# mooch443/trex

Measured on AMD Instinct MI355X. Metric: frames/s end-to-end (segment+CNN-ID), 2048x2048 x100 individuals, higher is better.
Workload: dtype fp16x3-split

## Files before the change

include/trexhip.h:

```cpp
#ifndef TREXHIP_H
#define TREXHIP_H
#include <stddef.h>
#include <stdint.h>
#ifdef __cplusplus
extern "C" {
#endif

#define TREXHIP_ABI_VERSION 26

enum {
    TREXHIP_OK = 0,
    TREXHIP_E_INVALID = -1,
    TREXHIP_E_DEVICE = -2,
    TREXHIP_E_CAPACITY = -3,
    TREXHIP_E_UNSUPPORTED = -4,
    TREXHIP_E_NOMEM = -5
};

#define TREXHIP_FRAME_OVERFLOW_RUNS   1u
#define TREXHIP_FRAME_OVERFLOW_OUTPUT 2u
#define TREXHIP_FRAME_MALFORMED       4u

typedef struct trexhip_params {
    int32_t device;
    int32_t width, height;
    int32_t max_batch;
    int32_t max_runs;
    int32_t max_blobs;
    int32_t max_pixels;
    int32_t threshold;
    int32_t threshold_maximum;
    int32_t enable_difference;
    int32_t absolute_difference;
    int32_t image_invert;
    int32_t inclusive;
    int32_t zero_is_background;
    int32_t connectivity;
    int32_t dilation_size;
    int32_t use_closing;
    int32_t closing_size;
    int32_t n_ranges;
    double  cm_per_pixel;
    double  ranges[16];
    int32_t pixel_encoding;
    int32_t image_adjust, blur_difference, equalize_histogram, correct_luminance, use_adaptive_threshold;
    int32_t device_color_reduce;
    int32_t reserved_[1];
} trexhip_params;
enum { TREXHIP_ENC_GRAY = 0, TREXHIP_ENC_R3G3B2 = 1, TREXHIP_ENC_RGB8 = 2 };

#define TREXHIP_BLOB_IN_RANGE    0u
#define TREXHIP_BLOB_BELOW_RANGE 1u
#define TREXHIP_BLOB_BIG         2u

typedef struct trexhip_run { uint16_t x0, x1, y, pad; } trexhip_run;

typedef struct trexhip_blob {
    uint32_t run_begin, n_runs;
    uint32_t pix_begin, n_pixels;
    uint16_t x0, y0, x1, y1;
    uint32_t bid;
    uint32_t px_min_max;
    uint32_t parent;
    uint32_t flags;
    uint64_t m10, m01;
    uint64_t m20, m11, m02;
    uint64_t sp, spx, spy;
} trexhip_blob;

typedef struct trexhip_frame_info {
    uint32_t n_blobs, n_runs, n_pixels;
    uint32_t blob_begin, run_begin, pix_begin;
    uint32_t n_raw_runs, n_raw_blobs;
    uint32_t flags;
    uint32_t reserved[3];
} trexhip_frame_info;

typedef struct trexhip_batch_result {
    int32_t n_frames;
    uint32_t total_blobs, total_runs, total_pixels;
    const trexhip_frame_info* frames;
    const trexhip_blob* blobs;
    const trexhip_run* runs;
    const uint8_t* pixels;
    uint32_t pixel_channels;
    uint32_t reserved_;
} trexhip_batch_result;

typedef struct trexhip_device_view {
    const trexhip_frame_info* frames;
    const trexhip_blob* blobs;
// ... 96 lines not shown
    double  size_ranges[16];
} trexhip_split_params;
typedef struct trexhip_split_info {
    int32_t threshold;
    int32_t effective_threshold;
    int32_t status;
    int32_t initial_action;
    int32_t n_result;
    int32_t n_evaluated;
    int32_t min_pixel, max_pixel;
    float   first_size;
    float   reserved_;
    double  min_size_bound;
} trexhip_split_info;
void trexhip_default_split_params(trexhip_split_params* p);
int trexhip_split_search_device(trexhip_ctx* ctx, const trexhip_split_params* sp, int32_t method, const int32_t* d_presumed_nr,
                                int32_t n_blobs, int32_t* d_thresholds, trexhip_split_info* d_info);

typedef struct trexhip_posture_params {
    float   outline_resample;
    int32_t outline_smooth_samples;
    int32_t outline_smooth_step;
    int32_t outline_approximate;
    float   outline_curvature_range_ratio;
    float   midline_walk_offset;
    int32_t max_points;
    int32_t posture_closing_steps, peak_mode, posture_direction_smoothing;
} trexhip_posture_params;
typedef struct trexhip_posture_info { int32_t status, n_outline, n_segments, tail_index, head_index, n_traced, reserved[2]; } trexhip_posture_info;
void trexhip_default_posture_params(trexhip_posture_params* p);
int trexhip_posture_device(trexhip_ctx* ctx, int32_t table, const trexhip_posture_params* pp, int32_t n_blobs,
                           float* d_outline, float* d_segments, trexhip_posture_info* d_info);

int trexhip_posture_auto_device(trexhip_ctx* ctx, const trexhip_posture_params* pp, int32_t method, int32_t track_posture_threshold,
                                int32_t n_blobs, float* d_outline, float* d_segments, trexhip_posture_info* d_info,
                                int32_t* d_threshold_used, int32_t* d_iterations);

typedef struct trexhip_midline_params {
    int32_t midline_resolution;
    float   midline_stiff_percentage;
    int32_t midline_invert;
    int32_t midline_start_with_head;
} trexhip_midline_params;
typedef struct trexhip_midline_info { int32_t status, n; float len, angle, offx, offy; int32_t reserved[2]; } trexhip_midline_info;
void trexhip_default_midline_params(trexhip_midline_params* p);
int trexhip_midline_device(trexhip_ctx* ctx, const trexhip_midline_params* mp, int32_t n_blobs, int32_t max_points,
                           const trexhip_posture_info* d_posture_info, float* d_segments, float* d_midline,
                           trexhip_midline_info* d_midline_info);
int trexhip_midline_movement_device(trexhip_ctx* ctx, const trexhip_midline_params* mp, int32_t n_blobs, int32_t max_points,
                                    const trexhip_posture_info* d_posture_info, float* d_segments, float* d_midline,
                                    trexhip_midline_info* d_midline_info, const float* d_movement_direction);

enum { TREXHIP_NORMALIZE_NONE = 0, TREXHIP_NORMALIZE_MOMENTS = 1, TREXHIP_NORMALIZE_POSTURE = 2 };
int trexhip_crops_device(trexhip_ctx* ctx, uint8_t* d_crops, int32_t n_blobs, int32_t out_w, int32_t out_h,
                         int32_t normalization, int32_t difference);

int trexhip_crops_transformed_device(trexhip_ctx* ctx, uint8_t* d_crops, int32_t n_blobs, int32_t out_w, int32_t out_h,
                                     const float* transforms, const float* midline_lengths, int32_t use_legacy,
                                     float image_scale, int32_t difference);
int trexhip_crops_posture_device(trexhip_ctx* ctx, uint8_t* d_crops, int32_t n_blobs, int32_t out_w, int32_t out_h,
                                 const trexhip_midline_info* d_midline_info, const float* midline_lengths, int32_t use_legacy,
                                 float image_scale, int32_t difference);

int trexhip_load_weights(trexhip_ctx* ctx, const void* blob, size_t bytes);
int trexhip_num_classes(trexhip_ctx* ctx);
int trexhip_network_channels(trexhip_ctx* ctx);
int trexhip_network_image_size(trexhip_ctx* ctx, int32_t* width, int32_t* height);
enum { TREXHIP_NET_V118_3 = 0, TREXHIP_NET_V100 = 1, TREXHIP_NET_V110 = 2, TREXHIP_NET_V119 = 3, TREXHIP_NET_V200 = 4 };
int trexhip_network_version(trexhip_ctx* ctx);
size_t trexhip_network_blob_bytes(int32_t version, int32_t classes, int32_t channels, int32_t width, int32_t height);
int trexhip_identify_chunk_crops(trexhip_ctx* ctx, int32_t* crops);
enum { TREXHIP_CNN_FP32 = 0, TREXHIP_CNN_BF16X6 = 1, TREXHIP_CNN_BF16X3 = 2, TREXHIP_CNN_FP16X3 = 3 };
int trexhip_set_identity_precision(trexhip_ctx* ctx, int32_t mode);
int trexhip_identify_device(trexhip_ctx* ctx, const uint8_t* d_crops, int32_t n, float* d_probs, float* d_logits);
int trexhip_identify_prepare_device(trexhip_ctx* ctx, const uint8_t* d_crops, int32_t n);
int trexhip_identify_prepare_stats(trexhip_ctx* ctx, uint32_t* records, uint32_t* hits);
int trexhip_identify(trexhip_ctx* ctx, const uint8_t* crops, int32_t n, float* probs);
int trexhip_identify_guard_stats(trexhip_ctx* ctx, uint32_t* rerun_crops, uint32_t* whole_batch);
int trexhip_identify_skip_stats(trexhip_ctx* ctx, uint32_t* passes, uint32_t* listed, uint64_t* bytes_filled);

int trexhip_identify_skip3_stats(trexhip_ctx* ctx, uint32_t* pairs, uint32_t* listed, uint32_t* passes, uint64_t* bytes_filled);

int trexhip_identify_skip3x_stats(trexhip_ctx* ctx, uint32_t* crops_windowed, uint32_t* windowed_passes, uint32_t* full_passes);

int trexhip_identify_skipx_stats(trexhip_ctx* ctx, uint32_t* crops_windowed, uint32_t* windowed_passes, uint32_t* full_passes);

int trexhip_identify_bgrow_stats(trexhip_ctx* ctx, uint32_t* rows_read, uint32_t* rows_made);

int trexhip_identify_fc1_stats(trexhip_ctx* ctx, uint32_t* rows, uint32_t* listed);

int trexhip_export_id_table_device(trexhip_ctx* ctx, const float* d_probs, int32_t n_blobs, int32_t classes,
                                   uint32_t frame_base, void* d_table, int32_t max_rows);
int trexhip_export_id_table_ex_device(trexhip_ctx* ctx, const float* d_probs, int32_t n_blobs, int32_t classes, uint32_t frame_base,
                                      const float* d_midline, const trexhip_midline_info* d_midline_info, int32_t midline_resolution,
                                      void* d_table, int32_t max_rows);

typedef struct trexhip_comm trexhip_comm;
int trexhip_comm_unique_id(void* id128);
int trexhip_comm_create(trexhip_ctx* ctx, const void* id128, int32_t rank, int32_t world, trexhip_comm** out);
void trexhip_comm_destroy(trexhip_comm* comm);
int trexhip_comm_rank(trexhip_comm* comm);
int trexhip_comm_world(trexhip_comm* comm);
int trexhip_comm_gather_device(trexhip_comm* comm, const void* d_send, size_t bytes, void* d_recv_rank0);
int trexhip_comm_gather_device_on(trexhip_comm* comm, trexhip_ctx* stream_ctx, const void* d_send, size_t bytes, void* d_recv_rank0);
int trexhip_comm_count_ranks(trexhip_comm* comm, int32_t* ranks_seen);

enum { TREXHIP_STAGE_ROWS = 0, TREXHIP_STAGE_SEGMENT_ALL = 1, TREXHIP_STAGE_CONV2 = 2, TREXHIP_STAGE_CONV3 = 3,
       TREXHIP_STAGE_CNN_ALL = 4, TREXHIP_STAGE_CROPS = 5, TREXHIP_STAGE_POSTURE = 6,
       TREXHIP_STAGE_UPLOAD_COPY = 8, TREXHIP_STAGE_UPLOAD_DMA = 9,
       TREXHIP_STAGE_PREPARE = 10, TREXHIP_STAGE_COUNT = 11 };
int trexhip_profile_enable(trexhip_ctx* ctx, int32_t on);
int trexhip_profile_read(trexhip_ctx* ctx, int32_t stage, double* total_ms, int64_t* launches);
int trexhip_profile_reset(trexhip_ctx* ctx);

#define TREXHIP_NET_CATEGORY 100
typedef struct trexhip_trainer trexhip_trainer;
typedef struct {
    int32_t max_batch;
    float lr;
    float beta1, beta2, eps;
    float bn_momentum;
    float dropout;
    int32_t precision;
    uint64_t seed;
} trexhip_train_params;
size_t trexhip_weight_blob_bytes(int32_t classes, int32_t channels);
int trexhip_trainer_create(trexhip_ctx* ctx, const void* blob, size_t bytes, const trexhip_train_params* params, trexhip_trainer** out);
void trexhip_trainer_destroy(trexhip_trainer* trainer);
int trexhip_trainer_set_lr(trexhip_trainer* trainer, float lr);
int64_t trexhip_trainer_steps(trexhip_trainer* trainer);
int trexhip_trainer_image_size(trexhip_trainer* trainer, int32_t* width, int32_t* height);
int trexhip_trainer_version(trexhip_trainer* trainer, int32_t* version);
size_t trexhip_trainer_keep_mask_bytes(trexhip_trainer* trainer, int32_t n);
int trexhip_train_step_device(trexhip_trainer* trainer, const float* d_inputs, const int32_t* d_targets, int32_t n, const uint8_t* d_keep_masks,
                              float* loss, int32_t* correct);
int trexhip_train_eval_device(trexhip_trainer* trainer, const float* d_inputs, const int32_t* d_targets, int32_t n, float* loss, int32_t* correct);
int trexhip_train_eval(trexhip_trainer* trainer, const float* inputs, const int32_t* targets, int32_t n, float* loss, int32_t* correct);
int trexhip_train_step(trexhip_trainer* trainer, const float* inputs, const int32_t* targets, int32_t n, const uint8_t* keep_masks, float* loss,
                       int32_t* correct);
int trexhip_train_predict_device(trexhip_trainer* trainer, const uint8_t* d_crops, int32_t n, float* d_probs);
int trexhip_trainer_read(trexhip_trainer* trainer, int32_t tensor, int32_t kind, float* out, size_t count);
int trexhip_trainer_export(trexhip_trainer* trainer, void* blob, size_t capacity, size_t* bytes);

typedef struct {
    float degrees;
    float translate_x, translate_y;
    float brightness_lo, brightness_hi;
    float contrast_lo, contrast_hi;
    float saturation_lo, saturation_hi;
    float hue_lo, hue_hi;
    uint64_t seed;
} trexhip_augment_params;
typedef struct {
    float angle; int32_t tx, ty;
    float brightness, contrast, saturation, hue;
    int32_t order;
} trexhip_augment_draw;
void trexhip_default_augment_params(trexhip_augment_params* p, int32_t width, int32_t height);
int trexhip_augment_device(trexhip_ctx* ctx, const trexhip_augment_params* ap, const uint8_t* d_pool, const int32_t* d_pool_targets,
                           int32_t pool_size, const int32_t* indices, int32_t n, int32_t width, int32_t height, int32_t channels,
                           trexhip_augment_draw* d_draws, int32_t draws_given, uint64_t counter, float* d_out, int32_t* d_targets_out);

typedef struct {
    uint32_t good_frames, bad_frames;
    float    good_ratio;
    float    mean_unique;
// ... 65 lines not shown
```

trex_amd/capi.py:

```python
import collections
import ctypes as C
import os
import numpy as np

_HERE = os.path.dirname(os.path.abspath(__file__))
LIB_PATH = os.environ.get("TREXHIP_LIB_PATH") or os.path.join(_HERE, "libtrexhip.so")
_LIB = None

RUN_DTYPE = np.dtype([("x0", "<u2"), ("x1", "<u2"), ("y", "<u2"), ("pad", "<u2")])
BLOB_DTYPE = np.dtype([
    ("run_begin", "<u4"), ("n_runs", "<u4"), ("pix_begin", "<u4"), ("n_pixels", "<u4"),
    ("x0", "<u2"), ("y0", "<u2"), ("x1", "<u2"), ("y1", "<u2"),
    ("bid", "<u4"), ("px_min_max", "<u4"), ("parent", "<u4"), ("flags", "<u4"),
    ("m10", "<u8"), ("m01", "<u8"), ("m20", "<u8"), ("m11", "<u8"), ("m02", "<u8"),
    ("sp", "<u8"), ("spx", "<u8"), ("spy", "<u8"),
])
INFO_DTYPE = np.dtype([
    ("n_blobs", "<u4"), ("n_runs", "<u4"), ("n_pixels", "<u4"),
    ("blob_begin", "<u4"), ("run_begin", "<u4"), ("pix_begin", "<u4"),
    ("n_raw_runs", "<u4"), ("n_raw_blobs", "<u4"), ("flags", "<u4"), ("reserved", "<u4", (3,)),
])
assert BLOB_DTYPE.itemsize == 104 and RUN_DTYPE.itemsize == 8 and INFO_DTYPE.itemsize == 48

CNN_FP32, CNN_BF16X6, CNN_BF16X3, CNN_FP16X3 = 0, 1, 2, 3
# ... 74 lines not shown
MIDLINE_INFO_DTYPE = np.dtype([("status", "<i4"), ("n", "<i4"), ("len", "<f4"), ("angle", "<f4"), ("offx", "<f4"), ("offy", "<f4"),
                               ("reserved", "<i4", (2,))])
POSTURE_INFO_DTYPE = np.dtype([("status", "<i4"), ("n_outline", "<i4"), ("n_segments", "<i4"), ("tail_index", "<i4"),
                               ("head_index", "<i4"), ("n_traced", "<i4"), ("reserved", "<i4", (2,))])


class BatchResult(C.Structure):
    _fields_ = [
        ("n_frames", C.c_int32), ("total_blobs", C.c_uint32), ("total_runs", C.c_uint32), ("total_pixels", C.c_uint32),
        ("frames", C.c_void_p), ("blobs", C.c_void_p), ("runs", C.c_void_p), ("pixels", C.c_void_p),
        ("pixel_channels", C.c_uint32), ("reserved_", C.c_uint32),
    ]


ENC_GRAY, ENC_R3G3B2, ENC_RGB8 = 0, 1, 2
FRAME_OVERFLOW_RUNS, FRAME_OVERFLOW_OUTPUT, FRAME_MALFORMED = 1, 2, 4


class DeviceView(C.Structure):
    _fields_ = [("frames", C.c_void_p), ("blobs", C.c_void_p), ("runs", C.c_void_p), ("pixels", C.c_void_p),
                ("totals", C.c_void_p), ("blob_frame", C.c_void_p)]


class TrexHipError(RuntimeError):
    def __init__(self, code, msg):
        super().__init__(f"libtrexhip error {code}: {msg}")
        self.code = code
        self.frames = None


class TrainParams(C.Structure):
    _fields_ = [("max_batch", C.c_int32), ("lr", C.c_float), ("beta1", C.c_float), ("beta2", C.c_float), ("eps", C.c_float),
                ("bn_momentum", C.c_float), ("dropout", C.c_float), ("precision", C.c_int32), ("seed", C.c_uint64)]


class AugmentParams(C.Structure):
    _fields_ = [("degrees", C.c_float), ("translate_x", C.c_float), ("translate_y", C.c_float), ("brightness_lo", C.c_float), ("brightness_hi", C.c_float),
                ("contrast_lo", C.c_float), ("contrast_hi", C.c_float), ("saturation_lo", C.c_float), ("saturation_hi", C.c_float),
                ("hue_lo", C.c_float), ("hue_hi", C.c_float), ("seed", C.c_uint64)]


AUGMENT_DRAW_DTYPE = np.dtype([("angle", "<f4"), ("tx", "<i4"), ("ty", "<i4"), ("brightness", "<f4"), ("contrast", "<f4"), ("saturation", "<f4"),
                               ("hue", "<f4"), ("order", "<i4")])
assert AUGMENT_DRAW_DTYPE.itemsize == 32
AUGMENT_IDENTITY_ORDER = 0xE4


class UniquenessResult(C.Structure):
    _fields_ = [("good_frames", C.c_uint32), ("bad_frames", C.c_uint32), ("good_ratio", C.c_float), ("mean_unique", C.c_float), ("mean_unique_raw", C.c_float)]


class ValidationMetrics:
    __slots__ = ("confusion", "per_class_accuracy", "good_frames", "bad_frames", "good_ratio", "mean_unique", "mean_unique_raw",
                 "unique_percent", "unique_percent_raw", "uniqueness_per_class")

    def __init__(self):
        for k in self.__slots__:
            setattr(self, k, None)


class ClassAverages:
    __slots__ = ("samples", "values", "max_index", "max_p")

    def __init__(self, samples, values, max_index, max_p):
        self.samples, self.values, self.max_index, self.max_p = samples, values, max_index, max_p


class VisualFieldResult:
    __slots__ = VF_OUTPUTS

    def __init__(self):
        for k in self.__slots__:
            setattr(self, k, None)


TrackletLabels = collections.namedtuple("TrackletLabels", "counts rows label share skipped")


SYMBOLS = [
    "trexhip_abi_version", "trexhip_network_channels", "trexhip_network_image_size", "trexhip_network_version", "trexhip_network_blob_bytes", "trexhip_identify_chunk_crops", "trexhip_comm_unique_id", "trexhip_comm_create", "trexhip_comm_destroy", "trexhip_comm_rank", "trexhip_comm_world", "trexhip_comm_gather_device", "trexhip_comm_gather_device_on", "trexhip_comm_count_ranks", "trexhip_last_error", "trexhip_default_params", "trexhip_create", "trexhip_destroy",
    "trexhip_set_stream", "trexhip_get_live_params", "trexhip_update_params", "trexhip_set_background", "trexhip_set_background_device", "trexhip_set_background_color", "trexhip_set_background_color_device", "trexhip_generate_average_device", "trexhip_get_background", "trexhip_segment_device",
    "trexhip_segment", "trexhip_segment_color", "trexhip_segment_color_device", "trexhip_rethreshold_device", "trexhip_rethreshold_per_blob_device", "trexhip_fetch_rethreshold", "trexhip_fetch", "trexhip_device_view_get", "trexhip_synchronize",
    "trexhip_profile_enable", "trexhip_profile_read", "trexhip_profile_reset",
    "trexhip_default_posture_params", "trexhip_posture_device", "trexhip_posture_auto_device", "trexhip_pack_frames_v6_device", "trexhip_crops_device", "trexhip_pixel_channels", "trexhip_device_alloc", "trexhip_device_free", "trexhip_copy_to_host", "trexhip_copy_to_device", "trexhip_crops_transformed_device", "trexhip_crops_posture_device", "trexhip_default_midline_params", "trexhip_midline_device", "trexhip_midline_movement_device", "trexhip_default_split_params", "trexhip_split_search_device", "trexhip_export_id_table_device", "trexhip_export_id_table_ex_device", "trexhip_load_weights", "trexhip_set_identity_precision", "trexhip_num_classes", "trexhip_identify_device", "trexhip_identify", "trexhip_identify_guard_stats", "trexhip_identify_skip_stats", "trexhip_identify_skip3_stats", "trexhip_identify_skip3x_stats", "trexhip_identify_skipx_stats", "trexhip_identify_bgrow_stats", "trexhip_identify_fc1_stats",
    "trexhip_weight_blob_bytes", "trexhip_trainer_create", "trexhip_trainer_destroy", "trexhip_trainer_set_lr", "trexhip_trainer_steps", "trexhip_trainer_image_size", "trexhip_trainer_version", "trexhip_trainer_keep_mask_bytes", "trexhip_train_step_device", "trexhip_train_step", "trexhip_train_eval_device", "trexhip_train_eval", "trexhip_trainer_read", "trexhip_trainer_export",
    "trexhip_default_augment_params", "trexhip_augment_device",
    "trexhip_train_predict_device", "trexhip_validation_metrics_device", "trexhip_class_averages_device",
    "trexhip_lzo1x_bound", "trexhip_lzo1x_compress", "trexhip_pv_write_frames",
    "trexhip_load_frames_v6_device", "trexhip_lzo1x_decompress", "trexhip_pv_read_frames",
    "trexhip_default_prefilter_params", "trexhip_prefilter_device",
    "trexhip_default_vf_params", "trexhip_visual_field_device",
    "trexhip_categorize_load_weights", "trexhip_categorize_info", "trexhip_categorize_blob_bytes", "trexhip_categorize_device", "trexhip_categorize",
    "trexhip_tracklet_labels_device", "trexhip_tracklet_medians_device",
    "trexhip_identify_prepare_device", "trexhip_fetch_begin", "trexhip_fetch_wait", "trexhip_identify_prepare_stats",
]


def lib():
    global _LIB
    if _LIB is None:
        if not os.path.exists(LIB_PATH):
            raise TrexHipError(-1, f"{LIB_PATH} is missing: run __graft_entry__.build() (make -C trex_amd/csrc)")
        L = C.CDLL(LIB_PATH)
        L.trexhip_last_error.restype = C.c_char_p
        L.trexhip_default_params.argtypes = [C.POINTER(Params), C.c_int32, C.c_int32]
        L.trexhip_default_params.restype = None
        L.trexhip_create.argtypes = [C.POINTER(Params), C.POINTER(C.c_void_p)]
        L.trexhip_destroy.argtypes = [C.c_void_p]
        L.trexhip_destroy.restype = None
        L.trexhip_set_stream.argtypes = [C.c_void_p, C.c_void_p]
        L.trexhip_get_live_params.argtypes = [C.c_void_p, C.POINTER(LiveParams)]
        L.trexhip_update_params.argtypes = [C.c_void_p, C.POINTER(LiveParams)]
        L.trexhip_set_background.argtypes = [C.c_void_p, C.c_void_p, C.c_int32]
        L.trexhip_set_background_device.argtypes = [C.c_void_p, C.c_void_p]
        L.trexhip_set_background_color.argtypes = [C.c_void_p, C.c_void_p, C.c_int32, C.c_int32, C.c_int32]
        L.trexhip_set_background_color_device.argtypes = [C.c_void_p, C.c_void_p, C.c_int32, C.c_int32]
        L.trexhip_generate_average_device.argtypes = [C.c_void_p, C.c_void_p, C.c_int32, C.c_int32]
        L.trexhip_get_background.argtypes = [C.c_void_p, C.c_void_p, C.c_int32]
        L.trexhip_segment_device.argtypes = [C.c_void_p, C.c_void_p, C.c_int32]
        L.trexhip_segment.argtypes = [C.c_void_p, C.POINTER(C.c_void_p), C.c_int32, C.c_int32]
        L.trexhip_segment_color.argtypes = [C.c_void_p, C.POINTER(C.c_void_p), C.c_int32, C.c_int32, C.c_int32, C.c_int32]
        L.trexhip_segment_color_device.argtypes = [C.c_void_p, C.c_void_p, C.c_int32, C.c_int32, C.c_int32]
        L.trexhip_rethreshold_device.argtypes = [C.c_void_p, C.c_int32, C.c_int32, C.c_void_p, C.c_int32]
        L.trexhip_rethreshold_per_blob_device.argtypes = [C.c_void_p, C.c_int32, C.c_void_p, C.c_int32, C.c_void_p, C.c_int32]
        L.trexhip_fetch_rethreshold.argtypes = [C.c_void_p, C.POINTER(BatchResult)]
        L.trexhip_fetch.argtypes = [C.c_void_p, C.POINTER(BatchResult)]
        L.trexhip_fetch_begin.argtypes = [C.c_void_p, C.POINTER(BatchResult)]
        L.trexhip_fetch_wait.argtypes = [C.c_void_p]
        L.trexhip_device_view_get.argtypes = [C.c_void_p, C.POINTER(DeviceView)]
        L.trexhip_synchronize.argtypes = [C.c_void_p]
        L.trexhip_profile_enable.argtypes = [C.c_void_p, C.c_int32]
        L.trexhip_profile_read.argtypes = [C.c_void_p, C.c_int32, C.POINTER(C.c_double), C.POINTER(C.c_int64)]
        L.trexhip_profile_reset.argtypes = [C.c_void_p]
        L.trexhip_default_midline_params.argtypes = [C.POINTER(MidlineParams)]
        L.trexhip_default_midline_params.restype = None
        L.trexhip_midline_device.argtypes = [C.c_void_p, C.POINTER(MidlineParams), C.c_int32, C.c_int32, C.c_void_p, C.c_void_p, C.c_void_p, C.c_void_p]
        L.trexhip_midline_movement_device.argtypes = [C.c_void_p, C.POINTER(MidlineParams), C.c_int32, C.c_int32, C.c_void_p, C.c_void_p, C.c_void_p, C.c_void_p, C.c_void_p]
        L.trexhip_default_split_params.argtypes = [C.POINTER(SplitParams)]
        L.trexhip_default_split_params.restype = None
        L.trexhip_split_search_device.argtypes = [C.c_void_p, C.POINTER(SplitParams), C.c_int32, C.c_void_p, C.c_int32, C.c_void_p, C.c_void_p]
        L.trexhip_crops_posture_device.argtypes = [C.c_void_p, C.c_void_p, C.c_int32, C.c_int32, C.c_int32, C.c_void_p, C.c_void_p, C.c_int32, C.c_float, C.c_int32]
        L.trexhip_default_posture_params.argtypes = [C.POINTER(PostureParams)]
        L.trexhip_default_posture_params.restype = None
        L.trexhip_posture_device.argtypes = [C.c_void_p, C.c_int32, C.POINTER(PostureParams), C.c_int32, C.c_void_p, C.c_void_p, C.c_void_p]
        L.trexhip_posture_auto_device.argtypes = [C.c_void_p, C.POINTER(PostureParams), C.c_int32, C.c_int32, C.c_int32, C.c_void_p, C.c_void_p, C.c_void_p, C.c_void_p, C.c_void_p]
        L.trexhip_crops_transformed_device.argtypes = [C.c_void_p, C.c_void_p, C.c_int32, C.c_int32, C.c_int32, C.c_void_p, C.c_void_p, C.c_int32, C.c_float, C.c_int32]
        L.trexhip_crops_device.argtypes = [C.c_void_p, C.c_void_p] + [C.c_int32] * 5
        L.trexhip_export_id_table_device.argtypes = [C.c_void_p, C.c_void_p, C.c_int32, C.c_int32, C.c_uint32, C.c_void_p, C.c_int32]
        L.trexhip_export_id_table_ex_device.argtypes = [C.c_void_p, C.c_void_p, C.c_int32, C.c_int32, C.c_uint32, C.c_void_p, C.c_void_p, C.c_int32, C.c_void_p, C.c_int32]
        L.trexhip_load_weights.argtypes = [C.c_void_p, C.c_void_p, C.c_size_t]
        L.trexhip_num_classes.argtypes = [C.c_void_p]
        L.trexhip_network_channels.argtypes = [C.c_void_p]
        L.trexhip_network_image_size.argtypes = [C.c_void_p, C.POINTER(C.c_int32), C.POINTER(C.c_int32)]
        L.trexhip_network_version.argtypes = [C.c_void_p]
        L.trexhip_network_blob_bytes.argtypes = [C.c_int32] * 5; L.trexhip_network_blob_bytes.restype = C.c_size_t
        L.trexhip_identify_chunk_crops.argtypes = [C.c_void_p, C.POINTER(C.c_int32)]
        L.trexhip_pack_frames_v6_device.argtypes = [C.c_void_p, C.c_void_p, C.c_void_p, C.c_size_t, C.c_void_p]
        L.trexhip_lzo1x_bound.argtypes = [C.c_size_t]; L.trexhip_lzo1x_bound.restype = C.c_size_t
        L.trexhip_lzo1x_compress.argtypes = [C.c_void_p, C.c_size_t, C.c_void_p, C.c_size_t, C.POINTER(C.c_size_t)]
        L.trexhip_pv_write_frames.argtypes = [C.c_void_p, C.c_void_p, C.c_int32, C.c_int32, C.c_uint64, C.c_void_p, C.c_size_t, C.c_void_p, C.POINTER(C.c_size_t)]
        L.trexhip_load_frames_v6_device.argtypes = [C.c_void_p, C.c_void_p, C.c_void_p, C.c_int32, C.c_void_p]
        L.trexhip_lzo1x_decompress.argtypes = [C.c_void_p, C.c_size_t, C.c_void_p, C.c_size_t, C.POINTER(C.c_size_t)]
        L.trexhip_pv_read_frames.argtypes = [C.c_void_p, C.c_size_t, C.c_uint64, C.c_void_p, C.c_int32, C.c_void_p, C.c_size_t, C.c_void_p, C.POINTER(C.c_size_t)]
        L.trexhip_comm_unique_id.argtypes = [C.c_void_p]
        L.trexhip_comm_create.argtypes = [C.c_void_p, C.c_void_p, C.c_int32, C.c_int32, C.POINTER(C.c_void_p)]
        L.trexhip_comm_destroy.argtypes = [C.c_void_p]
        L.trexhip_comm_destroy.restype = None
        L.trexhip_comm_rank.argtypes = [C.c_void_p]
        L.trexhip_comm_world.argtypes = [C.c_void_p]
        L.trexhip_comm_gather_device.argtypes = [C.c_void_p, C.c_void_p, C.c_size_t, C.c_void_p]
        L.trexhip_comm_gather_device_on.argtypes = [C.c_void_p, C.c_void_p, C.c_void_p, C.c_size_t, C.c_void_p]
        L.trexhip_comm_count_ranks.argtypes = [C.c_void_p, C.POINTER(C.c_int32)]
        L.trexhip_set_identity_precision.argtypes = [C.c_void_p, C.c_int32]
        L.trexhip_identify_device.argtypes = [C.c_void_p, C.c_void_p, C.c_int32, C.c_void_p, C.c_void_p]
        L.trexhip_identify_prepare_device.argtypes = [C.c_void_p, C.c_void_p, C.c_int32]
        L.trexhip_identify_prepare_stats.argtypes = [C.c_void_p, C.POINTER(C.c_uint32), C.POINTER(C.c_uint32)]
        L.trexhip_identify.argtypes = [C.c_void_p, C.c_void_p, C.c_int32, C.c_void_p]
        L.trexhip_identify_guard_stats.argtypes = [C.c_void_p, C.POINTER(C.c_uint32), C.POINTER(C.c_uint32)]
        L.trexhip_identify_skip_stats.argtypes = [C.c_void_p, C.POINTER(C.c_uint32), C.POINTER(C.c_uint32), C.POINTER(C.c_uint64)]
        L.trexhip_identify_skipx_stats.argtypes = [C.c_void_p, C.POINTER(C.c_uint32), C.POINTER(C.c_uint32), C.POINTER(C.c_uint32)]
        L.trexhip_identify_bgrow_stats.argtypes = [C.c_void_p, C.POINTER(C.c_uint32), C.POINTER(C.c_uint32)]
        L.trexhip_identify_skip3x_stats.argtypes = [C.c_void_p, C.POINTER(C.c_uint32), C.POINTER(C.c_uint32), C.POINTER(C.c_uint32)]
        L.trexhip_identify_skip3_stats.argtypes = [C.c_void_p, C.POINTER(C.c_uint32), C.POINTER(C.c_uint32), C.POINTER(C.c_uint32), C.POINTER(C.c_uint64)]
        L.trexhip_identify_fc1_stats.argtypes = [C.c_void_p, C.POINTER(C.c_uint32), C.POINTER(C.c_uint32)]
        L.trexhip_weight_blob_bytes.argtypes = [C.c_int32, C.c_int32]
        L.trexhip_weight_blob_bytes.restype = C.c_size_t
        L.trexhip_trainer_create.argtypes = [C.c_void_p, C.c_void_p, C.c_size_t, C.POINTER(TrainParams), C.POINTER(C.c_void_p)]
        L.trexhip_trainer_destroy.argtypes = [C.c_void_p]
        L.trexhip_trainer_destroy.restype = None
        L.trexhip_trainer_set_lr.argtypes = [C.c_void_p, C.c_float]
        L.trexhip_trainer_steps.argtypes = [C.c_void_p]
        L.trexhip_trainer_steps.restype = C.c_int64
        L.trexhip_trainer_image_size.argtypes = [C.c_void_p, C.POINTER(C.c_int32), C.POINTER(C.c_int32)]
        L.trexhip_trainer_version.argtypes = [C.c_void_p, C.POINTER(C.c_int32)]
        L.trexhip_trainer_keep_mask_bytes.argtypes = [C.c_void_p, C.c_int32]
        L.trexhip_trainer_keep_mask_bytes.restype = C.c_size_t
        L.trexhip_train_step_device.argtypes = [C.c_void_p, C.c_void_p, C.c_void_p, C.c_int32, C.c_void_p, C.POINTER(C.c_float), C.POINTER(C.c_int32)]
        L.trexhip_train_step.argtypes = [C.c_void_p, C.c_void_p, C.c_void_p, C.c_int32, C.c_void_p, C.POINTER(C.c_float), C.POINTER(C.c_int32)]
        L.trexhip_train_eval_device.argtypes = [C.c_void_p, C.c_void_p, C.c_void_p, C.c_int32, C.POINTER(C.c_float), C.POINTER(C.c_int32)]
        L.trexhip_train_eval.argtypes = [C.c_void_p, C.c_void_p, C.c_void_p, C.c_int32, C.POINTER(C.c_float), C.POINTER(C.c_int32)]
        L.trexhip_trainer_read.argtypes = [C.c_void_p, C.c_int32, C.c_int32, C.c_void_p, C.c_size_t]
        L.trexhip_trainer_export.argtypes = [C.c_void_p, C.c_void_p, C.c_size_t, C.POINTER(C.c_size_t)]
        L.trexhip_default_augment_params.argtypes = [C.POINTER(AugmentParams), C.c_int32, C.c_int32]
        L.trexhip_default_augment_params.restype = None
        L.trexhip_augment_device.argtypes = [C.c_void_p, C.POINTER(AugmentParams), C.c_void_p, C.c_void_p, C.c_int32, C.c_void_p, C.c_int32, C.c_int32, C.c_int32,
                                             C.c_int32, C.c_void_p, C.c_int32, C.c_uint64, C.c_void_p, C.c_void_p]
        L.trexhip_train_predict_device.argtypes = [C.c_void_p, C.c_void_p, C.c_int32, C.c_void_p]
        L.trexhip_validation_metrics_device.argtypes = [C.c_void_p, C.c_void_p, C.c_int32, C.c_int32, C.c_void_p, C.c_void_p, C.c_int32, C.c_void_p,
                                                        C.POINTER(UniquenessResult), C.c_void_p, C.c_void_p, C.c_void_p]
        L.trexhip_class_averages_device.argtypes = [C.c_void_p, C.c_void_p, C.c_int32, C.c_int32, C.c_void_p, C.c_int32, C.c_void_p, C.c_void_p, C.c_void_p, C.c_void_p]
        L.trexhip_device_alloc.argtypes = [C.c_void_p, C.c_size_t, C.POINTER(C.c_void_p)]
        L.trexhip_device_free.argtypes = [C.c_void_p, C.c_void_p]
        L.trexhip_copy_to_host.argtypes = [C.c_void_p, C.c_void_p, C.c_void_p, C.c_size_t]
        L.trexhip_copy_to_device.argtypes = [C.c_void_p, C.c_void_p, C.c_void_p, C.c_size_t]
        L.trexhip_default_prefilter_params.argtypes = [C.POINTER(PrefilterParams)]
        L.trexhip_default_prefilter_params.restype = None
        L.trexhip_prefilter_device.argtypes = [C.c_void_p, C.POINTER(PrefilterParams), C.POINTER(PrefilterTables), C.c_void_p, C.c_void_p, C.c_void_p, C.c_void_p]
        L.trexhip_default_vf_params.argtypes = [C.c_void_p, C.POINTER(VfParams)]
        L.trexhip_default_vf_params.restype = None
        L.trexhip_visual_field_device.argtypes = [C.c_void_p, C.POINTER(VfParams), C.c_void_p, C.c_void_p, C.c_void_p, C.c_int32, C.c_void_p, C.c_int32,
                                                  C.c_void_p, C.c_int32, C.c_void_p, C.c_void_p, C.c_void_p, C.c_void_p, C.c_void_p, C.c_void_p]
        L.trexhip_categorize_load_weights.argtypes = [C.c_void_p, C.c_void_p, C.c_size_t]
        L.trexhip_categorize_info.argtypes = [C.c_void_p, C.POINTER(C.c_int32), C.POINTER(C.c_int32), C.POINTER(C.c_int32), C.POINTER(C.c_int32)]
        L.trexhip_categorize_blob_bytes.argtypes = [C.c_int32, C.c_int32, C.c_int32, C.c_int32]
        L.trexhip_categorize_blob_bytes.restype = C.c_size_t
        L.trexhip_categorize_device.argtypes = [C.c_void_p, C.c_void_p, C.c_int32, C.c_void_p, C.c_void_p, C.c_void_p]
        L.trexhip_categorize.argtypes = [C.c_void_p, C.c_void_p, C.c_int32, C.c_void_p]
        L.trexhip_tracklet_labels_device.argtypes = [C.c_void_p, C.c_void_p, C.c_void_p, C.c_int32, C.c_int32, C.c_int32, C.c_void_p, C.c_void_p, C.c_void_p,
                                                     C.c_void_p, C.POINTER(C.c_uint32)]
        L.trexhip_tracklet_medians_device.argtypes = [C.c_void_p, C.c_void_p, C.c_int32, C.c_int32, C.c_int32, C.c_int32, C.c_void_p, C.c_int32, C.c_void_p, C.c_void_p]
        _LIB = L
    return _LIB


def _check(rc):
    if rc != 0:
        raise TrexHipError(rc, lib().trexhip_last_error().decode())


def default_params(width, height, **kw):
    p = Params()
    lib().trexhip_default_params(C.byref(p), width, height)
    ranges = kw.pop("size_ranges", None)
    for k, v in kw.items():
        if not hasattr(p, k):
            raise KeyError(k)
        setattr(p, k, v)
    if ranges is not None:
        p.n_ranges = len(ranges)
        for i, (a, b) in enumerate(ranges):
            p.ranges[2 * i], p.ranges[2 * i + 1] = a, b
    return p


def default_augment_params(width, height, **kw):
    p = AugmentParams()
    lib().trexhip_default_augment_params(C.byref(p), width, height)
    for k, v in kw.items():
        if not hasattr(p, k):
            raise KeyError(k)
        setattr(p, k, v)
    return p


def _from_addr(addr, count, dtype):
# ... 223 lines not shown
                                                  None if ln is None else ln.ctypes.data_as(C.c_void_p), 1 if legacy else 0, scale, difference))

    def crops_transformed_device(self, d_crops_ptr, transforms, midline_lengths, out_w=80, out_h=80, legacy=False, scale=1.0, difference=0):
        tr = np.ascontiguousarray(transforms, np.float32)
        ln = np.ascontiguousarray(midline_lengths, np.float32)
        _check(lib().trexhip_crops_transformed_device(self._h, C.c_void_p(d_crops_ptr), len(tr), out_w, out_h, tr.ctypes.data_as(C.c_void_p),
                                                      ln.ctypes.data_as(C.c_void_p), 1 if legacy else 0, scale, difference))

    def export_id_table_ex(self, d_probs_ptr, n_blobs, classes, frame_base, d_table_ptr, max_rows, d_midline_ptr=0, d_midline_info_ptr=0, midline_resolution=0):
        _check(lib().trexhip_export_id_table_ex_device(self._h, C.c_void_p(d_probs_ptr) if d_probs_ptr else None, n_blobs, classes, frame_base,
                                                       C.c_void_p(d_midline_ptr) if d_midline_ptr else None,
                                                       C.c_void_p(d_midline_info_ptr) if d_midline_info_ptr else None, midline_resolution,
                                                       C.c_void_p(d_table_ptr), max_rows))

    def export_id_table(self, d_probs_ptr, n_blobs, classes, frame_base, d_table_ptr, max_rows):
        _check(lib().trexhip_export_id_table_device(self._h, C.c_void_p(d_probs_ptr) if d_probs_ptr else None, n_blobs,
                                                    classes, frame_base, C.c_void_p(d_table_ptr), max_rows))

    def load_weights(self, blob: bytes):
        buf = (C.c_uint8 * len(blob)).from_buffer_copy(blob)
        _check(lib().trexhip_load_weights(self._h, buf, len(blob)))

    def set_identity_precision(self, mode):
        _check(lib().trexhip_set_identity_precision(self._h, mode))

    def num_classes(self):
        return lib().trexhip_num_classes(self._h)

    def network_image_size(self):
        w, h = C.c_int32(0), C.c_int32(0)
        _check(lib().trexhip_network_image_size(self._h, C.byref(w), C.byref(h)))
        return int(w.value), int(h.value)

    def network_version(self):
        return int(lib().trexhip_network_version(self._h))

    def identify_chunk_crops(self):
        c = C.c_int32(0)
        _check(lib().trexhip_identify_chunk_crops(self._h, C.byref(c)))
        return int(c.value)

    def probabilities(self, crops):
        crops = np.ascontiguousarray(crops, np.uint8)
        w, h = self.network_image_size()
        if w:
            want = (h, w, lib().trexhip_network_channels(self._h))
            if crops.ndim != 4 or tuple(crops.shape[1:]) != want:
                raise ValueError(f"crops must have shape (n, {want[0]}, {want[1]}, {want[2]}) for the loaded network, got {crops.shape}")
        n = crops.shape[0]
        out = np.empty((n, self.num_classes()), np.float32)
        _check(lib().trexhip_identify(self._h, crops.ctypes.data_as(C.c_void_p), n, out.ctypes.data_as(C.c_void_p)))
        return out

    def guard_stats(self):
        a, b = C.c_uint32(0), C.c_uint32(0)
        _check(lib().trexhip_identify_guard_stats(self._h, C.byref(a), C.byref(b)))
        return int(a.value), bool(b.value)

    def skip_stats(self):
        a, b, c = C.c_uint32(0), C.c_uint32(0), C.c_uint64(0)
        _check(lib().trexhip_identify_skip_stats(self._h, C.byref(a), C.byref(b), C.byref(c)))
        return int(a.value), int(b.value), int(c.value)

    def skipx_stats(self):
        a, b, c = C.c_uint32(0), C.c_uint32(0), C.c_uint32(0)
        _check(lib().trexhip_identify_skipx_stats(self._h, C.byref(a), C.byref(b), C.byref(c)))
        return int(a.value), int(b.value), int(c.value)

    def bgrow_stats(self):
        a, b = C.c_uint32(0), C.c_uint32(0)
        _check(lib().trexhip_identify_bgrow_stats(self._h, C.byref(a), C.byref(b)))
        return int(a.value), int(b.value)

    def skip3_stats(self):
        a, b, c, d = C.c_uint32(0), C.c_uint32(0), C.c_uint32(0), C.c_uint64(0)
        _check(lib().trexhip_identify_skip3_stats(self._h, C.byref(a), C.byref(b), C.byref(c), C.byref(d)))
        return int(a.value), int(b.value), int(c.value), int(d.value)

    def skip3x_stats(self):
        a, b, c = C.c_uint32(0), C.c_uint32(0), C.c_uint32(0)
        _check(lib().trexhip_identify_skip3x_stats(self._h, C.byref(a), C.byref(b), C.byref(c)))
        return int(a.value), int(b.value), int(c.value)

    def fc1_stats(self):
        a, b = C.c_uint32(0), C.c_uint32(0)
        _check(lib().trexhip_identify_fc1_stats(self._h, C.byref(a), C.byref(b)))
        return int(a.value), int(b.value)

    def identify_device(self, d_crops_ptr, n, d_probs_ptr, d_logits_ptr=None):
        _check(lib().trexhip_identify_device(self._h, C.c_void_p(d_crops_ptr), n, C.c_void_p(d_probs_ptr),
                                             C.c_void_p(d_logits_ptr) if d_logits_ptr else None))

    def identify_prepare_device(self, d_crops_ptr, n):
        _check(lib().trexhip_identify_prepare_device(self._h, C.c_void_p(d_crops_ptr), n))

    def prepare_stats(self):
        a, b = C.c_uint32(0), C.c_uint32(0)
        _check(lib().trexhip_identify_prepare_stats(self._h, C.byref(a), C.byref(b)))
        return int(a.value), int(b.value)

    def device_alloc(self, nbytes):
        out = C.c_void_p()
        _check(lib().trexhip_device_alloc(self._h, nbytes, C.byref(out)))
        return int(out.value)

    def device_free(self, d_ptr):
        _check(lib().trexhip_device_free(self._h, C.c_void_p(d_ptr or 0)))

    def copy_to_device(self, d_ptr, array):
        a = np.ascontiguousarray(array)
        _check(lib().trexhip_copy_to_device(self._h, C.c_void_p(d_ptr), a.ctypes.data_as(C.c_void_p), a.nbytes))

    def copy_to_host(self, d_ptr, shape, dtype):
        out = np.empty(shape, dtype)
        _check(lib().trexhip_copy_to_host(self._h, out.ctypes.data_as(C.c_void_p), C.c_void_p(d_ptr), out.nbytes))
        return out

    def augment_device(self, d_pool_ptr, pool_size, n, width, height, channels, d_out_ptr, ap=None, indices=None, d_pool_targets_ptr=0,
                       d_targets_out_ptr=0, d_draws_ptr=0, draws_given=False, counter=0):
        idx = None
        if indices is not None:
            idx = np.ascontiguousarray(indices, np.int32)
            if idx.shape != (n,):
                raise ValueError(f"indices must hold n = {n} entries, got shape {idx.shape}")
        _check(lib().trexhip_augment_device(self._h, C.byref(ap) if ap is not None else None, C.c_void_p(d_pool_ptr), C.c_void_p(d_pool_targets_ptr or 0), pool_size,
                                            idx.ctypes.data_as(C.c_void_p) if idx is not None else None, n, width, height, channels,
                                            C.c_void_p(d_draws_ptr or 0), 1 if draws_given else 0, counter, C.c_void_p(d_out_ptr), C.c_void_p(d_targets_out_ptr or 0)))

    def validation_metrics(self, d_probs_ptr, n, classes, d_targets_ptr=0, frame_ranges=None):
        out = ValidationMetrics()
        conf = np.zeros((classes, classes), np.uint32) if d_targets_ptr else None
        fr = None
        res = UniquenessResult()
        up = upr = upc = None
        if frame_ranges is not None:
            fr = np.ascontiguousarray(frame_ranges, np.int32).reshape(-1, 2)
            up, upr, upc = np.zeros(len(fr), np.float32), np.zeros(len(fr), np.float32), np.zeros(classes, np.float32)
        ptr = lambda a: a.ctypes.data_as(C.c_void_p) if a is not None else None
        _check(lib().trexhip_validation_metrics_device(self._h, C.c_void_p(d_probs_ptr or 0), n, classes, C.c_void_p(d_targets_ptr or 0), ptr(fr),
                                                       len(fr) if fr is not None else 0, ptr(conf), C.byref(res) if fr is not None else None,
                                                       ptr(up), ptr(upr), ptr(upc)))
        if conf is not None:
            rows = conf.sum(axis=1, dtype=np.int64)
            out.confusion = conf
            out.per_class_accuracy = np.zeros(classes, np.float64)
            np.divide(np.diagonal(conf), rows, out=out.per_class_accuracy, where=rows > 0)
        if fr is not None:
            out.good_frames, out.bad_frames = int(res.good_frames), int(res.bad_frames)
            out.good_ratio, out.mean_unique, out.mean_unique_raw = float(res.good_ratio), float(res.mean_unique), float(res.mean_unique_raw)
            out.unique_percent, out.unique_percent_raw, out.uniqueness_per_class = up, upr, upc
        return out

    def class_averages(self, d_probs_ptr, n, classes, d_ids_ptr, n_ids):
        samples, values = np.zeros(max(n_ids, 0), np.float32), np.zeros((max(n_ids, 0), max(classes, 0)), np.float32)
        max_index, max_p = np.zeros(max(n_ids, 0), np.int32), np.zeros(max(n_ids, 0), np.float32)
        ptr = lambda a: a.ctypes.data_as(C.c_void_p)
        _check(lib().trexhip_class_averages_device(self._h, C.c_void_p(d_probs_ptr or 0), n, classes, C.c_void_p(d_ids_ptr or 0), n_ids,
                                                   ptr(samples), ptr(values), ptr(max_index), ptr(max_p)))
        return ClassAverages(samples, values, max_index, max_p)

    def load_category_weights(self, blob):
        _check(lib().trexhip_categorize_load_weights(self._h, blob, len(blob)))

    def category_info(self):
        v = [C.c_int32(0) for _ in range(4)]
        _check(lib().trexhip_categorize_info(self._h, *[C.byref(x) for x in v]))
# ... 429 lines not shown
```

trex_amd/csrc/cnn.hip:

```cpp
#include "cnn_net.h"
#include "cnn_arch.h"
#include "cnn_split.h"
#include "conv_tiled.h"
#include "cnn_weights.h"
#include <algorithm>
#include <cmath>
#include <cstdio>
#include <cstdlib>
#include <cstring>
#include <vector>

namespace trexhip {

template <int CH>
__global__ __launch_bounds__(256, 2) void k_conv1(const uint8_t* __restrict__ crops, const float* __restrict__ w ,
                                                  const float* __restrict__ bias , float* __restrict__ out, int S) {
    extern __shared__ __attribute__((aligned(16))) float lds[];
    const int PW = S + 4;
    float* wl = lds;
    float* img = lds + CH * 25 * 16;
    const int crop = blockIdx.x;
    const uint8_t* src = crops + (size_t)crop * S * S * CH;
    for (int i = threadIdx.x; i < CH * PW * PW; i += 256) img[i] = 0.f;
    for (int i = threadIdx.x; i < CH * 25 * 16; i += 256) wl[i] = w[i];
// ... 1169 lines not shown
    const int prc = parse_weight_blob(blob, bytes, "trexhip_load_weights", &wb, [](int W, int H) -> int {
        if (W < 8 || W > 256 || H < 8 || H > 256) {
            set_error("trexhip_load_weights: individual_image_size " + std::to_string(W) + "x" + std::to_string(H) + " is outside 8..256 x 8..256");
            return TREXHIP_E_UNSUPPORTED;
        }
        return TREXHIP_OK;
    });
    if (prc != TREXHIP_OK) return prc;
    const int classes = wb.classes, W = wb.W, H = wb.H, CH = wb.CH;
    const bool at80 = W == 80 && H == 80;

    TH_CHECK_HIP(hipSetDevice(ctx->p.device));
    free_net(static_cast<Net*>(ctx->net));
    ctx->net = nullptr;
    Net* net = new Net();
    net->classes = classes; net->W = W; net->H = H; net->CH = CH;
    int rc = TREXHIP_OK;
    const Folded c1 = fold_conv1(&wb.t[T_C1W], CH);
    TRY(upload(net, &net->w1, c1.w)); TRY(upload(net, &net->b1, c1.b));
    if (at80) TRY(upload(net, &net->w1h, &net->inv1h, pack_conv1_frags(c1.w, CH)));
    const Folded c2 = fold_conv(&wb.t[T_C2W], 64, 16, 16);
    TRY(upload(net, &net->w2, c2.w)); TRY(upload(net, &net->b2, c2.b));
    TRY(upload(net, &net->w2s, pack_bf16x3(c2.w, 16, 64)));
    TRY(upload(net, &net->w2h, &net->inv2h, pack_f16x2(c2.w, 16, 64)));
    if (at80) TRY(upload(net, &net->w2w, &net->inv2w, pack_wino_f16(c2.w, 16, 64)));
    const Folded c3 = fold_conv(&wb.t[T_C3W], 128, 64, 16);
    TRY(upload(net, &net->w3s, pack_bf16x3(c3.w, 64, 128)));
    TRY(upload(net, &net->w3h, &net->inv3h, pack_f16x2(c3.w, 64, 128)));
    if (at80) TRY(upload(net, &net->w3w, &net->inv3w, pack_wino_f16(c3.w, 64, 128)));
    TRY(net->weights.device_bytes(&net->d_ovf, OVF_WORDS * 4, "trexhip_load_weights"));
    if (rc == TREXHIP_OK && hipMemset(net->d_ovf, 0, OVF_WORDS * 4) != hipSuccess) rc = TREXHIP_E_DEVICE;
    const Folded c3x = fold_conv(&wb.t[T_C3W], 128, 64, 32);
    TRY(upload(net, &net->w3, c3x.w)); TRY(upload(net, &net->b3, c3x.b));
    const Folded f1 = pack_fc1(wb.t[T_F1W], wb.t[T_F1B], W, H);
    TRY(upload(net, &net->wf1, f1.w)); TRY(upload(net, &net->bf1, f1.b));
    if (at80) TRY(upload(net, &net->wf1h, &net->invf1h, pack_fc1_f16(f1.w)));
    TRY(upload(net, &net->lng, wb.t[T_LNG], 100 * sizeof(float)));
    TRY(upload(net, &net->lnb, wb.t[T_LNB], 100 * sizeof(float)));
    TRY(upload(net, &net->wf2t, pack_fc2(wb.t[T_F2W], classes)));
    TRY(upload(net, &net->bf2, wb.t[T_F2B], classes * sizeof(float)));
    if (at80 && CH == 1) TRY(make_empty_v3(ctx, net));
    if (rc != TREXHIP_OK) { free_net(net); return rc; }
    ctx->net = net;
    return TREXHIP_OK;
}

static int ensure_act(trexhip_ctx* ctx, Net* net, int n) {
    if (n <= net->max_crops) return TREXHIP_OK;
    drop_graphs(net);
    ctx->prepared.batch_reallocated();
    net->batch.free_all();
    net->h_probs = nullptr;
    net->max_crops = 0;
    Mem& B = net->batch;
    const char* who = "trexhip_identify_device";
    const size_t N = n;
    const size_t W = net->W, H = net->H;
    int rc = B.device_bytes(&net->d_ovfc, N, who);
    TRY(B.device_bytes(&net->act1, N * (H / 2) * (W / 2) * 16 * 4, who));
    TRY(B.device_bytes(&net->act2, N * (H / 4) * (W / 4) * 64 * 4, who));
    TRY(B.device_bytes(&net->act3, N * (H / 8) * (W / 8) * 128 * 4, who));
    TRY(B.device_bytes(&net->fc1, N * 128 * 4 * FC1_KSPLIT, who));
    TRY(B.device_bytes(&net->probs, N * net->classes * 4, who));
    TRY(B.device_bytes(&net->logits, N * net->classes * 4, who));
    if (W == 80 && H == 80) {
        TRY(B.device_bytes(&net->v2, N * 40 * V2_ROWB, who));
        const size_t img = net->v3e ? (size_t)SkipGeom::V3_ROWS * V3_ROWB : 0;
        TRY(B.device_bytes(&net->v3, N * 20 * V3_ROWB + 2 * img, who));
        if (rc == TREXHIP_OK && img) {
            TH_CHECK_HIP(hipMemcpyAsync(net->v3, net->v3e, img, hipMemcpyDeviceToDevice, ctx->stream));
            TH_CHECK_HIP(hipMemcpyAsync(net->v3 + img + N * 20 * V3_ROWB, net->v3e, img, hipMemcpyDeviceToDevice, ctx->stream));
            net->v3 += img;
        }
    }
    if (net->v3e) {
        const size_t n_pass = (N * SkipGeom::V3_ROWS + SkipGeom::RPP - 1) / SkipGeom::RPP;
        TRY(B.device_bytes(&net->skip_bands, N * sizeof(int2), who));
        TRY(B.device_bytes(&net->skip_counts, ((n_pass + SKIP_LB - 1) / SKIP_LB) * SKIP_NCNT * 4, who));
        TRY(B.device_bytes(&net->skip_list, (n_pass + SKIP_PAD) * 4, who));
        TRY(B.device_bytes(&net->skipx_cols, N * sizeof(int2), who));
        TRY(B.device_bytes(&net->skipx_list, (N * skipx_passes({0, SkipGeom::V3_ROWS - 1}) + SKIP_PAD) * 4, who));
        TRY(B.device_bytes(&net->skipx_rows, (N * skipx_passes({0, SkipGeom::V3_ROWS - 1}) + SKIP_PAD) * 4, who));
        const size_t blocks3 = (N + Skip3Geom::BLOCK - 1) / Skip3Geom::BLOCK;
        TRY(B.device_bytes(&net->skip3_counts, ((blocks3 + SKIP3_TB - 1) / SKIP3_TB) * sizeof(uint4), who));
        TRY(B.device_bytes(&net->skip3_tcounts, blocks3 * 2 * sizeof(uint32_t), who));
        TRY(B.device_bytes(&net->skip3_desc, blocks3 * Skip3Geom::BLOCK_PASSES * Skip3Geom::DESC * 4, who));
        TRY(B.device_bytes(&net->skip3_rows, blocks3 * Skip3Geom::BLOCK_PASSES * Skip3Reach::WORDS * 4, who));
        TRY(B.device_bytes(&net->skip3x_desc, blocks3 * Skip3XGeom::BLOCK_PASSES * Skip3XGeom::DESC * 4, who));
        TRY(B.device_bytes(&net->skip3x_rows, blocks3 * Skip3XGeom::BLOCK_PASSES * Skip3Reach::WORDS * 4, who));
        TRY(B.device_bytes(&net->fc1_list, Skip3Geom::PAIRS * N * sizeof(int), who));
    }
    TRY(B.device_bytes(&net->crops, N * net->W * net->H * net->CH, who));
    TRY(B.pinned(&net->h_probs, N * net->classes, who));
    if (rc != TREXHIP_OK) return rc;
    TH_CHECK_HIP(hipMemsetAsync(net->d_ovfc, 0, N, ctx->stream));
    net->max_crops = n;
    return TREXHIP_OK;
}
#undef TRY

std::vector<LdsAttr>& lds_attrs() { static std::vector<LdsAttr> v; return v; }

static const ByChannels K_CONV1{Kern(k_conv1<1>, 256, (84 * 84 + 25 * 16) * 4, false), Kern(k_conv1<3>, 256, 3 * (84 * 84 + 25 * 16) * 4, false)};
static const ByChannels K_CONV1_MFMA{Kern(k_conv1_mfma, 256), Kern(k_conv1_mfma3, 256)};
static const ByChannels K_CONV1_WPRE{Kern(k_conv1_wpre<1>, 256), Kern(k_conv1_wpre<3>, 256)};
static const Kern K_CONV12_RS(k_conv12_rs<W12RGeom>, 512, W12RGeom::LDS_BYTES);
static const Kern K_CONV12_RSX(k_conv12_rs<W12XGeom>, 512, W12XGeom::LDS_BYTES);
static const Kern K_CONV12_WPRE(k_conv12_wpre, 256, W12Geom::LDS_BYTES);
static const Kern K_CROP_BANDS(k_crop_bands, 256);
static const Kern K_PASS_COUNT(k_pass_count, SKIP_LB);
static const Kern K_PASS_LIST(k_pass_list, SKIP_LB);
static const Kern K_V3_FILL(k_v3_fill, SKIP_FILL_TB);
static const Kern K_CONV2_WPRE2(k_conv2_wpre2, 256, W2bGeom::LDS_BYTES);
static const Kern K_CONV2_STREAM(k_conv5_stream<16, 64, 40, 8, 4>, 256, ConvGeomS<16, 64, 40, 8, 4>::LDS_BYTES);
using GW3 = WinoGeom<64, 128, 20, 2>;
static const Kern K_CONV3_WINO(k_conv5_wino<64, 128, 20, 2>, GW3::NTHR, GW3::LDS_BYTES);
static const Kern K_CONV3_WPAIR(k_conv5_wpair<false>, 256, GW3::LDS_BYTES + 1024 );
static const Kern K_CONV3_WPAIR_LIST(k_conv5_wpair<true>, 256, GW3::LDS_BYTES + 1024);
using GW3X = Wino3Pass<Skip3XGeom::TILES, Skip3XGeom::NR>;
static const Kern K_CONV3_WPAIR_LISTX(k_conv5_wpair<true, Skip3XGeom>, 256, GW3X::LDS_BYTES + 1024);
static const Kern K_PAIR_COUNT(k_pair_count, SKIP3_NT);
static const Kern K_PAIR_LIST(k_pair_list, SKIP3_NT);
static const Kern K_ACT3_FILL(k_act3_fill, 256);
template <int CI, int CO, int S, int ROWS, int NTERMS>
static auto split_kern() { return Kern(k_conv5_split<CI, CO, S, ROWS, NTERMS>, 512, ConvGeomB<CI, CO, S, ROWS, SPLIT_NP>::LDS_BYTES); }
struct ExactLayer { decltype(Kern(k_conv5<16, 64, 40, 20, 16>, 512)) f32; decltype(split_kern<16, 64, 40, 10, 6>()) x6, x3, x6_plan; };
static const auto K_CONV2_X6 = split_kern<16, 64, 40, 10, 6>();
static const ExactLayer K_CONV2{Kern(k_conv5<16, 64, 40, 20, 16>, 512, ConvGeom<16, 64, 40, 20, 16>::LDS_BYTES), K_CONV2_X6, split_kern<16, 64, 40, 10, 3>(), K_CONV2_X6};
static const ExactLayer K_CONV3{Kern(k_conv5<64, 128, 20, 20, 32>, 512, ConvGeom<64, 128, 20, 20, 32>::LDS_BYTES), split_kern<64, 128, 20, 20, 6>(),
                                split_kern<64, 128, 20, 20, 3>(), split_kern<64, 128, 20, 4, 6>()};
static const Kern K_FC1(k_fc1, 256);
static const Kern K_FC1_SPLIT1(k_fc1_split<1>, 256), K_FC1_SPLIT4(k_fc1_split<4>, 256), K_FC1_SPLIT4_LIST(k_fc1_split<4, true>, 256);
static const Kern K_FC1_LIST(k_fc1_list, FC1L_TB);
static const Kern K_HEAD(k_head, 256);
static const Kern K_HEAD_SMALL(k_head_small, 256);
static const Kern K_GUARD_PLAN(k_guard_plan, 1024);

struct Pass {
    const Net& net; const CnnPlan& p; hipStream_t s; int mode;
    const uint8_t* crops; int n; float *probs, *logits;
};

static void launch_conv1(const Pass& f, const Conv1 kind, const uint32_t* guard) {
    const Net& net = f.net;
    switch (kind) {
    case Conv1::FUSED: break;
    case Conv1::WPRE: K_CONV1_WPRE[net.CH](f.s, f.p.conv1_grid, f.crops, net.w1h, net.b1, net.v2, net.inv1h, net.ovf(OVF_RANGE)); break;
    case Conv1::MFMA: K_CONV1_MFMA[net.CH](f.s, f.p.conv1_grid, f.crops, net.w1h, net.b1, net.act1, net.inv1h, guard); break;
    case Conv1::VALU: K_CONV1[net.CH](f.s, f.p.conv1_grid, f.crops, net.w1, net.b1, net.act1, net.W); break;
    case Conv1::ANY: any_conv1(f.s, net, f.p, f.crops); break;
    }
}

static void launch_exact(const Pass& f, const int layer, const int mode, const uint32_t* guard) {
    const Net& net = f.net;
    const bool c2 = layer == 2;
    const ExactLayer& K = c2 ? K_CONV2 : K_CONV3;
    const Launch& l = guard ? (c2 ? f.p.r_conv2 : f.p.r_conv3) : (c2 ? f.p.conv2 : f.p.conv3);
    const float *in = c2 ? net.act1 : net.act2, *b = c2 ? net.b2 : net.b3;
    float* out = c2 ? net.act2 : net.act3;
    if (mode == TREXHIP_CNN_FP32) K.f32(f.s, l.grid, in, c2 ? net.w2 : net.w3, b, out);
    else (guard ? K.x6_plan : mode == TREXHIP_CNN_BF16X6 ? K.x6 : K.x3)(f.s, l.grid, in, c2 ? net.w2s : net.w3s, b, out, 1.0f, guard, l.items);
}

static void launch_tail(const Pass& f, const uint32_t* guard) {
    const Net& net = f.net;
    const CnnPlan& p = f.p;
    if (guard || p.fc1 == Fc1::EXACT)
        K_FC1(f.s, dim3(guard ? p.r_fc1_grid : p.fc1_grid, p.planes), net.act3, net.wf1, net.bf1, net.fc1, f.n, p.K, guard);
    else if (p.fc1_listed)
        K_FC1_SPLIT4_LIST(f.s, dim3(p.fc1_grid, p.planes), net.act3, net.wf1h, net.bf1, net.fc1, f.n, p.K, net.invf1h, net.ovf(OVF_RANGE), net.d_ovfc,
                          net.fc1_list, net.d_skip + SK3_FC1_LEN, net.max_crops);
    else
        (p.fc1 == Fc1::SPLIT1 ? K_FC1_SPLIT1 : K_FC1_SPLIT4)(f.s, dim3(p.fc1_grid, p.planes), net.act3, net.wf1h, net.bf1, net.fc1, f.n, p.K, net.invf1h,
                                                            net.ovf(OVF_RANGE), net.d_ovfc, nullptr, nullptr, 0);
    if (guard || p.head == Head::BIG) {
        const bool listed = !guard && p.fc1_listed;
        K_HEAD(f.s, guard ? p.r_head_grid : p.head_grid, net.fc1, net.lng, net.lnb, net.wf2t, net.bf2, f.probs, f.logits, f.n, net.classes, guard, p.planes,
               listed ? net.fc1e : nullptr, listed ? net.skip_bands : nullptr, listed ? net.d_skip : nullptr);
    }
    else
        K_HEAD_SMALL(f.s, p.head_grid, net.fc1, net.lng, net.lnb, net.wf2t, net.bf2, f.probs, f.logits, f.n, net.classes, p.planes,
                     p.head_plans ? net.ovf(OVF_RANGE) : nullptr, net.d_ovfc, p.head_plans ? net.ovf(OVF_PLAN) : nullptr);
}

static void launch_rerun(const Pass& f) {
    const uint32_t* g = f.net.ovf(OVF_PLAN);
    if (!f.p.head_plans) K_GUARD_PLAN(f.s, 1, f.net.ovf(OVF_RANGE), f.net.d_ovfc, f.n, f.net.ovf(OVF_PLAN));
    if (f.p.rerun_conv1) launch_conv1(f, Conv1::MFMA, g);
    for (const int layer : {2, 3}) {
        if (f.p.chain == Chain::ANY_SIZE) any_conv(f.s, f.net, f.p, layer, TREXHIP_CNN_BF16X6, g);
        else launch_exact(f, layer, TREXHIP_CNN_BF16X6, g);
    }
    launch_tail(f, g);
}

static int make_empty_v3(trexhip_ctx* ctx, Net* net) {
    const char* who = "trexhip_load_weights";
    uint8_t* zero = nullptr;
    int rc = net->weights.device_bytes(&net->v3e, (size_t)SkipGeom::V3_ROWS * V3_ROWB, who);
    if (rc == TREXHIP_OK) rc = net->weights.device_bytes(&net->act3e, (size_t)Skip3Geom::PAIRS * 10 * 128 * 4, who);
    if (rc == TREXHIP_OK) rc = net->weights.device_bytes(&net->fc1e, (size_t)FC1_KSPLIT * 128 * 4, who);
    if (rc == TREXHIP_OK) rc = net->weights.device_bytes(&net->d_skip, SK_WORDS * 4, who);
    if (rc == TREXHIP_OK) rc = net->weights.device_bytes(&net->act2e, (size_t)SkipGeom::V3_ROWS * 20 * 64 * 4, who);
    if (rc == TREXHIP_OK) rc = net->weights.device_bytes(&net->bgtab, (size_t)W2xGeom::NBG * W2xGeom::BG_UNITS * sizeof(uint4), who);
    if (rc == TREXHIP_OK) rc = net->weights.device_bytes(&zero, SkipGeom::CROP_ROWS * 80, who);
    if (rc != TREXHIP_OK) return rc;
    const CnnPlan p = cnn_plan(80, 80, 1, TREXHIP_CNN_FP16X3, true, GEOM_ROLE_SPLIT | GEOM_NO_SKIP, 1, ctx->n_cus);
    TH_CHECK_HIP(hipFuncSetAttribute(reinterpret_cast<const void*>(K_CONV12_RS.fn), hipFuncAttributeMaxDynamicSharedMemorySize, K_CONV12_RS.lds));
    TH_CHECK_HIP(hipMemsetAsync(net->d_skip, 0, SK_WORDS * 4, ctx->stream));
    TH_CHECK_HIP(hipMemsetAsync(zero, 0, SkipGeom::CROP_ROWS * 80, ctx->stream));
    K_CONV12_RS(ctx->stream, p.conv2.grid, zero, net->w1h, net->b1, net->inv1h, net->w2w, net->b2, net->v3e, net->inv2w, net->d_skip + SK_EMPTY_RANGE, 1,
                net->d_skip + SK_EMPTY_CTR, p.pk2, nullptr, nullptr, nullptr, net->act2e, nullptr, nullptr);
    TH_CHECK_HIP(hipGetLastError());
    TH_CHECK_HIP(hipFuncSetAttribute(reinterpret_cast<const void*>(K_CONV12_RSX.fn), hipFuncAttributeMaxDynamicSharedMemorySize, K_CONV12_RSX.lds));
    K_CONV12_RSX(ctx->stream, 1, zero, net->w1h, net->b1, net->inv1h, net->w2w, net->b2, net->v3e, net->inv2w, net->d_skip + SK_EMPTY_RANGE, 1,
                 net->d_skip + SKX_CTR, 1, nullptr, nullptr, nullptr, net->act2e, nullptr, net->bgtab);
    TH_CHECK_HIP(hipGetLastError());
    TH_CHECK_HIP(hipFuncSetAttribute(reinterpret_cast<const void*>(K_CONV3_WPAIR.fn), hipFuncAttributeMaxDynamicSharedMemorySize, K_CONV3_WPAIR.lds));
    K_CONV3_WPAIR(ctx->stream, p.conv3.grid, net->v3e, net->w3w, net->b3, net->act3e, net->inv3w, 1, net->d_skip + SK3_EMPTY_CTR, p.n_big3, nullptr, nullptr, nullptr);
    TH_CHECK_HIP(hipGetLastError());
    const CnnPlan pf = cnn_plan(80, 80, 1, TREXHIP_CNN_FP16X3, true, 0, 1, ctx->n_cus);
    K_FC1_SPLIT4(ctx->stream, dim3(1, pf.planes), net->act3e, net->wf1h, net->bf1, net->fc1e, 1, pf.K, net->invf1h, net->d_skip + SK3_FC1E_RANGE, nullptr,
                 nullptr, nullptr, 0);
    TH_CHECK_HIP(hipGetLastError());
    uint32_t range = 0;
    TH_CHECK_HIP(hipMemcpyAsync(&range, net->d_skip + SK3_FC1E_RANGE, 4, hipMemcpyDeviceToHost, ctx->stream));
    TH_CHECK_HIP(hipStreamSynchronize(ctx->stream));
    if (range) {
        const uint32_t one = 1;
        TH_CHECK_HIP(hipMemcpy(net->d_skip + SK_EMPTY_RANGE, &one, 4, hipMemcpyHostToDevice));
    }
    return TREXHIP_OK;
}

struct PrepArgs { long long alloc_rows; bool direct, x3 ; };
static PrepArgs prep_args(const Net& net, const CnnPlan& p) {
    const long long alloc_rows = (long long)net.max_crops * SkipGeom::V3_ROWS;
    const bool direct = p.v3_direct && skip3_direct_fits(alloc_rows);
    return {alloc_rows, direct, p.skip3x && direct && skip3x_direct_fits(alloc_rows)};
}
static void launch_skip_prep(const Pass& f, const bool direct, const bool x3) {
    const Net& net = f.net;
    const CnnPlan& p = f.p;
    const int n = f.n, lb = ceil_div(p.conv2.items, SKIP_LB);
    int2* cols = p.skipx ? net.skipx_cols : nullptr;
    K_CROP_BANDS(f.s, ceil_div(n, 4), f.crops, n, net.skip_bands, cols || x3 ? net.skipx_cols : nullptr);
    K_PASS_COUNT(f.s, lb, net.skip_bands, cols, n, net.d_skip, net.skip_counts, (int)p.bgrows);
    K_PASS_LIST(f.s, lb, net.skip_bands, cols, n, net.d_skip, net.skip_counts, net.skip_list, net.skipx_list, net.skipx_rows, (int)p.bgrows);
    if (p.skip3) {
        const int2* cols3 = x3 ? net.skipx_cols : nullptr;
        K_PAIR_COUNT(f.s, p.skip3_grid, net.skip_bands, cols3, n, net.d_skip, net.skip3_counts, net.skip3_tcounts);
        K_PAIR_LIST(f.s, p.skip3_grid, net.skip_bands, cols3, n, net.d_skip, net.skip3_counts, net.skip3_tcounts, net.skip3_desc, net.skip3x_desc);
        if (p.fc1_listed) K_FC1_LIST(f.s, Skip3Geom::PAIRS, net.skip_bands, n, net.d_skip, net.fc1_list, net.max_crops);
    }
    K_V3_FILL(f.s, ceil_div(n * SkipGeom::V3_ROWS, SKIP_FILL_TB), net.skip_bands, cols, n, net.d_skip, reinterpret_cast<const uint4*>(net.v3e),
              reinterpret_cast<uint4*>(net.v3), (int)direct);
}

enum : int { PREP_LISTS = 1, PREP_ACT3 = 2 };
static bool plan_prepares(const CnnPlan& p) { return p.chain == Chain::ROLE_SPLIT && p.skip; }
static void launch_prep(const Pass& f, const int parts) {
    const Net& net = f.net;
    const CnnPlan& p = f.p;
    if (!plan_prepares(p)) return;
    const PrepArgs a = prep_args(net, p);
    if (parts & PREP_LISTS) launch_skip_prep(f, a.direct, a.x3);
    if ((parts & PREP_ACT3) && p.skip3)
        K_ACT3_FILL(f.s, p.act3_fill.grid, net.skip_bands, a.x3 ? net.skipx_cols : nullptr, f.n, net.d_skip, reinterpret_cast<const uint4*>(net.act3e),
                    reinterpret_cast<uint4*>(net.act3), net.skip3_desc, net.skip3_rows, net.skip3x_desc, net.skip3x_rows, a.alloc_rows, (int)a.direct, (int)!p.fc1_listed);
}

static int set_cnn_attrs(trexhip_ctx* ctx) {
    if (!ctx->attr_cnn) {
        for (const LdsAttr& a : lds_attrs()) TH_CHECK_HIP(hipFuncSetAttribute(a.fn, hipFuncAttributeMaxDynamicSharedMemorySize, a.bytes));
        ctx->attr_cnn = true;
    }
    return TREXHIP_OK;
}

static int net_forward_launch(trexhip_ctx* ctx, const uint8_t* d_crops, int n, float* d_probs, float* d_logits, const bool prepared = false) {
    const Net& net = *static_cast<Net*>(ctx->net);
    if (const int rc = set_cnn_attrs(ctx)) return rc;
    const CnnPlan p = cnn_plan(net.W, net.H, net.CH, ctx->cnn_mode, (reinterpret_cast<uintptr_t>(d_crops) & 15) == 0, ctx->tune_conv_geom, n, ctx->n_cus);
    const Pass f{net, p, ctx->stream, ctx->cnn_mode, d_crops, n, d_probs, d_logits};
    hipStream_t s = f.s;
    const bool x3 = prep_args(net, p).x3;
    stage_begin(ctx, TREXHIP_STAGE_CNN_ALL);
    launch_conv1(f, p.conv1, nullptr);
    if (p.chain == Chain::ANY_SIZE) {
        any_conv(s, net, p, 2, f.mode, nullptr);
        any_conv(s, net, p, 3, f.mode, nullptr);
    } else {
        const bool pre = p.chain == Chain::ROLE_SPLIT || p.chain == Chain::FUSED_2WG || p.chain == Chain::TWO_KERNEL;
        stage_begin(ctx, TREXHIP_STAGE_CONV2);
        switch (p.chain) {
        case Chain::ROLE_SPLIT:
            if (!prepared) launch_prep(f, PREP_LISTS);
            if (p.skipx)
                K_CONV12_RSX(s, p.conv2.grid, d_crops, net.w1h, net.b1, net.inv1h, net.w2w, net.b2, net.v3, net.inv2w, net.ovf(OVF_RANGE), n, net.d_skip + SKX_CTR,
                             p.pk2, net.d_ovfc, net.skipx_list, net.d_skip + SKX_PASSES, net.act2e, net.skipx_rows, net.bgtab);
            K_CONV12_RS(s, p.conv2.grid, d_crops, net.w1h, net.b1, net.inv1h, net.w2w, net.b2, net.v3, net.inv2w, net.ovf(OVF_RANGE), n, net.ovf(OVF_PASS2),
                        p.pk2, net.d_ovfc, p.skip ? net.skip_list : nullptr, p.skip ? net.d_skip + (p.skipx ? SKX_FULL : SK_LEN) : nullptr, nullptr, nullptr, nullptr);
            break;
        case Chain::FUSED_2WG:
            K_CONV12_WPRE(s, p.conv2.grid, d_crops, net.w1h, net.b1, net.inv1h, net.w2w, net.b2, net.v3, net.inv2w, net.ovf(OVF_RANGE), n, net.ovf(OVF_PASS2),
                          p.pk2, net.d_ovfc);
            break;
        case Chain::TWO_KERNEL:
            K_CONV2_WPRE2(s, p.conv2.grid, net.v2, net.w2w, net.b2, net.v3, net.inv2w, net.ovf(OVF_RANGE), n, net.ovf(OVF_PASS2));
            break;
        case Chain::FP32_ACT:
            K_CONV2_STREAM(s, p.conv2.grid, net.act1, net.w2h, net.b2, net.act2, net.inv2h, net.ovf(OVF_RANGE), p.conv2.items);
            break;
        default: launch_exact(f, 2, f.mode, nullptr);
        }
        stage_end(ctx, TREXHIP_STAGE_CONV2);
        stage_begin(ctx, TREXHIP_STAGE_CONV3);
        if (pre) {
            if (p.skip3) {
                if (!prepared) launch_prep(f, PREP_ACT3);
                if (x3)
                    K_CONV3_WPAIR_LISTX(s, p.conv3.grid, net.v3, net.w3w, net.b3, net.act3, net.inv3w, n, net.d_skip + SK3X_CTR, 0, net.skip3x_desc, net.skip3x_rows, net.d_skip);
                K_CONV3_WPAIR_LIST(s, p.conv3.grid, net.v3, net.w3w, net.b3, net.act3, net.inv3w, n, net.ovf(OVF_PASS3), 0, net.skip3_desc, net.skip3_rows, net.d_skip);
            }
            K_CONV3_WPAIR(s, p.conv3.grid, net.v3, net.w3w, net.b3, net.act3, net.inv3w, n, net.ovf(OVF_PASS3), p.n_big3, nullptr, nullptr, p.skip3 ? net.d_skip : nullptr);
        }
        else if (p.chain == Chain::FP32_ACT)
            K_CONV3_WINO(s, p.conv3.grid, net.act2, net.w3w, net.b3, net.act3, net.inv3w, net.ovf(OVF_RANGE), n, net.ovf(OVF_PASS3));
        else launch_exact(f, 3, f.mode, nullptr);
        stage_end(ctx, TREXHIP_STAGE_CONV3);
    }
    launch_tail(f, nullptr);
    if (p.rerun) launch_rerun(f);
    stage_end(ctx, TREXHIP_STAGE_CNN_ALL);
    TH_CHECK_HIP(hipGetLastError());
    return TREXHIP_OK;
}

static constexpr int GRAPH_MAX_CROPS = 6400;
static constexpr size_t GRAPH_CACHE = 8;
static constexpr int GRAPH_MIN_SEEN = 3;

static bool graph_path(const trexhip_ctx* ctx, const Net* net, const int n) {
    static const bool enabled = [] { const char* e = std::getenv("TREXHIP_GRAPHS"); return !(e && std::atoi(e) == 0); }();
    return enabled && net->graphs_ok && n <= GRAPH_MAX_CROPS && !ctx->profiling && ctx->attr_cnn;
}

static int net_forward_inner(trexhip_ctx* ctx, const uint8_t* d_crops, int n, float* d_probs, float* d_logits, bool prepared);
int net_forward(trexhip_ctx* ctx, const uint8_t* d_crops, int n, float* d_probs, float* d_logits) {
    Net* net = static_cast<Net*>(ctx->net);
    const bool prepared = ctx->prepared.consume(ctx->prepared.make(d_crops, n, ctx->cnn_mode, ctx->tune_conv_geom, ctx->stream));
    if (ctx->cnn_mode == TREXHIP_CNN_FP16X3) {
        if (!net->ovf_clean) TH_CHECK_HIP(hipMemsetAsync(net->d_ovf, 0, OVF_PLAN * 4, ctx->stream));
        net->ovf_clean = false;
    }
    const int rc = net_forward_inner(ctx, d_crops, n, d_probs, d_logits, prepared);
    if (rc == TREXHIP_OK) { net->last_mode = ctx->cnn_mode; if (ctx->cnn_mode == TREXHIP_CNN_FP16X3) net->ovf_clean = true; }
    net->last_fc1_n = rc == TREXHIP_OK && !net->arch && cnn_plan(net->W, net->H, net->CH, ctx->cnn_mode, (reinterpret_cast<uintptr_t>(d_crops) & 15) == 0,
                                                                 ctx->tune_conv_geom, n, ctx->n_cus).fc1_listed ? n : 0;
    return rc;
}

static bool capture_chain(trexhip_ctx* ctx, Net* net, Net::GraphEntry* cand, const uint8_t* d_crops, int n, float* d_probs, float* d_logits) {
    hipGraph_t graph = nullptr;
    hipGraphExec_t exec = nullptr;
    hipEvent_t ev = nullptr;
    bool ok = hipStreamBeginCapture(ctx->stream, hipStreamCaptureModeThreadLocal) == hipSuccess;
    if (ok) {
        const int rc = net_forward_launch(ctx, d_crops, n, d_probs, d_logits);
        const hipError_t e_end = hipStreamEndCapture(ctx->stream, &graph);
        ok = rc == TREXHIP_OK && e_end == hipSuccess && graph && hipGraphInstantiate(&exec, graph, nullptr, nullptr, 0) == hipSuccess &&
             hipEventCreateWithFlags(&ev, hipEventDisableTiming) == hipSuccess;
    }
    if (graph) (void)hipGraphDestroy(graph);
    if (!ok) {
        (void)hipGetLastError();
        if (exec) (void)hipGraphExecDestroy(exec);
        net->graphs_ok = false;
        return false;
    }
    cand->exec = exec; cand->last = ev;
    return true;
}

static int net_forward_inner(trexhip_ctx* ctx, const uint8_t* d_crops, int n, float* d_probs, float* d_logits, const bool prepared) {
    Net* net = static_cast<Net*>(ctx->net);
    if (net->arch) return arch_forward(ctx, *net, d_crops, n, d_probs, d_logits);
    if (!graph_path(ctx, net, n)) return net_forward_launch(ctx, d_crops, n, d_probs, d_logits, prepared);
    hipStream_t s = ctx->stream;
    const Net::GraphKey key{d_crops, n, d_probs, d_logits, ctx->cnn_mode, ctx->tune_conv_geom, s};
    ++net->tick;
    Net::GraphEntry* cand = nullptr;
    for (auto& g : net->graphs)
        if (g.key == key) { cand = &g; break; }
    if (!cand) {
        if (net->graphs.size() >= GRAPH_CACHE) {
            size_t lru = 0;
            for (size_t i = 1; i < net->graphs.size(); ++i) if (net->graphs[i].used < net->graphs[lru].used) lru = i;
            destroy_graph_entry(net->graphs[lru]);
            net->graphs.erase(net->graphs.begin() + (long)lru);
        }
        net->graphs.push_back({key, nullptr, net->tick, nullptr, 1});
        return net_forward_launch(ctx, d_crops, n, d_probs, d_logits);
    }
    cand->used = net->tick;
    if (!cand->exec && (++cand->seen < GRAPH_MIN_SEEN || !capture_chain(ctx, net, cand, d_crops, n, d_probs, d_logits)))
// ... 50 lines not shown
    ctx->prepared.set(ctx->prepared.make(d_crops, n, ctx->cnn_mode, ctx->tune_conv_geom, ctx->stream));
    return TREXHIP_OK;
}

int trexhip_identify_prepare_stats(trexhip_ctx* ctx, uint32_t* records, uint32_t* hits) {
    if (!ctx) { set_error("trexhip_identify_prepare_stats: null ctx"); return TREXHIP_E_INVALID; }
    if (records) *records = ctx->prepared.records;
    if (hits) *hits = ctx->prepared.hits;
    return TREXHIP_OK;
}

int trexhip_identify(trexhip_ctx* ctx, const uint8_t* crops, int32_t n, float* probs) {
    Net* net;
    int rc = identify_prepare(ctx, ctx && crops && probs, "trexhip_identify", n, &net);
    if (rc || !net) return rc;
    const size_t cb = (size_t)net->W * net->H * net->CH;
    TH_CHECK_HIP(hipMemcpyAsync(net->crops, crops, cb * n, hipMemcpyHostToDevice, ctx->stream));
    rc = net_forward(ctx, net->crops, n, net->probs, nullptr);
    if (rc) return rc;
    TH_CHECK_HIP(hipMemcpyAsync(probs, net->probs, (size_t)n * net->classes * 4, hipMemcpyDeviceToHost, ctx->stream));
    TH_CHECK_HIP(hipStreamSynchronize(ctx->stream));
    return TREXHIP_OK;
}

int trexhip_identify_guard_stats(trexhip_ctx* ctx, uint32_t* rerun_crops, uint32_t* whole_batch) {
    if (!ctx || !ctx->net) { set_error("trexhip_identify_guard_stats: no context / weights not loaded"); return TREXHIP_E_INVALID; }
    Net* net = static_cast<Net*>(ctx->net);
    uint32_t plan[2] = {0, 0};
    TH_CHECK_HIP(hipStreamSynchronize(ctx->stream));
    if (net->last_mode == TREXHIP_CNN_FP16X3 && net->arch) {
        uint32_t st[2] = {0, 0};
        TH_CHECK_HIP(hipMemcpy(st, net->ovf(ARCH_STAT_RERUN), 8, hipMemcpyDeviceToHost));
        if (rerun_crops) *rerun_crops = st[0];
        if (whole_batch) *whole_batch = st[1] ? 1u : 0u;
        return TREXHIP_OK;
    }
    if (net->last_mode == TREXHIP_CNN_FP16X3) TH_CHECK_HIP(hipMemcpy(plan, net->ovf(OVF_PLAN), 8, hipMemcpyDeviceToHost));
    if (rerun_crops) *rerun_crops = plan[1] == 1u ? plan[0] : 0u;
    if (whole_batch) *whole_batch = plan[1] == 2u ? 1u : 0u;
    return TREXHIP_OK;
}

static int read_skip_words(trexhip_ctx* ctx, const char* who, uint32_t (&w)[SK_WORDS]) {
    if (!ctx || !ctx->net) { set_error(std::string(who) + ": no context / weights not loaded"); return TREXHIP_E_INVALID; }
    const Net* net = static_cast<Net*>(ctx->net);
    std::fill(w, w + SK_WORDS, 0u);
    TH_CHECK_HIP(hipStreamSynchronize(ctx->stream));
    if (net->d_skip) TH_CHECK_HIP(hipMemcpy(w, net->d_skip, sizeof w, hipMemcpyDeviceToHost));
    return TREXHIP_OK;
}

int trexhip_identify_skip_stats(trexhip_ctx* ctx, uint32_t* passes, uint32_t* listed, uint64_t* bytes_filled) {
    uint32_t w[SK_WORDS];
    if (const int rc = read_skip_words(ctx, "trexhip_identify_skip_stats", w)) return rc;
    if (passes) *passes = w[SK_NPASS];
    if (listed) *listed = w[SK_LEN];
    if (bytes_filled) *bytes_filled = (uint64_t)w[SK_FILLED] * V3_ROWB;
    return TREXHIP_OK;
}

int trexhip_identify_skipx_stats(trexhip_ctx* ctx, uint32_t* crops_windowed, uint32_t* windowed_passes, uint32_t* full_passes) {
    uint32_t w[SK_WORDS];
    if (const int rc = read_skip_words(ctx, "trexhip_identify_skipx_stats", w)) return rc;
    if (crops_windowed) *crops_windowed = w[SKX_CROPS];
    if (windowed_passes) *windowed_passes = w[SKX_PASSES];
    if (full_passes) *full_passes = w[SKX_FULL];
    return TREXHIP_OK;
}

int trexhip_identify_bgrow_stats(trexhip_ctx* ctx, uint32_t* rows_read, uint32_t* rows_made) {
    uint32_t w[SK_WORDS];
    if (const int rc = read_skip_words(ctx, "trexhip_identify_bgrow_stats", w)) return rc;
    if (rows_read) *rows_read = w[SKX_V2_READ];
    if (rows_made) *rows_made = w[SKX_V2_MADE];
    return TREXHIP_OK;
}

int trexhip_identify_skip3x_stats(trexhip_ctx* ctx, uint32_t* crops_windowed, uint32_t* windowed_passes, uint32_t* full_passes) {
    uint32_t w[SK_WORDS];
    if (const int rc = read_skip_words(ctx, "trexhip_identify_skip3x_stats", w)) return rc;
    if (crops_windowed) *crops_windowed = w[SK3_USE] ? w[SK3X_CROPS] : 0u;
    if (windowed_passes) *windowed_passes = w[SK3_USE] ? w[SK3X_PASSES] : 0u;
    if (full_passes) *full_passes = w[SK3_USE] ? w[SK3_PASSES] : 0u;
    return TREXHIP_OK;
}

int trexhip_identify_skip3_stats(trexhip_ctx* ctx, uint32_t* pairs, uint32_t* listed, uint32_t* passes, uint64_t* bytes_filled) {
    uint32_t w[SK_WORDS];
    if (const int rc = read_skip_words(ctx, "trexhip_identify_skip3_stats", w)) return rc;
    if (pairs) *pairs = w[SK3_PAIRS];
    if (listed) *listed = w[SK3_LISTED];
    uint32_t by_rows = w[SK3_PASSES];
    if (passes && w[SK3_USE] && w[SK3X_PASSES]) {
        const Net* net = static_cast<Net*>(ctx->net);
        const int n = (int)(w[SK3_PAIRS] / Skip3Geom::PAIRS);
        std::vector<int2> bands((size_t)n);
        TH_CHECK_HIP(hipMemcpy(bands.data(), net->skip_bands, (size_t)n * sizeof(int2), hipMemcpyDeviceToHost));
        int count = 0;
        for (int c0 = 0; c0 < n; c0 += Skip3Geom::BLOCK) {
            Skip3Pass p{};
            for (int c = c0; c < n && c < c0 + Skip3Geom::BLOCK; ++c) {
                const SkipPairs r = skip3_pairs({bands[(size_t)c].x, bands[(size_t)c].y});
                if (r.lo <= r.hi) skip3_add_run(p, count, c * Skip3Geom::PAIRS + r.lo, r.hi - r.lo + 1, [](int, const Skip3Pass&) {});
            }
            skip3_flush(p, count, [](int, const Skip3Pass&) {});
        }
        by_rows = (uint32_t)count;
    }
    if (passes) *passes = w[SK3_USE] ? by_rows : 0u;
    if (bytes_filled) *bytes_filled = (uint64_t)w[SK3_FILLED] * (10 * 128 * 4);
    return TREXHIP_OK;
}

int trexhip_identify_fc1_stats(trexhip_ctx* ctx, uint32_t* rows, uint32_t* listed) {
    uint32_t w[SK_WORDS];
    if (const int rc = read_skip_words(ctx, "trexhip_identify_fc1_stats", w)) return rc;
    const Net* net = static_cast<Net*>(ctx->net);
    uint32_t sum = 0;
    for (int q = 0; q < Skip3Geom::PAIRS && net->last_fc1_n; ++q) sum += w[SK3_FC1_LEN + q];
    if (rows) *rows = (uint32_t)net->last_fc1_n * Skip3Geom::PAIRS;
    if (listed) *listed = sum;
    return TREXHIP_OK;
}

int trexhip_set_identity_precision(trexhip_ctx* ctx, int32_t mode) {
    if (!ctx || mode < 0 || mode > 3) { set_error("trexhip_set_identity_precision: mode must be one of TREXHIP_CNN_*"); return TREXHIP_E_INVALID; }
    ctx->cnn_mode = mode;
    ctx->prepared.precision_changed();
    return TREXHIP_OK;
}

int trexhip_num_classes(trexhip_ctx* ctx) {
    if (!ctx || !ctx->net) return 0;
    return static_cast<Net*>(ctx->net)->classes;
}

int trexhip_network_version(trexhip_ctx* ctx) {
    if (!ctx || !ctx->net) return 0;
    const Net* net = static_cast<const Net*>(ctx->net);
    return net->arch ? net->arch->plan.spec->id : TREXHIP_NET_V118_3;
}

size_t trexhip_network_blob_bytes(int32_t version, int32_t classes, int32_t channels, int32_t width, int32_t height) {
    return arch_blob_bytes(version, classes, channels, width, height);
}

int trexhip_identify_chunk_crops(trexhip_ctx* ctx, int32_t* crops) {
    if (!ctx || !crops) { set_error("trexhip_identify_chunk_crops: null argument"); return TREXHIP_E_INVALID; }
    const Net* net = static_cast<const Net*>(ctx->net);
    *crops = net && net->arch ? net->arch->plan.chunk : 0;
    return TREXHIP_OK;
}

int trexhip_network_channels(trexhip_ctx* ctx) {
    if (!ctx || !ctx->net) return 0;
    return static_cast<Net*>(ctx->net)->CH;
}

int trexhip_network_image_size(trexhip_ctx* ctx, int32_t* width, int32_t* height) {
    if (!ctx) { set_error("trexhip_network_image_size: null context"); return TREXHIP_E_INVALID; }
    const Net* net = static_cast<const Net*>(ctx->net);
    if (width) *width = net ? net->W : 0;
    if (height) *height = net ? net->H : 0;
    return TREXHIP_OK;
}

// ... 10 lines not shown
```

trex_amd/csrc/cnn_conv3p.h:

```cpp

template <bool LISTED, class L = Skip3Geom>
__global__ __launch_bounds__(256) void k_conv5_wpair(const uint8_t* __restrict__ v3, const uint4* __restrict__ wp ,
                                                     const float* __restrict__ bias, float* __restrict__ out, const float out_scale,
                                                     const int n_crops, uint32_t* __restrict__ pass_ctr,
                                                     const int n_big_dense ,
                                                     const int* __restrict__ desc ,
                                                     const uint32_t* __restrict__ rowsrc ,
                                                     const uint32_t* __restrict__ words ) {
    constexpr int CI = 64, CO = 128, S = 20, TPW = 2;
    constexpr int BD = 5;
    constexpr int AD = 1;
    constexpr int PK = 4;
    constexpr int DT0 = 2;
    using G = WinoGeom<CI, CO, S, TPW>;
    static_assert(G::NTHR == 256 && G::RP0 == 1280 && G::NCH * 2 * G::RP0 == V3_ROWB && G::NT == 4 && G::WM == 1, "geometry");
    static_assert(BD >= 1 && BD <= 7, "weight ring of 8 taps");
    extern __shared__ __attribute__((aligned(16))) uint8_t ldsb[];
    __shared__ int s_next_pass;
    const int tid = threadIdx.x, lane = tid & 63, wave = __builtin_amdgcn_readfirstlane(tid >> 6);
    const int j = lane & 31, h = lane >> 5;
    using LR = Skip3Reach;
    using P = Wino3Pass<L::TILES, L::NR>;
    constexpr bool WIN = L::TILES != G::TPR;
    static_assert(LISTED || !WIN, "only a listed pass has a window");
    static_assert(LR::ROWB == V3_ROWB && SkipGeom::V3_ROWS == S, "the images in front of V3 and behind it are S rows of V3_ROWB bytes");
    static_assert((WIN || (P::NR == G::NR && P::RP == G::RP && P::BUF == G::BUF)) && L::SLOTS * P::TPP <= G::MB && L::PAIRS * 2 == S, "a listed pass fits the dense pass's rows and tiles");
    if (words && (words[SK3_USE] != 0) != LISTED) return;
    const int total_tiles = n_crops * G::TPC;
    const int n_pass = LISTED ? __builtin_amdgcn_readfirstlane((int)words[WIN ? SK3X_PASSES : SK3_PASSES]) : (total_tiles + G::MB - 1) / G::MB;
    const int n_big = LISTED ? (n_pass >= 16 * (int)gridDim.x ? (int)((long long)n_pass * 7 / 8) / 4 : 0) : n_big_dense;
    const int big_end = n_big * PK;
    auto ticket_first = [&](const int t) { return t < n_big ? t * PK : big_end + (t - n_big); };
    int pass = ticket_first((int)blockIdx.x);
    if (pass >= n_pass) return;
    const uint32_t lds0 = (uint32_t)(uintptr_t)ldsb;
    constexpr int RNG = (2 * P::NR + 1) * P::RP, NI = (RNG + 1023) / 1024, NDW = (NI + 3) / 4;
    static_assert(DT0 + NDW <= 40 - BD, "the DMA instructions are older than the last 2 BD weight loads of a unit");
    static_assert(NI * 1024 - RNG <= 1024, "slack behind the second buffer");
    uint32_t dvo[NDW];
#pragma unroll
    for (int k = 0; k < NDW; ++k) {
        const int o = (wave + 4 * k) * 1024 + lane * 16;
        const int pc = o >= (P::NR + 1) * P::RP ? 1 : 0, q = o - pc * (P::NR + 1) * P::RP;
        const int row = q / P::RP, w = q - row * P::RP;
        const bool real = q < P::NR * P::RP && o < RNG;
        const int wv = WIN ? (w / P::PS) * G::PS + w % P::PS : w;
        const uint32_t inrow = (uint32_t)(pc * 1280 + (w < P::RP0 ? wv : G::RP0 - 16 - (WIN ? 2 * LR::TILEB : 0)));
        dvo[k] = LISTED ? (real ? (uint32_t)row << LR::ROW_SHIFT | inrow : (uint32_t)P::NR << LR::ROW_SHIFT)
                        : real ? (uint32_t)(row * V3_ROWB) + inrow : 0x80000000u;
    }
    const uint32_t mbase = (uint32_t)__builtin_amdgcn_readfirstlane((int)(lds0 + P::RP + wave * 1024));
    auto stage_rsrc = [&](const int g, const int qmin_, const int nrows_) {
        const unsigned long long base = wave_uniform64(reinterpret_cast<unsigned long long>(v3) + (unsigned long long)(long long)(qmin_ - (LISTED ? S : 0)) * V3_ROWB + (unsigned)(g * 2560));
        return __builtin_amdgcn_make_buffer_rsrc(reinterpret_cast<void*>(base), 0,
                                                 LISTED ? (int)(LR::NUM_RECORDS - (unsigned)(g * 2560)) : __builtin_amdgcn_readfirstlane(nrows_ * V3_ROWB - g * 2560), 0x00020000);
    };
#define P3_SRC(k_, tab_) (uint32_t)__builtin_amdgcn_ds_bpermute((int)(dvo[k_] >> (LR::ROW_SHIFT - 2)), (int)(tab_))
#define P3_DMA(k_, srs_, buf_, src_)                                                                                             \
    do {                                                                                                                         \
        if ((k_) < NDW - 1 || wave + 4 * (NDW - 1) < NI) {                                                                       \
            const uint32_t vo_ = LISTED ? dvo[k_] + (src_) : dvo[k_];                                                            \
            asm volatile("s_add_u32 m0, %0, %1\n\ts_nop 0\n\tbuffer_load_dwordx4 %2, %3, 0 offen lds"                          \
                         :: "s"(mbase), "n"((buf_) * P::BUF + (k_) * 4096), "v"(vo_), "s"(srs_) : "memory", "scc");               \
        }                                                                                                                        \
    } while (0)
    for (int i = tid; i < 4 * (P::RP / 16); i += G::NTHR) {
        const int pl = i / (P::RP / 16), o = i - pl * (P::RP / 16);
        *reinterpret_cast<uint4*>(ldsb + pl * P::PLANE + o * 16) = make_uint4(0, 0, 0, 0);
    }
    const __amdgpu_buffer_rsrc_t wrs = make_rsrc(wp, (uint32_t)(G::NCH * 40 * G::BV * 16));
    const int boff = (h * CO + wave * 32 + j) * 16;
    const int co = wave * 32 + j;
    const float bz = bias[co];
    const int ooff = (4 * h * CO + co) * 4;
    int lps[TPW], lr2[TPW];
#pragma unroll
    for (int m = 0; m < TPW; ++m) {
        const int t = m * 32 + j;
        lps[m] = t / P::TPP < L::SLOTS ? t / P::TPP : L::SLOTS - 1;
        lr2[m] = t % P::TPP;
    }
    int raw_w = 0, ent[TPW] = {};
    uint32_t tab = 0;
    auto pass_fetch = [&](const int pass_) {
        const int* d = desc + (size_t)pass_ * L::DESC;
        raw_w = d[lane & (L::DESC - 1)];
        tab = rowsrc[(size_t)pass_ * LR::WORDS + (lane & (LR::WORDS - 1))];
#pragma unroll
        for (int m = 0; m < TPW; ++m) ent[m] = d[S3_SLOT + lps[m]];
    };
    auto pass_decode = [&](int& qmin_, int& gp0_, int& span_, uint32_t (&rel_)[L::SLOTS]) {
        const int w = raw_w;
        qmin_ = __builtin_amdgcn_readlane((int)tab, LR::BASE);
        gp0_ = __builtin_amdgcn_readlane(w, S3_GP0);
        span_ = __builtin_amdgcn_readlane(w, S3_SPAN);
#pragma unroll
        for (int s2 = 0; s2 < L::SLOTS; ++s2) {
            const uint32_t e = (uint32_t)__builtin_amdgcn_readlane(w, S3_SLOT + s2), rp = e >> 16;
            rel_[s2] = rp == (uint32_t)S3_IDLE ? 0x80000000u
                     : rp * (uint32_t)(G::TPP * CO * 4) + (WIN ? ((e >> S3_T0_SHIFT) & S3_T0_MASK) * (uint32_t)(2 * CO * 4) : 0u);
        }
    };
    int qmin = 0, nrows = 0, gp0 = 0, span = 0;
    uint32_t rel[L::SLOTS] = {};
    if (LISTED) { pass_fetch(pass); pass_decode(qmin, gp0, span, rel); }
    else wino_pass_rows<G, S>(pass, total_tiles, qmin, nrows);
    const __amdgpu_buffer_rsrc_t srs0 = stage_rsrc(0, qmin, nrows);
#pragma unroll
    for (int k = 0; k < NDW; ++k) P3_DMA(k, srs0, 0, P3_SRC(k, tab));
    asm volatile("s_waitcnt vmcnt(0)" ::: "memory");
    __syncthreads();
    auto w_off = [](const int g, const int tt) {
        const int hp = tt & 1, p = g == 3 ? (hp ? 7 : 0) : 2 * g + 1 + hp;
        return ((tt / 10) * 40 + ((tt % 10) / 2) * 8 + p) * G::BV * 16;
    };
    uint4 bq[8][2];
#pragma unroll
    for (int t = 0; t < BD; ++t) {
        bq[t][0] = buf_load16(wrs, boff, w_off(0, t));
        bq[t][1] = buf_load16(wrs, boff, w_off(0, t) + 2 * CO * 16);
    }
    auto a_base = [&](const int pass_, const int qmin_, const int m, int& inr, int& zr, int& yy) {
        if (LISTED) {
            const int r2 = lr2[m], par = r2 & 1, e = ent[m];
            yy = 2 * ((e >> 8) & (WIN ? S3_Q_MASK : 0xff)) + par; zr = (r2 >> 1) * 32 + h * 16; inr = ((e & 0xff) + par) * P::RP + zr;
            return;
        }
        int T = pass_ * G::MB + m * 32 + j;
        if (T > total_tiles - 1) T = total_tiles - 1;
        const int gp = T / G::TPP, r2 = T - gp * G::TPP;
        const int tx = r2 >> 1, qo = 2 * gp + (r2 & 1);
        yy = qo % S; zr = tx * 32 + h * 16; inr = (qo - qmin_ + 1) * G::RP + zr;
    };
    auto a_offset = [&](const int inr, const int zr, const int yy, const int ky) {
        const int iy = yy + ky - 2;
        return (iy >= 0 && iy < S) ? inr + (ky - 2) * P::RP : zr;
    };
    int aoff[TPW][5];
#pragma unroll
    for (int m = 0; m < TPW; ++m) {
        int inr, zr, yy;
        a_base(pass, qmin, m, inr, zr, yy);
#pragma unroll
        for (int ky = 0; ky < 5; ++ky) aoff[m][ky] = a_offset(inr, zr, yy, ky);
    }
    int an_in[TPW] = {}, an_z[TPW] = {}, an_y[TPW] = {};
    auto P3_ACC = [](const float a) { float v; asm volatile("v_accvgpr_read_b32 %0, %1" : "=v"(v) : "a"(a)); return v; };
    const f32x16 zero16 = {0.f, 0.f, 0.f, 0.f, 0.f, 0.f, 0.f, 0.f, 0.f, 0.f, 0.f, 0.f, 0.f, 0.f, 0.f, 0.f};
    f32x16 acc[2][TPW][2];
    float y[TPW][4][16];
#pragma unroll
    for (int m = 0; m < TPW; ++m) {
#pragma unroll
        for (int k = 0; k < 4; ++k) {
            acc[k >> 1][m][k & 1] = zero16;
#pragma unroll
            for (int r = 0; r < 16; ++r) y[m][k][r] = 0.f;
        }
    }
#define P3_PIN(x_) asm volatile("" : "+v"(x_))
    __amdgpu_buffer_rsrc_t ors_prev = make_rsrc(out, 0);
    uint32_t rel_prev[L::SLOTS] = {};
    auto tail = [&](const __amdgpu_buffer_rsrc_t rs, const int m, const int rr) {
        const int r = 2 * rr, i = (r & 3) + 8 * (r >> 2);
        const float a0 = y[m][0][r] + P3_ACC(acc[1][m][0][r]), a1 = y[m][0][r + 1] + P3_ACC(acc[1][m][0][r + 1]);
        const float d0 = y[m][3][r] + P3_ACC(acc[1][m][1][r]), d1 = y[m][3][r + 1] + P3_ACC(acc[1][m][1][r + 1]);
        const float v0 = fmaxf(fmaxf(a0, y[m][1][r]), fmaxf(a1, y[m][1][r + 1]));
        const float v1 = fmaxf(fmaxf(y[m][2][r], d0), fmaxf(y[m][2][r + 1], d1));
        if (LISTED) {
            const int t0 = m * 32 + i, t1 = t0 + 4;
            const uint32_t o0 = rel_prev[t0 / P::TPP] + (uint32_t)((t0 % P::TPP) * CO * 4);
            const uint32_t o1 = t1 / P::TPP < L::SLOTS ? rel_prev[t1 / P::TPP < L::SLOTS ? t1 / P::TPP : 0] + (uint32_t)((t1 % P::TPP) * CO * 4) : 0x80000000u;
            const int vo = co * 4 + (int)(h ? o1 : o0);
            __builtin_amdgcn_raw_buffer_store_b32(__float_as_uint(fmaxf(v0 * out_scale + bz, 0.f)), rs, vo, 0, 2 );
            __builtin_amdgcn_raw_buffer_store_b32(__float_as_uint(fmaxf(v1 * out_scale + bz, 0.f)), rs, vo + CO * 4, 0, 2);
            return;
        }
        __builtin_amdgcn_raw_buffer_store_b32(__float_as_uint(fmaxf(v0 * out_scale + bz, 0.f)), rs, ooff, (m * 32 + i) * CO * 4, 2 );
        __builtin_amdgcn_raw_buffer_store_b32(__float_as_uint(fmaxf(v1 * out_scale + bz, 0.f)), rs, ooff, (m * 32 + i + 1) * CO * 4, 2);
    };
    auto fold = [&](const int g, const int m, const int r) {
        const float a = P3_ACC(acc[g & 1][m][0][r]), b = P3_ACC(acc[g & 1][m][1][r]);
        const float e = a + b, o = a - b;
        if (g == 0) { y[m][2][r] = e; y[m][1][r] = o; P3_PIN(y[m][2][r]); P3_PIN(y[m][1][r]); }
        if (g == 1) {
            const float e1 = y[m][2][r], o1 = y[m][1][r];
            y[m][0][r] = e1 + e; y[m][1][r] = o1 + 2.f * o; y[m][2][r] = e1 + 4.f * e; y[m][3][r] = o1 + 8.f * o;
        }
        if (g == 2) { y[m][0][r] += e; y[m][1][r] += 0.5f * o; y[m][2][r] += 0.25f * e; y[m][3][r] += 0.125f * o; }
        if (g >= 1) { P3_PIN(y[m][0][r]); P3_PIN(y[m][1][r]); P3_PIN(y[m][2][r]); P3_PIN(y[m][3][r]); }
    };
    for (;;) {
        const int tleft = total_tiles - pass * G::MB;
        const __amdgpu_buffer_rsrc_t ors = LISTED ? make_rsrc(out + (size_t)gp0 * (G::TPP * CO), (uint32_t)(span * (G::TPP * CO * 4)))
                                                  : make_rsrc(out + (size_t)(pass * G::MB) * CO, (uint32_t)((tleft < G::MB ? tleft : G::MB) * CO * 4));
        int next_pass = pass + 1;
        const bool draw = pass >= big_end || pass % PK == PK - 1;
        if (draw && tid == 0) s_next_pass = ticket_first((int)atomicAdd(pass_ctr, 1u) + (int)gridDim.x);
        bool have_next = false;
        int qmin_n = qmin, nrows_n = nrows, gp0_n = gp0, span_n = span;
        uint32_t rel_n[L::SLOTS];
#pragma unroll
        for (int s2 = 0; s2 < L::SLOTS; ++s2) rel_n[s2] = rel[s2];
#pragma clang loop unroll(full)
        for (int g = 0; g < 4; ++g) {
            const bool last_u = g == 3;
            if (!LISTED && last_u) {
                if (draw) next_pass = s_next_pass;
                have_next = next_pass < n_pass;
                if (have_next) wino_pass_rows<G, S>(next_pass, total_tiles, qmin_n, nrows_n);
            }
            if (LISTED && last_u) pass_decode(qmin_n, gp0_n, span_n, rel_n);
            const uint8_t* pbase = ldsb + (g & 1) * P::BUF;
            const int sg = last_u ? 0 : g + 1;
            const int sqmin = last_u ? qmin_n : qmin, snrows = last_u ? nrows_n : nrows;
            const __amdgpu_buffer_rsrc_t srs = stage_rsrc(sg, sqmin, snrows);
            uint32_t src_next = 0;
            uint4 af[AD + 1][TPW][2];
#pragma unroll
            for (int a = 0; a < AD; ++a)
#pragma unroll
                for (int m = 0; m < TPW; ++m) {
                    af[a][m][0] = *reinterpret_cast<const uint4*>(pbase + (a & 1) * P::PS + aoff[m][a / 2]);
                    af[a][m][1] = *reinterpret_cast<const uint4*>(pbase + (a & 1) * P::PS + aoff[m][a / 2] + P::PLANE);
                }
#pragma clang loop unroll(full)
            for (int tt = 0; tt < 40; ++tt) {
                const int cur = tt % (AD + 1), nxt = (tt + AD) % (AD + 1);
                const uint32_t src_cur = src_next;
                if (LISTED && tt + 1 >= DT0 && tt + 1 < DT0 + NDW) src_next = P3_SRC(tt + 1 - DT0, tab);
                if (tt + AD < 40) {
                    const uint8_t* an = pbase + (((tt + AD) / 10) * 2 + ((tt + AD) & 1)) * P::PS;
#pragma unroll
                    for (int m = 0; m < TPW; ++m) {
                        af[nxt][m][0] = *reinterpret_cast<const uint4*>(an + aoff[m][((tt + AD) % 10) / 2]);
                        af[nxt][m][1] = *reinterpret_cast<const uint4*>(an + aoff[m][((tt + AD) % 10) / 2] + P::PLANE);
                    }
                }
                const int wt = tt + BD < 40 ? w_off(g, tt + BD) : w_off(sg, tt + BD - 40);
                bq[(tt + BD) % 8][0] = buf_load16(wrs, boff, wt);
                bq[(tt + BD) % 8][1] = buf_load16(wrs, boff, wt + 2 * CO * 16);
                if (LISTED && g == 2 && tt == 34) {
                    if (draw) next_pass = s_next_pass;
                    have_next = next_pass < n_pass;
                    pass_fetch(have_next ? next_pass : pass);
                }
                if (tt >= DT0 && tt < DT0 + NDW) P3_DMA(tt - DT0, srs, (g & 1) ^ 1, src_cur);
                const int hp = tt & 1;
                const f16x8 b1 = __builtin_bit_cast(f16x8, bq[tt % 8][0]);
                const f16x8 b2 = __builtin_bit_cast(f16x8, bq[tt % 8][1]);
                f16x8 a1[TPW], a2[TPW];
#pragma unroll
                for (int m = 0; m < TPW; ++m) { a1[m] = __builtin_bit_cast(f16x8, af[cur][m][0]); a2[m] = __builtin_bit_cast(f16x8, af[cur][m][1]); }
#pragma unroll
                for (int m = 0; m < TPW; ++m) acc[g & 1][m][hp] = mfma16(a2[m], b1, tt < 2 ? zero16 : acc[g & 1][m][hp]);
#pragma unroll
                for (int m = 0; m < TPW; ++m) acc[g & 1][m][hp] = mfma16(a1[m], b2, acc[g & 1][m][hp]);
#pragma unroll
                for (int m = 0; m < TPW; ++m) acc[g & 1][m][hp] = mfma16(a1[m], b1, acc[g & 1][m][hp]);
                if (g == 0) {
                    if (tt >= 2 && tt < 34 && !(tt & 1)) tail(ors_prev, (tt - 2) / 16, ((tt - 2) / 2) % 8);
                } else if (tt >= 2 && tt < 34) {
                    fold(g - 1, (tt - 2) / 16, (tt - 2) % 16);
                }
                if (last_u && have_next && (tt == 28 || tt == 30)) a_base(next_pass, qmin_n, (tt - 28) / 2, an_in[(tt - 28) / 2], an_z[(tt - 28) / 2], an_y[(tt - 28) / 2]);
                if (last_u && have_next && (tt == 39 || (tt >= 32 && tt < 39 && !(tt & 1)))) {
                    const int ky = tt == 39 ? 4 : (tt - 32) / 2;
#pragma unroll
                    for (int m = 0; m < TPW; ++m) aoff[m][ky] = a_offset(an_in[m], an_z[m], an_y[m], ky);
                }
                __builtin_amdgcn_sched_group_barrier(0x100, 2 * TPW, 0);
                __builtin_amdgcn_sched_group_barrier(0x020, 10, 0);
#pragma unroll
                for (int k = 0; k < 3 * TPW; ++k) {
                    __builtin_amdgcn_sched_group_barrier(0x008, 1, 0);
                    __builtin_amdgcn_sched_group_barrier(0x246, 8, 0);
                }
                __builtin_amdgcn_sched_barrier(0);
            }
            asm volatile("s_waitcnt vmcnt(%0)" :: "n"(2 * BD) : "memory");
            __syncthreads();
        }
        ors_prev = ors;
#pragma unroll
        for (int s2 = 0; s2 < L::SLOTS; ++s2) { rel_prev[s2] = rel[s2]; rel[s2] = rel_n[s2]; }
        if (!have_next) break;
        pass = next_pass; qmin = qmin_n; nrows = nrows_n; gp0 = gp0_n; span = span_n;
    }
#pragma unroll
    for (int b = 0; b < 16; ++b) tail(ors_prev, b / 8, b % 8);
#undef P3_DMA
#undef P3_SRC
#undef P3_PIN
}
```

trex_amd/csrc/cnn_plan.h:

```cpp
#pragma once
#include <algorithm>
#include "../../include/trexhip.h"
#include "cnn_geom.h"
#include "cnn_skip_words.h"
#include "cnn_skipx.h"

namespace trexhip {

enum : int {
    GEOM_FP32_ACT = 0xfff,
    GEOM_NO_SKIP3X = 1 << 21,
    GEOM_NO_BGROWS = 1 << 22,
    GEOM_NO_SKIPX = 1 << 23,
    GEOM_DENSE_FC1 = 1 << 24,
    GEOM_V3_COPY = 1 << 25,
    GEOM_DENSE_CONV3 = 1 << 26,
    GEOM_NO_SKIP = 1 << 27,
    GEOM_TWO_KERNEL = 1 << 28,
    GEOM_ROLE_SPLIT = 1 << 29,
    GEOM_FUSED_2WG = 1 << 30,
    GEOM_MASK = GEOM_FP32_ACT | GEOM_NO_SKIP3X | GEOM_NO_BGROWS | GEOM_NO_SKIPX | GEOM_DENSE_FC1 | GEOM_V3_COPY | GEOM_DENSE_CONV3 | GEOM_NO_SKIP | GEOM_TWO_KERNEL | GEOM_ROLE_SPLIT | GEOM_FUSED_2WG
};

enum class Chain { ROLE_SPLIT, FUSED_2WG, TWO_KERNEL, FP32_ACT, EXACT, ANY_SIZE };
enum class Conv1 { FUSED , WPRE, MFMA, VALU, ANY };
enum class Fc1 { EXACT , SPLIT1 , SPLIT4  };
enum class Head { SMALL , BIG  };

struct Launch { int grid, items; };

struct CnnPlan {
    Chain chain;
    Conv1 conv1;
    int conv1_grid;
    Launch conv2, conv3;
    int pk2;
    int n_big3;
    Fc1 fc1;
    int fc1_grid, planes, K;
    Head head;
    int head_grid;
    bool rerun;
    bool head_plans;
    bool rerun_conv1;
    Launch r_conv2, r_conv3;
    int r_fc1_grid, r_head_grid;
    AnyTiles t2, t3;
    int tx1, t1;
    bool skip;
    bool skip3;
    int skip3_grid;
    Launch act3_fill;
    bool v3_direct;
    bool skip3x;
    bool fc1_listed;
    bool skipx;
    bool bgrows;
};

inline int ceil_div(const int a, const int b) { return (a + b - 1) / b; }
inline Launch whole(const int items) { return {items, items}; }
inline Launch guarded(const int items, const int n_cus) { return {std::min(items, 4 * n_cus), items}; }

inline CnnPlan cnn_plan(const int W, const int H, const int CH, const int mode, const bool aligned, const int geom, const int n, const int n_cus) {
    using GW = WinoGeom<64, 128, 20, 2>;
    CnnPlan p{};
    const bool h16 = mode == TREXHIP_CNN_FP16X3;
    const int P = (H / 8) * (W / 8);
    p.planes = FC1_KSPLIT;
    while (P % p.planes) --p.planes;
    p.K = 128 * P;
    p.fc1 = Fc1::EXACT;
    p.fc1_grid = p.r_fc1_grid = ceil_div(n, 32);
    p.head = Head::BIG;
    p.head_grid = p.r_head_grid = ceil_div(n, 4 * HEAD_CPW);
    p.rerun = h16;

    if (W != 80 || H != 80) {
        p.chain = Chain::ANY_SIZE;
        p.conv1 = Conv1::ANY;
        p.tx1 = ceil_div(W / 2, C1T);
        p.t1 = ceil_div(H / 2, C1T) * p.tx1;
        p.conv1_grid = n * p.t1;
        p.t2 = any_tiles(H / 4, W / 4);
        p.t3 = any_tiles(H / 8, W / 8);
        p.conv2 = whole(n * p.t2.tiles);
        p.conv3 = whole(n * p.t3.tiles);
        p.r_conv2 = guarded(p.conv2.items, n_cus);
        p.r_conv3 = guarded(p.conv3.items, n_cus);
        return p;
    }

    const bool pre = h16 && aligned && (geom & GEOM_FP32_ACT) == 0;
    const bool fused12 = pre && CH == 1 && !(geom & GEOM_TWO_KERNEL);
    const bool role_split = fused12 && !(geom & GEOM_FUSED_2WG) && ((geom & GEOM_ROLE_SPLIT) || n >= 3200);
    p.chain = role_split ? Chain::ROLE_SPLIT : fused12 ? Chain::FUSED_2WG : pre ? Chain::TWO_KERNEL : h16 ? Chain::FP32_ACT : Chain::EXACT;
    p.conv1 = fused12 ? Conv1::FUSED : pre ? Conv1::WPRE : aligned ? Conv1::MFMA : Conv1::VALU;
    p.conv1_grid = n;
    p.skip = role_split && !(geom & GEOM_NO_SKIP);
    p.skip3 = p.skip && !(geom & GEOM_DENSE_CONV3);
    p.skipx = p.skip && !(geom & GEOM_NO_SKIPX) && n < SKIPX_MAX_CROPS;
    p.bgrows = p.skipx && !(geom & GEOM_NO_BGROWS);
    if (p.skip3) {
        p.skip3_grid = ceil_div(ceil_div(n, 32 ), 256);
        p.act3_fill = {ceil_div(n, 16), n};
        p.v3_direct = !(geom & GEOM_V3_COPY) && skip3_direct_fits((long long)n * SkipGeom::V3_ROWS);
        p.skip3x = p.v3_direct && !(geom & GEOM_NO_SKIP3X) && skip3x_direct_fits((long long)n * SkipGeom::V3_ROWS);
    }

    const int n_pass2 = ceil_div(n * 20, W2bGeom::RPP), n_pass3 = ceil_div(n * GW::TPC, GW::MB);
    if (fused12) {
        const int wgs = role_split ? n_cus : 2 * n_cus;
        p.pk2 = std::max(1, std::min(role_split ? 32 : 16, n_pass2 / (wgs * 4)));
        p.conv2 = {std::min(ceil_div(n_pass2, p.pk2), wgs), n_pass2};
    }
    else if (pre) p.conv2 = {std::min(n_pass2, 2 * n_cus), n_pass2};
    else if (h16) p.conv2 = whole(n * ConvGeomS<16, 64, 40, 8, 4>::BPC);
    else if (mode == TREXHIP_CNN_FP32) p.conv2 = whole(n * ConvGeom<16, 64, 40, 20, 16>::BPC);
    else p.conv2 = whole(n * ConvGeomB<16, 64, 40, 10, SPLIT_NP>::BPC);
    if (pre) {
        p.n_big3 = n_pass3 >= 16 * n_cus ? (int)((long long)n_pass3 * 7 / 8) / 4 : 0;
        p.conv3 = {std::min(p.n_big3 + (n_pass3 - p.n_big3 * 4), n_cus), n_pass3};
    }
    else if (h16) p.conv3 = {std::min(n_pass3, n_cus), n_pass3};
    else if (mode == TREXHIP_CNN_FP32) p.conv3 = whole(n * ConvGeom<64, 128, 20, 20, 32>::BPC);
    else p.conv3 = whole(n * ConvGeomB<64, 128, 20, 20, SPLIT_NP>::BPC);

    const bool small = n <= 1024;
    if (h16) {
        p.fc1 = small ? Fc1::SPLIT1 : Fc1::SPLIT4;
        if (!small) p.fc1_grid = ceil_div(n, 128);
    }
    if (small) { p.head = Head::SMALL; p.head_grid = ceil_div(n, 4); }
    p.fc1_listed = p.skip3 && p.fc1 == Fc1::SPLIT4 && p.head == Head::BIG && !(geom & GEOM_DENSE_FC1);
    p.head_plans = h16 && small;
    p.rerun_conv1 = pre;
    p.r_conv2 = guarded(n * ConvGeomB<16, 64, 40, 10, SPLIT_NP>::BPC, n_cus);
    p.r_conv3 = guarded(n * ConvGeomB<64, 128, 20, 4, SPLIT_NP>::BPC, n_cus);
    return p;
}

}
```

trex_amd/csrc/cnn_skip3.h:

```cpp
#pragma once
#include "cnn_skip.h"

namespace trexhip {

constexpr bool S3X_DESC_OK(const int desc, const int slots) { return 8 + slots <= desc && (desc & (desc - 1)) == 0; }
struct Skip3Geom {
    static constexpr int PAIRS = SkipGeom::V3_ROWS / SkipGeom::POOL;
    static constexpr int SLOTS = 6;
    static constexpr int RUNS = 2;
    static constexpr int HALO = skip_layer_hi(0) - (SkipGeom::POOL - 1);
    static constexpr int NR = SkipGeom::POOL * SLOTS + 2 * HALO * RUNS;
    static constexpr int SPAN = 0xfff0;
    static constexpr int BLOCK = 32;
    static constexpr int BLOCK_PASSES = (BLOCK * PAIRS + SLOTS - 1) / SLOTS + BLOCK + 1;
    static constexpr int DESC = 16;
    static constexpr int TILES = SkipGeom::V3_ROWS / 4;
    static_assert(PAIRS == 10 && HALO == 2 && NR == 20, "pair q reads V3 rows 2q - 2 .. 2q + 3");
    static_assert((long long)(SPAN + SLOTS) * SkipGeom::POOL * 10240 < (1ll << 31), "V3 byte distance inside a pass");
};

struct Skip3XGeom {
    static constexpr int PAIRS = Skip3Geom::PAIRS, RUNS = Skip3Geom::RUNS, HALO = Skip3Geom::HALO, SPAN = Skip3Geom::SPAN, BLOCK = Skip3Geom::BLOCK;
    static constexpr int TILE = 4;
    static constexpr int ROW_TILES = SkipGeom::V3_ROWS / TILE;
// ... 65 lines not shown
}

enum : int { S3_ROW0 = 0, S3_NA = 1, S3_GAP = 2, S3_ROWS = 3, S3_GP0 = 4, S3_SPAN = 5, S3_SLOT = 8, S3_T0_SHIFT = 12, S3_Q_MASK = 0xf, S3_T0_MASK = 0x3 };
static constexpr int S3_IDLE = 0xffff;
template <class G = Skip3Geom>
TREXHIP_HD constexpr void skip3_describe(const Skip3Pass& p, int (&d)[G::DESC], const int t0a = 0, const int t0b = 0) {
    const bool two = p.runs > 1;
    const int la = p.len[0], lb = two ? p.len[1] : 0, ga = p.gp0[0], gb = two ? p.gp0[1] : ga + la;
    const Skip3Rows a = skip3_run_rows(ga, la);
    const Skip3Rows b = two ? skip3_run_rows(gb, lb) : Skip3Rows{a.row0 + a.n, 0};
    for (int i = 0; i < G::DESC; ++i) d[i] = 0;
    d[S3_ROW0] = a.row0; d[S3_NA] = a.n; d[S3_GAP] = b.row0 - (a.row0 + a.n); d[S3_ROWS] = a.n + b.n;
    d[S3_GP0] = ga; d[S3_SPAN] = (two ? gb + lb : ga + la) - ga;
    for (int s = 0; s < G::SLOTS; ++s) {
        const bool in_a = s < la, in_b = !in_a && s - la < lb;
        const int gp = in_a ? ga + s : gb + (s - la);
        const int slot = 1 + (in_a ? 0 : a.n) + SkipGeom::POOL * gp - (in_a ? a.row0 : b.row0);
        d[S3_SLOT + s] = in_a || in_b ? (gp - ga) << 16 | (in_a ? t0a : t0b) << S3_T0_SHIFT | (gp % G::PAIRS) << 8 | slot : S3_IDLE << 16 | 1;
    }
}

enum : int { S3_SRC_NONE = -1, S3_SRC_IMAGE = 1 << 30 };
template <class G = Skip3Geom>
TREXHIP_HD constexpr void skip3_row_sources(const Skip3Pass& p, const SkipRows own_a, const SkipRows own_b, int (&src)[G::NR]) {
    const bool two = p.runs > 1;
    const Skip3Rows a = skip3_run_rows(p.gp0[0], p.len[0]);
    const Skip3Rows b = two ? skip3_run_rows(p.gp0[1], p.len[1]) : Skip3Rows{a.row0 + a.n, 0};
    const int ca = p.gp0[0] / G::PAIRS, cb = two ? p.gp0[1] / G::PAIRS : ca;
    for (int i = 0; i < G::NR; ++i) {
        const bool in_a = i < a.n, in_b = !in_a && i - a.n < b.n;
        const int row = in_a ? a.row0 + i : b.row0 + (i - a.n);
        const int y = row - (in_a ? ca : cb) * SkipGeom::V3_ROWS;
        const SkipRows own = in_a ? own_a : own_b;
        src[i] = in_a || in_b ? (y >= own.lo && y <= own.hi ? row : S3_SRC_IMAGE | y) : S3_SRC_NONE;
    }
}

struct Skip3Reach {
    static constexpr int ROWB = 10240;
    static constexpr int WORDS = 32, BASE = 31, ROW_SHIFT = 18;
    static constexpr unsigned REACH = 0xF0000000u;
    static constexpr unsigned NUM_RECORDS = 0xF8000000u;
    static constexpr unsigned OFF_NONE = 0xFFFF0000u;
    static constexpr long long REACH_ROWS = REACH / ROWB;
    static constexpr int PASS_ROWS = (Skip3Geom::SPAN + Skip3Geom::SLOTS) * SkipGeom::POOL + 2 * Skip3Geom::HALO;
    static constexpr int PASS_ROWS_X = (Skip3XGeom::SPAN + Skip3XGeom::SLOTS) * SkipGeom::POOL + 2 * Skip3XGeom::HALO;
    static constexpr int TILEB = 32;
    static_assert(ROWB * 4 <= (1 << ROW_SHIFT) && Skip3Geom::NR < WORDS - 1 && (Skip3Geom::NR << ROW_SHIFT) > 0, "the packed constant");
    static_assert(Skip3XGeom::NR < WORDS - 1 && (Skip3XGeom::NR << ROW_SHIFT) > 0, "the packed constant, windowed passes");
    static_assert(NUM_RECORDS - 4 * 2560 >= REACH && OFF_NONE >= NUM_RECORDS, "none is out of range in every unit's resource");
};
TREXHIP_HD constexpr bool skip3_direct_fits(const long long total) {
    using R = Skip3Reach;
    return total <= 2 * R::REACH_ROWS - 2 * SkipGeom::V3_ROWS - R::PASS_ROWS - 1;
}
TREXHIP_HD constexpr bool skip3x_direct_fits(const long long total) {
    using R = Skip3Reach;
    return total <= 2 * R::REACH_ROWS - 2 * SkipGeom::V3_ROWS - R::PASS_ROWS_X - 1;
}
template <class G = Skip3Geom>
TREXHIP_HD constexpr void skip3_row_words(const Skip3Pass& p, const SkipRows own_a, const SkipRows own_b, const long long total,
                                          unsigned (&w)[Skip3Reach::WORDS], const int t0a = 0, const int t0b = 0) {
    using R = Skip3Reach;
    constexpr int IMG = SkipGeom::V3_ROWS;
    int src[G::NR] = {};
    skip3_row_sources<G>(p, own_a, own_b, src);
    const bool two = p.runs > 1;
    const Skip3Rows a = skip3_run_rows(p.gp0[0], p.len[0]);
    const Skip3Rows b = two ? skip3_run_rows(p.gp0[1], p.len[1]) : Skip3Rows{a.row0 + a.n, 0};
    const long long last = b.row0 + b.n - 1;
    bool image = false;
    for (int i = 0; i < G::NR; ++i) image = image || (src[i] != S3_SRC_NONE && (src[i] & S3_SRC_IMAGE));
    const bool front = image && IMG + last + 1 <= R::REACH_ROWS;
    const long long base = front ? 0 : IMG + a.row0, back = IMG + total;
    for (int i = 0; i < R::WORDS; ++i) {
        const int s = i < G::NR ? src[i < G::NR ? i : 0] : S3_SRC_NONE;
        const bool none = s == S3_SRC_NONE, img = !none && (s & S3_SRC_IMAGE);
        const long long row = img ? (front ? 0 : back) + (s & ~S3_SRC_IMAGE) : IMG + s;
        const unsigned off = none ? R::OFF_NONE : (unsigned)((row - base) * R::ROWB) + (unsigned)((i < a.n ? t0a : t0b) * R::TILEB);
        w[i] = i == R::BASE ? (unsigned)base : off - ((unsigned)i << R::ROW_SHIFT);
    }
}


static_assert(Skip3Geom::PAIRS == FC1_KSPLIT, "plane s of the split-K fc1 is row pair s");
TREXHIP_HD constexpr bool skip3_fc1_listed(const bool all, const SkipBand b, const int q) {
    if (all) return true;
    const SkipPairs r = skip3_pairs(b);
    return q >= r.lo && q <= r.hi;
}

static constexpr int SKIP3_FACTOR_NUM = 100, SKIP3_FACTOR_DEN = 100;
TREXHIP_HD constexpr bool skip3_use_list(const long long listed, const long long dense) {
    return listed * SKIP3_FACTOR_NUM < dense * SKIP3_FACTOR_DEN;
}

}
```

trex_amd/csrc/cnn_skip_kernels.h:

```cpp
#pragma once

static constexpr int SKIP_LB = 1024;
static constexpr int SKIP_PAD = 1;
static constexpr int SKIP_NCNT = 6;
static constexpr int SKIP_FILL_TB = 256;

__global__ __launch_bounds__(256) void k_crop_bands(const uint8_t* __restrict__ crops, const int n, int2* __restrict__ bands, int2* __restrict__ cols) {
    using G = SkipGeom;
    constexpr int UPR = 80 / 16, UNITS = G::CROP_ROWS * UPR;
    const int lane = threadIdx.x & 63, crop = blockIdx.x * 4 + (threadIdx.x >> 6);
    if (crop >= n) return;
    const uint4* src = reinterpret_cast<const uint4*>(crops + (size_t)crop * (G::CROP_ROWS * 80));
    uint4 px[(UNITS + 63) / 64];
#pragma unroll
    for (int k = 0; k < (UNITS + 63) / 64; ++k) {
        const int i = lane + 64 * k;
        px[k] = i < UNITS ? src[i] : make_uint4(0, 0, 0, 0);
    }
    int y0 = G::CROP_ROWS, y1 = -1;
#pragma unroll
    for (int k = 0; k < (UNITS + 63) / 64; ++k) {
        if (px[k].x | px[k].y | px[k].z | px[k].w) {
            const int row = (lane + 64 * k) / UPR;
            y0 = row < y0 ? row : y0;
// ... 99 lines not shown
    uint32_t part[SKIP_NCNT] = {0, 0, 0, 0, 0, 0};
    for (int b = tid; b < (int)blockIdx.x; b += SKIP_LB) {
#pragma unroll
        for (int k = 0; k < SKIP_NCNT; ++k) part[k] += counts[b * SKIP_NCNT + k];
    }
#pragma unroll
    for (int k = 0; k < SKIP_NCNT; ++k) {
#pragma unroll
        for (int d = 32; d >= 1; d >>= 1) part[k] += __shfl_xor(part[k], d);
        if (lane == 0 && part[k]) atomicAdd(&s_base[k], part[k]);
    }
    const SkipXItem it = skipx_item(i, n, bands, cols, words[SK_EMPTY_RANGE] != 0, bgrows != 0);
    uint32_t sc[2] = {it.full ? 1u : 0u, (uint32_t)it.wpasses};
#pragma unroll
    for (int k = 0; k < 2; ++k) {
#pragma unroll
        for (int d = 1; d < 64; d <<= 1) { const uint32_t v = __shfl_up(sc[k], d); if (lane >= d) sc[k] += v; }
        if (lane == 63) s_wave[k][wave] = sc[k];
    }
    __syncthreads();
#pragma unroll
    for (int k = 0; k < 2; ++k) {
        uint32_t before = 0;
        for (int w = 0; w < wave; ++w) before += s_wave[k][w];
        sc[k] += before;
    }
    if (it.full) list[s_base[0] + sc[0] - 1] = i;
    if (it.wpasses) {
        const uint32_t at = s_base[2] + sc[1] - (uint32_t)it.wpasses;
        for (int k = 0; k < it.wpasses; ++k) { wlist[at + k] = skipx_pack(skipx_pass(i, it.rows, it.t0, k)); wrows[at + k] = skipx_v2_pack(it.v2); }
    }
    if (blockIdx.x == gridDim.x - 1 && tid == SKIP_LB - 1) {
        const uint32_t full = s_base[0] + sc[0], wp = s_base[2] + sc[1];
        uint32_t need = s_base[1], wc = s_base[3];
        for (int k = 0; k < 2; ++k) { const uint32_t c = counts[blockIdx.x * SKIP_NCNT + 1 + 2 * k]; if (k) wc += c; else need += c; }
        for (int k = 0; k < SKIP_PAD; ++k) list[full + k] = n_pass;
        const bool last_need = skip_needed(n_pass - 1, total_pairs, bands, words[SK_EMPTY_RANGE] != 0);
        const uint32_t listed_rows = need * SkipGeom::RPP - (last_need ? (uint32_t)(n_pass * SkipGeom::RPP - total_pairs) : 0u);
        words[SK_LEN] = need; words[SK_NPASS] = (uint32_t)n_pass; words[SK_FILLED] = (uint32_t)total_pairs - listed_rows;
        if (cols) {
            for (int k = 0; k < SKIP_PAD; ++k) { wlist[wp + k] = 0; wrows[wp + k] = skipx_v2_pack(SKIPX_V2_ALL); }
            words[SKX_CROPS] = wc; words[SKX_PASSES] = wp; words[SKX_FULL] = full; words[SKX_CTR] = 0;
            words[SKX_V2_READ] = s_base[4] + counts[blockIdx.x * SKIP_NCNT + 4]; words[SKX_V2_MADE] = s_base[5] + counts[blockIdx.x * SKIP_NCNT + 5];
        }
    }
}
__global__ __launch_bounds__(SKIP_FILL_TB) void k_v3_fill(const int2* __restrict__ bands, const int2* __restrict__ cols, const int n, const uint32_t* __restrict__ words,
                                                          const uint4* __restrict__ v3e, uint4* __restrict__ v3, const int direct) {
    using G = SkipGeom;
    constexpr int ROWQ = V3_ROWB / 16;
    __shared__ unsigned long long s_fill[SKIP_FILL_TB / 64];
    if (direct && words[SK3_USE]) return;
    const bool all = words[SK_EMPTY_RANGE] != 0;
    const int total_pairs = n * G::V3_ROWS, tid = threadIdx.x, gp0 = blockIdx.x * SKIP_FILL_TB;
    {
        const int gp = gp0 + tid;
        bool fill = false;
        if (gp < total_pairs && !all) {
            const int crop = gp / G::V3_ROWS, r = gp - crop * G::V3_ROWS;
            if (!cols) fill = !skip_pass_needed(gp / G::RPP, total_pairs, SkipBandsOf{bands});
            else {
                const SkipXWinOf win{cols, all};
                bool computed = false;
                if (win(crop) >= 0) { const int2 b = bands[crop]; const SkipRows need = skip_rows({b.x, b.y}); computed = r >= need.lo && r <= need.hi; }
                fill = !computed && !skipx_full_needed(gp / G::RPP, total_pairs, SkipBandsOf{bands}, win);
            }
        }
        const unsigned long long m = __ballot(fill);
        if ((tid & 63) == 0) s_fill[tid >> 6] = m;
    }
    __syncthreads();
    for (int w = 0; w < SKIP_FILL_TB / 64; ++w) {
        unsigned long long m = s_fill[w];
        while (m) {
            const int gp = gp0 + w * 64 + __ffsll((long long)m) - 1;
            m &= m - 1;
            for (int q = tid; q < ROWQ; q += SKIP_FILL_TB) v3[(size_t)gp * ROWQ + q] = v3e[(gp % G::V3_ROWS) * ROWQ + q];
        }
    }
}

static constexpr int SKIP3_TB = 256;

static constexpr int SKIP3_NT = 2 * SKIP3_TB;
__device__ __forceinline__ void skip3_stage_runs(const int2* __restrict__ bands, const int2* __restrict__ cols, const int n, const bool all, uint16_t* s_run) {
    using G = Skip3Geom;
    const int c0 = blockIdx.x * SKIP3_TB * G::BLOCK;
    constexpr int U = 8;
    static_assert(G::BLOCK % U == 0 && (SKIP3_TB * G::BLOCK) % (U * SKIP3_NT) == 0, "whole groups of loads");
    for (int i0 = threadIdx.x; i0 < SKIP3_TB * G::BLOCK; i0 += U * SKIP3_NT) {
        int2 b[U], c[U];
#pragma unroll
        for (int u = 0; u < U; ++u) {
            const int i = i0 + u * SKIP3_NT;
            b[u] = c0 + i < n ? bands[c0 + i] : make_int2(SKIP_BAND_NONE.y0, SKIP_BAND_NONE.y1);
            c[u] = cols && c0 + i < n ? cols[c0 + i] : make_int2(SKIP_BAND_NONE.y0, SKIP_BAND_NONE.y1);
        }
#pragma unroll
        for (int u = 0; u < U; ++u) {
            const int i = i0 + u * SKIP3_NT;
            const SkipPairs r = all && c0 + i < n ? SkipPairs{0, G::PAIRS - 1} : skip3_pairs({b[u].x, b[u].y});
            const int t0 = skip3_window({c[u].x, c[u].y}, all);
            s_run[(i % G::BLOCK) * SKIP3_TB + i / G::BLOCK] = (uint16_t)(r.lo <= r.hi ? r.lo | (r.hi - r.lo + 1) << 8 | (t0 + 1) << 12 : 0);
        }
    }
    __syncthreads();
}
template <class G, class E>
__device__ __forceinline__ int skip3_walk(const uint16_t* s_run, const int t, const int blk, int& passes, int& crops, E&& emit) {
    constexpr bool WIN = G::TILES != Skip3Geom::TILES;
    Skip3Pass p{};
    int listed = 0;
#pragma unroll 1
    for (int k = 0; k < G::BLOCK; ++k) {
        const int r = s_run[k * SKIP3_TB + t], len = (r >> 8) & 0xf;
        if (len && ((r >> 12) != 0) == WIN) {
            listed += len;
            ++crops;
            skip3_add_run<G>(p, passes, (blk * G::BLOCK + k) * G::PAIRS + (r & 0xff), len, emit);
        }
    }
    skip3_flush(p, passes, emit);
    return listed;
}

__global__ __launch_bounds__(SKIP3_NT) void k_pair_count(const int2* __restrict__ bands, const int2* __restrict__ cols, const int n, const uint32_t* __restrict__ words,
                                                         uint4* __restrict__ counts ,
                                                         uint32_t* __restrict__ tcounts ) {
    __shared__ uint32_t s_pass, s_pair, s_wpass, s_wcrop;
    __shared__ uint16_t s_run[SKIP3_TB * Skip3Geom::BLOCK];
    if (threadIdx.x == 0) { s_pass = 0; s_pair = 0; s_wpass = 0; s_wcrop = 0; }
    skip3_stage_runs(bands, cols, n, words[SK_EMPTY_RANGE] != 0, s_run);
    const bool win = threadIdx.x >= SKIP3_TB;
    const int t = threadIdx.x & (SKIP3_TB - 1), blk = blockIdx.x * SKIP3_TB + t;
    if (blk * Skip3Geom::BLOCK < n) {
        int passes = 0, crops = 0, listed = 0;
        if (!win) listed = skip3_walk<Skip3Geom>(s_run, t, blk, passes, crops, [](int, const Skip3Pass&) {});
        else if (cols) listed = skip3_walk<Skip3XGeom>(s_run, t, blk, passes, crops, [](int, const Skip3Pass&) {});
        tcounts[2 * blk + (win ? 1 : 0)] = (uint32_t)passes;
        if (passes) atomicAdd(win ? &s_wpass : &s_pass, (uint32_t)passes);
        if (listed) atomicAdd(&s_pair, (uint32_t)listed);
        if (win && crops) atomicAdd(&s_wcrop, (uint32_t)crops);
    }
    __syncthreads();
    if (threadIdx.x == 0) counts[blockIdx.x] = make_uint4(s_pass, s_pair, s_wpass, s_wcrop);
}

__global__ __launch_bounds__(SKIP3_NT) void k_pair_list(const int2* __restrict__ bands, const int2* __restrict__ cols, const int n, uint32_t* __restrict__ words,
                                                        const uint4* __restrict__ counts, const uint32_t* __restrict__ tcounts, int* __restrict__ desc,
                                                        int* __restrict__ xdesc ) {
    using G = Skip3Geom;
    using X = Skip3XGeom;
    __shared__ uint2 s_scan[SKIP3_TB];
    __shared__ uint16_t s_run[SKIP3_TB * G::BLOCK];
    const int tid = threadIdx.x, t = tid & (SKIP3_TB - 1), blk = blockIdx.x * SKIP3_TB + t;
    const bool win = tid >= SKIP3_TB;
    const bool mine = blk * G::BLOCK < n;
    skip3_stage_runs(bands, cols, n, words[SK_EMPTY_RANGE] != 0, s_run);
    uint32_t before = 0, wbefore = 0, pairs = 0, wcrops = 0;
    for (int b = 0; b <= (int)blockIdx.x; ++b) {
        const uint4 c = counts[b];
        if (b < (int)blockIdx.x) { before += c.x; wbefore += c.z; }
        pairs += c.y; wcrops += c.w;
    }
    const uint2 cnt = mine ? make_uint2(tcounts[2 * blk], tcounts[2 * blk + 1]) : make_uint2(0, 0);
    if (!win) s_scan[t] = cnt;
    __syncthreads();
    for (int d = 1; d < SKIP3_TB; d <<= 1) {
        const uint2 v = !win && t >= d ? s_scan[t - d] : make_uint2(0, 0);
        __syncthreads();
        if (!win) { s_scan[t].x += v.x; s_scan[t].y += v.y; }
        __syncthreads();
    }
    int at = win ? (int)(wbefore + s_scan[t].y - cnt.y) : (int)(before + s_scan[t].x - cnt.x), crops = 0;
    if (mine && !win)
        skip3_walk<G>(s_run, t, blk, at, crops, [&](const int idx, const Skip3Pass& p) {
            *reinterpret_cast<int4*>(desc + (size_t)idx * G::DESC) = make_int4(p.gp0[0], p.len[0], p.gp0[1], p.runs > 1 ? p.len[1] : 0);
        });
    if (mine && win && cols)
        skip3_walk<X>(s_run, t, blk, at, crops, [&](const int idx, const Skip3Pass& p) {
            *reinterpret_cast<int4*>(xdesc + (size_t)idx * X::DESC) = make_int4(p.gp0[0], p.len[0], p.gp0[1], p.runs > 1 ? p.len[1] : 0);
        });
    if (blockIdx.x == gridDim.x - 1 && tid == SKIP3_TB - 1) {
        const uint32_t listed = before + s_scan[t].x, wlisted = wbefore + s_scan[t].y;
        const long long dense = ((long long)n * (G::PAIRS * 10) + 63) / 64;
        words[SK3_PAIRS] = (uint32_t)(n * G::PAIRS); words[SK3_LISTED] = pairs; words[SK3_PASSES] = listed; words[SK3_FILLED] = 0;
        words[SK3X_PASSES] = wlisted; words[SK3X_CROPS] = wcrops; words[SK3X_CTR] = 0;
        words[SK3_USE] = skip3_use_list((long long)listed + wlisted, dense) ? 1u : 0u;
    }
}

static constexpr int FC1L_TB = 1024, FC1L_SEG = FC1L_TB * 64;
__global__ __launch_bounds__(FC1L_TB) void k_fc1_list(const int2* __restrict__ bands, const int n, uint32_t* __restrict__ words,
                                                      int* __restrict__ list , const int stride) {
    constexpr int NW = FC1L_TB / 64, U = 8;
    __shared__ unsigned long long s_mask[FC1L_TB];
    __shared__ uint32_t s_off[FC1L_TB], s_wave[NW];
    const int tid = threadIdx.x, lane = tid & 63, wave = tid >> 6, q = blockIdx.x;
    const bool all = words[SK_EMPTY_RANGE] != 0;
    int* out = list + (size_t)q * stride;
    uint32_t base = 0;
    for (int seg0 = 0; seg0 < n; seg0 += FC1L_SEG) {
        const int left = n - seg0, nw = left >= FC1L_SEG ? FC1L_TB : (left + 63) / 64;
        for (int w0 = wave; w0 < nw; w0 += U * NW) {
            int2 b[U];
#pragma unroll
            for (int u = 0; u < U; ++u) {
                const int crop = seg0 + (w0 + u * NW) * 64 + lane;
                b[u] = w0 + u * NW < nw && crop < n ? bands[crop] : make_int2(SKIP_BAND_NONE.y0, SKIP_BAND_NONE.y1);
            }
#pragma unroll
            for (int u = 0; u < U; ++u) {
                const int crop = seg0 + (w0 + u * NW) * 64 + lane;
                const unsigned long long m = __ballot(crop < n && skip3_fc1_listed(all, {b[u].x, b[u].y}, q));
                if (lane == 0 && w0 + u * NW < nw) s_mask[w0 + u * NW] = m;
            }
        }
        __syncthreads();
        const uint32_t cnt = tid < nw ? (uint32_t)__popcll(s_mask[tid]) : 0u;
        uint32_t incl = cnt;
#pragma unroll
        for (int d = 1; d < 64; d <<= 1) { const uint32_t v = __shfl_up(incl, d); if (lane >= d) incl += v; }
        if (lane == 63) s_wave[wave] = incl;
        __syncthreads();
        uint32_t before = base, total = base;
        for (int w = 0; w < NW; ++w) { const uint32_t c = s_wave[w]; if (w < wave) before += c; total += c; }
        s_off[tid] = before + incl - cnt;
        __syncthreads();
        for (int w = wave; w < nw; w += NW) {
            const unsigned long long m = s_mask[w];
            if ((m >> lane) & 1ull) out[s_off[w] + (uint32_t)__popcll(m & ((1ull << lane) - 1ull))] = seg0 + w * 64 + lane;
        }
        base = total;
        __syncthreads();
    }
    if (tid == 0) words[SK3_FC1_LEN + q] = base;
}

static constexpr int SKIP3_FC = 16;
__global__ __launch_bounds__(256) void k_act3_fill(const int2* __restrict__ bands, const int2* __restrict__ cols, const int n, uint32_t* __restrict__ words,
                                                   const uint4* __restrict__ act3e, uint4* __restrict__ act3, int* __restrict__ desc,
                                                   uint32_t* __restrict__ rows ,
                                                   int* __restrict__ xdesc, uint32_t* __restrict__ xrows,
                                                   const long long alloc_rows , const int direct,
                                                   const int copy ) {
    using G = Skip3Geom;
    constexpr int PQ = 10 * 128 * 4 / 16;
    using X = Skip3XGeom;
    constexpr int CQ = 128 * 4 / 16;
    static_assert((Skip3Geom::BLOCK_PASSES + X::BLOCK_PASSES) * SKIP3_FC <= Skip3Geom::BLOCK * 256 && SKIP3_FC % 4 == 0, "a thread per pass of either list: 256 threads per SKIP3_FC crops");
    __shared__ uint32_t s_filled;
    const int lane = threadIdx.x & 63;
    if (!words[SK3_USE]) return;
    if (threadIdx.x == 0) s_filled = 0;
    __syncthreads();
    const bool all = words[SK_EMPTY_RANGE] != 0;
    const int gid = blockIdx.x * 256 + threadIdx.x;
    const int n_full = (int)words[SK3_PASSES], n_win = cols ? (int)words[SK3X_PASSES] : 0;
    const SkipRows every{0, SkipGeom::V3_ROWS - 1};
    const bool from_v3 = all || !direct;
    if (gid >= n_full && gid - n_full < n_win) {
        int4* dst = reinterpret_cast<int4*>(xdesc + (size_t)(gid - n_full) * X::DESC);
        const int4 r = dst[0];
        Skip3Pass p{};
        p.runs = r.w ? 2 : 1; p.n = r.y + r.w;
        p.gp0[0] = r.x; p.len[0] = r.y; p.gp0[1] = r.z; p.len[1] = r.w;
        const int ca = r.x / X::PAIRS, cb = (r.w ? r.z : r.x) / X::PAIRS;
        const int2 xa = cols[ca], xb = cols[cb];
        const int t0a = skip3_window({xa.x, xa.y}, all), t0b = skip3_window({xb.x, xb.y}, all);
        int d[X::DESC];
        skip3_describe<X>(p, d, t0a, t0b);
#pragma unroll
        for (int k = 0; k < X::DESC / 4; ++k) dst[k] = make_int4(d[4 * k], d[4 * k + 1], d[4 * k + 2], d[4 * k + 3]);
        const int2 ba = bands[ca], bb = bands[cb];
        unsigned w[Skip3Reach::WORDS];
        skip3_row_words<X>(p, from_v3 ? every : skip_rows({ba.x, ba.y}), from_v3 ? every : skip_rows({bb.x, bb.y}), alloc_rows, w, t0a, t0b);
        uint4* wd = reinterpret_cast<uint4*>(xrows + (size_t)(gid - n_full) * Skip3Reach::WORDS);
#pragma unroll
        for (int k = 0; k < Skip3Reach::WORDS / 4; ++k) wd[k] = make_uint4(w[4 * k], w[4 * k + 1], w[4 * k + 2], w[4 * k + 3]);
    }
    if (gid < n_full) {
        int4* dst = reinterpret_cast<int4*>(desc + (size_t)gid * G::DESC);
        const int4 r = dst[0];
        Skip3Pass p{};
        p.runs = r.w ? 2 : 1; p.n = r.y + r.w;
        p.gp0[0] = r.x; p.len[0] = r.y; p.gp0[1] = r.z; p.len[1] = r.w;
        int d[G::DESC];
        skip3_describe(p, d);
#pragma unroll
        for (int k = 0; k < G::DESC / 4; ++k) dst[k] = make_int4(d[4 * k], d[4 * k + 1], d[4 * k + 2], d[4 * k + 3]);
        const int2 ba = bands[r.x / G::PAIRS], bb = bands[(r.w ? r.z : r.x) / G::PAIRS];
        unsigned w[Skip3Reach::WORDS];
        skip3_row_words(p, from_v3 ? every : skip_rows({ba.x, ba.y}), from_v3 ? every : skip_rows({bb.x, bb.y}), alloc_rows, w);
        uint4* wd = reinterpret_cast<uint4*>(rows + (size_t)gid * Skip3Reach::WORDS);
#pragma unroll
        for (int k = 0; k < Skip3Reach::WORDS / 4; ++k) wd[k] = make_uint4(w[4 * k], w[4 * k + 1], w[4 * k + 2], w[4 * k + 3]);
    }
    uint32_t filled = 0;
    for (int k = 0; k < SKIP3_FC / 4; ++k) {
        const int crop = blockIdx.x * SKIP3_FC + (threadIdx.x >> 6) * (SKIP3_FC / 4) + k;
        if (crop >= n) break;
        const int2 b = bands[crop];
        const SkipPairs r = all ? SkipPairs{0, G::PAIRS - 1} : skip3_pairs({b.x, b.y});
        const int2 c = cols ? cols[crop] : make_int2(SKIP_BAND_NONE.y0, SKIP_BAND_NONE.y1);
        const int t0 = skip3_window({c.x, c.y}, all);
        for (int q = 0; q < G::PAIRS; ++q) {
            if (q >= r.lo && q <= r.hi) {
                if (t0 >= 0) {
                    constexpr int OUT = (10 - 2 * X::WT3) * CQ;
                    for (int i = lane; i < OUT; i += 64) {
                        const int u = i < 2 * t0 * CQ ? i : i + 2 * X::WT3 * CQ;
                        act3[((size_t)crop * G::PAIRS + q) * PQ + u] = act3e[q * PQ + u];
                    }
                }
                continue;
            }
            ++filled;
            if (!copy) continue;
#pragma unroll
            for (int i = lane; i < PQ; i += 64) act3[((size_t)crop * G::PAIRS + q) * PQ + i] = act3e[q * PQ + i];
        }
    }
    if (lane == 0 && filled) atomicAdd(&s_filled, filled);
    __syncthreads();
    if (threadIdx.x == 0 && s_filled) atomicAdd(&words[SK3_FILLED], s_filled);
}
```

trex_amd/csrc/cnn_skip_words.h:

```cpp
#pragma once
#include "cnn_skip3.h"

namespace trexhip {

enum : int {
    SK_EMPTY_RANGE = 0,
    SK_EMPTY_CTR = 1,
    SK_LEN = 2,
    SK_NPASS = 3,
    SK_FILLED = 4,
    SK3X_CROPS = 5,
    SK3X_PASSES = 6,
    SK3X_CTR = 7,
    SK3_PAIRS = 8,
    SK3_LISTED = 9,
    SK3_PASSES = 10,
    SK3_FILLED = 11,
    SK3_USE = 12,
    SK3_EMPTY_CTR = 13,
    SK3_FC1E_RANGE = 14,
    SK3_FC1_LEN = 16,
    SK3_LAST = SK3_FC1_LEN + Skip3Geom::PAIRS - 1,
    SKX_CROPS = 26,
    SKX_PASSES = 27,
    SKX_FULL = 28,
    SKX_CTR = 29,
    SKX_V2_READ = 30,
    SKX_V2_MADE = 31,
    SK_WORDS = 32
};
static_assert(SK_FILLED < SK3X_CROPS && SK3X_CTR < SK3_PAIRS && SK3_LAST < SKX_CROPS && SKX_V2_MADE < SK_WORDS, "no word twice, the last one inside the table");

}
```

Before: 47180.

## Add tiled pair-pass lists for the skip-listed conv3 Winograd pass

Adds a tiled variant of the conv3 pair-list scheme. The pass descriptors carry a tile count and per-pass row words, so each listed pass packs tiles from several pair slots instead of a fixed slot-per-pair layout. New count, list and fill kernels and conv3 kernel instantiations are chosen when the plan enables skip3t and the buffers fit. Separate 'ran' counters record how many passes are launched, apart from the logical pass counts. The aim is to pack listed conv3 work more densely and launch fewer passes. The cost is more descriptor decoding, an extra counter word and larger buffer allocations.

After: 49040, median of 6. +3.9%, better.

```diff
diff --git a/include/trexhip.h b/include/trexhip.h
--- a/include/trexhip.h
+++ b/include/trexhip.h
@@ -6,7 +6,7 @@
 extern "C" {
 #endif
 
-#define TREXHIP_ABI_VERSION 26
+#define TREXHIP_ABI_VERSION 27
 
 enum {
     TREXHIP_OK = 0,
@@ -269,6 +269,8 @@
 int trexhip_identify_skip3_stats(trexhip_ctx* ctx, uint32_t* pairs, uint32_t* listed, uint32_t* passes, uint64_t* bytes_filled);
 
 int trexhip_identify_skip3x_stats(trexhip_ctx* ctx, uint32_t* crops_windowed, uint32_t* windowed_passes, uint32_t* full_passes);
+
+int trexhip_identify_skip3_ran(trexhip_ctx* ctx, uint32_t* windowed_passes, uint32_t* full_passes);
 
 int trexhip_identify_skipx_stats(trexhip_ctx* ctx, uint32_t* crops_windowed, uint32_t* windowed_passes, uint32_t* full_passes);
 
diff --git a/trex_amd/capi.py b/trex_amd/capi.py
--- a/trex_amd/capi.py
+++ b/trex_amd/capi.py
@@ -180,7 +180,7 @@
     "trexhip_set_stream", "trexhip_get_live_params", "trexhip_update_params", "trexhip_set_background", "trexhip_set_background_device", "trexhip_set_background_color", "trexhip_set_background_color_device", "trexhip_generate_average_device", "trexhip_get_background", "trexhip_segment_device",
     "trexhip_segment", "trexhip_segment_color", "trexhip_segment_color_device", "trexhip_rethreshold_device", "trexhip_rethreshold_per_blob_device", "trexhip_fetch_rethreshold", "trexhip_fetch", "trexhip_device_view_get", "trexhip_synchronize",
     "trexhip_profile_enable", "trexhip_profile_read", "trexhip_profile_reset",
-    "trexhip_default_posture_params", "trexhip_posture_device", "trexhip_posture_auto_device", "trexhip_pack_frames_v6_device", "trexhip_crops_device", "trexhip_pixel_channels", "trexhip_device_alloc", "trexhip_device_free", "trexhip_copy_to_host", "trexhip_copy_to_device", "trexhip_crops_transformed_device", "trexhip_crops_posture_device", "trexhip_default_midline_params", "trexhip_midline_device", "trexhip_midline_movement_device", "trexhip_default_split_params", "trexhip_split_search_device", "trexhip_export_id_table_device", "trexhip_export_id_table_ex_device", "trexhip_load_weights", "trexhip_set_identity_precision", "trexhip_num_classes", "trexhip_identify_device", "trexhip_identify", "trexhip_identify_guard_stats", "trexhip_identify_skip_stats", "trexhip_identify_skip3_stats", "trexhip_identify_skip3x_stats", "trexhip_identify_skipx_stats", "trexhip_identify_bgrow_stats", "trexhip_identify_fc1_stats",
+    "trexhip_default_posture_params", "trexhip_posture_device", "trexhip_posture_auto_device", "trexhip_pack_frames_v6_device", "trexhip_crops_device", "trexhip_pixel_channels", "trexhip_device_alloc", "trexhip_device_free", "trexhip_copy_to_host", "trexhip_copy_to_device", "trexhip_crops_transformed_device", "trexhip_crops_posture_device", "trexhip_default_midline_params", "trexhip_midline_device", "trexhip_midline_movement_device", "trexhip_default_split_params", "trexhip_split_search_device", "trexhip_export_id_table_device", "trexhip_export_id_table_ex_device", "trexhip_load_weights", "trexhip_set_identity_precision", "trexhip_num_classes", "trexhip_identify_device", "trexhip_identify", "trexhip_identify_guard_stats", "trexhip_identify_skip_stats", "trexhip_identify_skip3_stats", "trexhip_identify_skip3x_stats", "trexhip_identify_skip3_ran", "trexhip_identify_skipx_stats", "trexhip_identify_bgrow_stats", "trexhip_identify_fc1_stats",
     "trexhip_weight_blob_bytes", "trexhip_trainer_create", "trexhip_trainer_destroy", "trexhip_trainer_set_lr", "trexhip_trainer_steps", "trexhip_trainer_image_size", "trexhip_trainer_version", "trexhip_trainer_keep_mask_bytes", "trexhip_train_step_device", "trexhip_train_step", "trexhip_train_eval_device", "trexhip_train_eval", "trexhip_trainer_read", "trexhip_trainer_export",
     "trexhip_default_augment_params", "trexhip_augment_device",
     "trexhip_train_predict_device", "trexhip_validation_metrics_device", "trexhip_class_averages_device",
@@ -279,6 +279,7 @@
         L.trexhip_identify_skipx_stats.argtypes = [C.c_void_p, C.POINTER(C.c_uint32), C.POINTER(C.c_uint32), C.POINTER(C.c_uint32)]
         L.trexhip_identify_bgrow_stats.argtypes = [C.c_void_p, C.POINTER(C.c_uint32), C.POINTER(C.c_uint32)]
         L.trexhip_identify_skip3x_stats.argtypes = [C.c_void_p, C.POINTER(C.c_uint32), C.POINTER(C.c_uint32), C.POINTER(C.c_uint32)]
+        L.trexhip_identify_skip3_ran.argtypes = [C.c_void_p, C.POINTER(C.c_uint32), C.POINTER(C.c_uint32)]
         L.trexhip_identify_skip3_stats.argtypes = [C.c_void_p, C.POINTER(C.c_uint32), C.POINTER(C.c_uint32), C.POINTER(C.c_uint32), C.POINTER(C.c_uint64)]
         L.trexhip_identify_fc1_stats.argtypes = [C.c_void_p, C.POINTER(C.c_uint32), C.POINTER(C.c_uint32)]
         L.trexhip_weight_blob_bytes.argtypes = [C.c_int32, C.c_int32]
@@ -668,6 +669,11 @@
         _check(lib().trexhip_identify_skip3x_stats(self._h, C.byref(a), C.byref(b), C.byref(c)))
         return int(a.value), int(b.value), int(c.value)
 
+    def skip3_ran(self):
+        a, b = C.c_uint32(0), C.c_uint32(0)
+        _check(lib().trexhip_identify_skip3_ran(self._h, C.byref(a), C.byref(b)))
+        return int(a.value), int(b.value)
+
     def fc1_stats(self):
         a, b = C.c_uint32(0), C.c_uint32(0)
         _check(lib().trexhip_identify_fc1_stats(self._h, C.byref(a), C.byref(b)))
diff --git a/trex_amd/csrc/cnn.hip b/trex_amd/csrc/cnn.hip
--- a/trex_amd/csrc/cnn.hip
+++ b/trex_amd/csrc/cnn.hip
@@ -1275,12 +1275,14 @@
         TRY(B.device_bytes(&net->skipx_list, (N * skipx_passes({0, SkipGeom::V3_ROWS - 1}) + SKIP_PAD) * 4, who));
         TRY(B.device_bytes(&net->skipx_rows, (N * skipx_passes({0, SkipGeom::V3_ROWS - 1}) + SKIP_PAD) * 4, who));
         const size_t blocks3 = (N + Skip3Geom::BLOCK - 1) / Skip3Geom::BLOCK;
-        TRY(B.device_bytes(&net->skip3_counts, ((blocks3 + SKIP3_TB - 1) / SKIP3_TB) * sizeof(uint4), who));
+        constexpr size_t BP3 = std::max(Skip3Geom::BLOCK_PASSES, Skip3TGeom::BLOCK_PASSES), BP3X = std::max(Skip3XGeom::BLOCK_PASSES, Skip3TXGeom::BLOCK_PASSES);
+        static_assert(Skip3Geom::DESC == Skip3TGeom::DESC && Skip3XGeom::DESC == Skip3TXGeom::DESC, "one descriptor size per list");
+        TRY(B.device_bytes(&net->skip3_counts, 2 * ((blocks3 + SKIP3_TB - 1) / SKIP3_TB) * sizeof(uint4), who));
         TRY(B.device_bytes(&net->skip3_tcounts, blocks3 * 2 * sizeof(uint32_t), who));
-        TRY(B.device_bytes(&net->skip3_desc, blocks3 * Skip3Geom::BLOCK_PASSES * Skip3Geom::DESC * 4, who));
-        TRY(B.device_bytes(&net->skip3_rows, blocks3 * Skip3Geom::BLOCK_PASSES * Skip3Reach::WORDS * 4, who));
-        TRY(B.device_bytes(&net->skip3x_desc, blocks3 * Skip3XGeom::BLOCK_PASSES * Skip3XGeom::DESC * 4, who));
-        TRY(B.device_bytes(&net->skip3x_rows, blocks3 * Skip3XGeom::BLOCK_PASSES * Skip3Reach::WORDS * 4, who));
+        TRY(B.device_bytes(&net->skip3_desc, blocks3 * BP3 * Skip3Geom::DESC * 4, who));
+        TRY(B.device_bytes(&net->skip3_rows, blocks3 * BP3 * Skip3Reach::WORDS * 4, who));
+        TRY(B.device_bytes(&net->skip3x_desc, blocks3 * BP3X * Skip3XGeom::DESC * 4, who));
+        TRY(B.device_bytes(&net->skip3x_rows, blocks3 * BP3X * std::max(Skip3Reach::WORDS, Skip3TXGeom::ROW_WORDS) * 4, who));
         TRY(B.device_bytes(&net->fc1_list, Skip3Geom::PAIRS * N * sizeof(int), who));
     }
     TRY(B.device_bytes(&net->crops, N * net->W * net->H * net->CH, who));
@@ -1312,9 +1314,13 @@
 static const Kern K_CONV3_WPAIR_LIST(k_conv5_wpair<true>, 256, GW3::LDS_BYTES + 1024);
 using GW3X = Wino3Pass<Skip3XGeom::TILES, Skip3XGeom::NR>;
 static const Kern K_CONV3_WPAIR_LISTX(k_conv5_wpair<true, Skip3XGeom>, 256, GW3X::LDS_BYTES + 1024);
-static const Kern K_PAIR_COUNT(k_pair_count, SKIP3_NT);
-static const Kern K_PAIR_LIST(k_pair_list, SKIP3_NT);
-static const Kern K_ACT3_FILL(k_act3_fill, 256);
+using GW3T = Wino3Pass<Skip3TGeom::TILES, Skip3TGeom::NR>;
+using GW3TX = Wino3Pass<Skip3TXGeom::TILES, Skip3TXGeom::NR>;
+static const Kern K_CONV3_WPAIR_TLIST(k_conv5_wpair<true, Skip3TGeom>, 256, GW3T::LDS_BYTES + 1024);
+static const Kern K_CONV3_WPAIR_TLISTX(k_conv5_wpair<true, Skip3TXGeom>, 256, GW3TX::LDS_BYTES + 1024);
+static const Kern K_PAIR_COUNT(k_pair_count<false>, SKIP3_NT), K_PAIR_COUNT_T(k_pair_count<true>, SKIP3_NT_TILED);
+static const Kern K_PAIR_LIST(k_pair_list<false>, SKIP3_NT), K_PAIR_LIST_T(k_pair_list<true>, SKIP3_NT);
+static const Kern K_ACT3_FILL(k_act3_fill<false>, 256), K_ACT3_FILL_T(k_act3_fill<true>, 256);
 template <int CI, int CO, int S, int ROWS, int NTERMS>
 static auto split_kern() { return Kern(k_conv5_split<CI, CO, S, ROWS, NTERMS>, 512, ConvGeomB<CI, CO, S, ROWS, SPLIT_NP>::LDS_BYTES); }
 struct ExactLayer { decltype(Kern(k_conv5<16, 64, 40, 20, 16>, 512)) f32; decltype(split_kern<16, 64, 40, 10, 6>()) x6, x3, x6_plan; };
@@ -1427,13 +1433,13 @@
     return TREXHIP_OK;
 }
 
-struct PrepArgs { long long alloc_rows; bool direct, x3 ; };
+struct PrepArgs { long long alloc_rows; bool direct, x3 , tiled ; };
 static PrepArgs prep_args(const Net& net, const CnnPlan& p) {
     const long long alloc_rows = (long long)net.max_crops * SkipGeom::V3_ROWS;
     const bool direct = p.v3_direct && skip3_direct_fits(alloc_rows);
-    return {alloc_rows, direct, p.skip3x && direct && skip3x_direct_fits(alloc_rows)};
-}
-static void launch_skip_prep(const Pass& f, const bool direct, const bool x3) {
+    return {alloc_rows, direct, p.skip3x && direct && skip3x_direct_fits(alloc_rows), p.skip3t && skip3t_direct_fits(alloc_rows)};
+}
+static void launch_skip_prep(const Pass& f, const bool direct, const bool x3, const bool tiled) {
     const Net& net = f.net;
     const CnnPlan& p = f.p;
     const int n = f.n, lb = ceil_div(p.conv2.items, SKIP_LB);
@@ -1443,8 +1449,8 @@
     K_PASS_LIST(f.s, lb, net.skip_bands, cols, n, net.d_skip, net.skip_counts, net.skip_list, net.skipx_list, net.skipx_rows, (int)p.bgrows);
     if (p.skip3) {
         const int2* cols3 = x3 ? net.skipx_cols : nullptr;
-        K_PAIR_COUNT(f.s, p.skip3_grid, net.skip_bands, cols3, n, net.d_skip, net.skip3_counts, net.skip3_tcounts);
-        K_PAIR_LIST(f.s, p.skip3_grid, net.skip_bands, cols3, n, net.d_skip, net.skip3_counts, net.skip3_tcounts, net.skip3_desc, net.skip3x_desc);
+        (tiled ? K_PAIR_COUNT_T : K_PAIR_COUNT)(f.s, p.skip3_grid, net.skip_bands, cols3, n, net.d_skip, net.skip3_counts, net.skip3_tcounts);
+        (tiled ? K_PAIR_LIST_T : K_PAIR_LIST)(f.s, p.skip3_grid, net.skip_bands, cols3, n, net.d_skip, net.skip3_counts, net.skip3_tcounts, net.skip3_desc, net.skip3x_desc);
         if (p.fc1_listed) K_FC1_LIST(f.s, Skip3Geom::PAIRS, net.skip_bands, n, net.d_skip, net.fc1_list, net.max_crops);
     }
     K_V3_FILL(f.s, ceil_div(n * SkipGeom::V3_ROWS, SKIP_FILL_TB), net.skip_bands, cols, n, net.d_skip, reinterpret_cast<const uint4*>(net.v3e),
@@ -1458,9 +1464,9 @@
     const CnnPlan& p = f.p;
     if (!plan_prepares(p)) return;
     const PrepArgs a = prep_args(net, p);
-    if (parts & PREP_LISTS) launch_skip_prep(f, a.direct, a.x3);
+    if (parts & PREP_LISTS) launch_skip_prep(f, a.direct, a.x3, a.tiled);
     if ((parts & PREP_ACT3) && p.skip3)
-        K_ACT3_FILL(f.s, p.act3_fill.grid, net.skip_bands, a.x3 ? net.skipx_cols : nullptr, f.n, net.d_skip, reinterpret_cast<const uint4*>(net.act3e),
+        (a.tiled ? K_ACT3_FILL_T : K_ACT3_FILL)(f.s, p.act3_fill.grid, net.skip_bands, a.x3 ? net.skipx_cols : nullptr, f.n, net.d_skip, reinterpret_cast<const uint4*>(net.act3e),
                     reinterpret_cast<uint4*>(net.act3), net.skip3_desc, net.skip3_rows, net.skip3x_desc, net.skip3x_rows, a.alloc_rows, (int)a.direct, (int)!p.fc1_listed);
 }
 
@@ -1478,7 +1484,7 @@
     const CnnPlan p = cnn_plan(net.W, net.H, net.CH, ctx->cnn_mode, (reinterpret_cast<uintptr_t>(d_crops) & 15) == 0, ctx->tune_conv_geom, n, ctx->n_cus);
     const Pass f{net, p, ctx->stream, ctx->cnn_mode, d_crops, n, d_probs, d_logits};
     hipStream_t s = f.s;
-    const bool x3 = prep_args(net, p).x3;
+    const bool x3 = prep_args(net, p).x3, tiled = prep_args(net, p).tiled;
     stage_begin(ctx, TREXHIP_STAGE_CNN_ALL);
     launch_conv1(f, p.conv1, nullptr);
     if (p.chain == Chain::ANY_SIZE) {
@@ -1514,8 +1520,8 @@
             if (p.skip3) {
                 if (!prepared) launch_prep(f, PREP_ACT3);
                 if (x3)
-                    K_CONV3_WPAIR_LISTX(s, p.conv3.grid, net.v3, net.w3w, net.b3, net.act3, net.inv3w, n, net.d_skip + SK3X_CTR, 0, net.skip3x_desc, net.skip3x_rows, net.d_skip);
-                K_CONV3_WPAIR_LIST(s, p.conv3.grid, net.v3, net.w3w, net.b3, net.act3, net.inv3w, n, net.ovf(OVF_PASS3), 0, net.skip3_desc, net.skip3_rows, net.d_skip);
+                    (tiled ? K_CONV3_WPAIR_TLISTX : K_CONV3_WPAIR_LISTX)(s, p.conv3.grid, net.v3, net.w3w, net.b3, net.act3, net.inv3w, n, net.d_skip + SK3X_CTR, 0, net.skip3x_desc, net.skip3x_rows, net.d_skip);
+                (tiled ? K_CONV3_WPAIR_TLIST : K_CONV3_WPAIR_LIST)(s, p.conv3.grid, net.v3, net.w3w, net.b3, net.act3, net.inv3w, n, net.ovf(OVF_PASS3), 0, net.skip3_desc, net.skip3_rows, net.d_skip);
             }
             K_CONV3_WPAIR(s, p.conv3.grid, net.v3, net.w3w, net.b3, net.act3, net.inv3w, n, net.ovf(OVF_PASS3), p.n_big3, nullptr, nullptr, p.skip3 ? net.d_skip : nullptr);
         }
@@ -1732,6 +1738,14 @@
     if (crops_windowed) *crops_windowed = w[SK3_USE] ? w[SK3X_CROPS] : 0u;
     if (windowed_passes) *windowed_passes = w[SK3_USE] ? w[SK3X_PASSES] : 0u;
     if (full_passes) *full_passes = w[SK3_USE] ? w[SK3_PASSES] : 0u;
+    return TREXHIP_OK;
+}
+
+int trexhip_identify_skip3_ran(trexhip_ctx* ctx, uint32_t* windowed_passes, uint32_t* full_passes) {
+    uint32_t w[SK_WORDS];
+    if (const int rc = read_skip_words(ctx, "trexhip_identify_skip3_ran", w)) return rc;
+    if (windowed_passes) *windowed_passes = w[SK3_USE] ? w[SK3X_RAN] : 0u;
+    if (full_passes) *full_passes = w[SK3_USE] ? w[SK3_RAN] : 0u;
     return TREXHIP_OK;
 }
 
diff --git a/trex_amd/csrc/cnn_conv3p.h b/trex_amd/csrc/cnn_conv3p.h
--- a/trex_amd/csrc/cnn_conv3p.h
+++ b/trex_amd/csrc/cnn_conv3p.h
@@ -22,12 +22,15 @@
     using LR = Skip3Reach;
     using P = Wino3Pass<L::TILES, L::NR>;
     constexpr bool WIN = L::TILES != G::TPR;
-    static_assert(LISTED || !WIN, "only a listed pass has a window");
+    constexpr bool TS = Skip3Tiled<L>::value;
+    constexpr int RW = Skip3Tiled<L>::ROW_WORDS;
+    static_assert(LISTED || (!WIN && !TS), "only a listed pass has a window or tile slots");
     static_assert(LR::ROWB == V3_ROWB && SkipGeom::V3_ROWS == S, "the images in front of V3 and behind it are S rows of V3_ROWB bytes");
-    static_assert((WIN || (P::NR == G::NR && P::RP == G::RP && P::BUF == G::BUF)) && L::SLOTS * P::TPP <= G::MB && L::PAIRS * 2 == S, "a listed pass fits the dense pass's rows and tiles");
+    static_assert((WIN || TS || (P::NR == G::NR && P::RP == G::RP && P::BUF == G::BUF)) && (TS || L::SLOTS * P::TPP <= G::MB) && L::PAIRS * 2 == S, "a listed pass fits the dense pass's rows and tiles");
+    static_assert(!TS || (P::TPP - 2 + G::MB - 1) / P::TPP < L::SLOTS, "tile slots: every lane's pair slot is one of the descriptor's");
     if (words && (words[SK3_USE] != 0) != LISTED) return;
     const int total_tiles = n_crops * G::TPC;
-    const int n_pass = LISTED ? __builtin_amdgcn_readfirstlane((int)words[WIN ? SK3X_PASSES : SK3_PASSES]) : (total_tiles + G::MB - 1) / G::MB;
+    const int n_pass = LISTED ? __builtin_amdgcn_readfirstlane((int)words[WIN ? SK3X_RAN : SK3_RAN]) : (total_tiles + G::MB - 1) / G::MB;
     const int n_big = LISTED ? (n_pass >= 16 * (int)gridDim.x ? (int)((long long)n_pass * 7 / 8) / 4 : 0) : n_big_dense;
     const int big_end = n_big * PK;
     auto ticket_first = [&](const int t) { return t < n_big ? t * PK : big_end + (t - n_big); };
@@ -85,15 +88,17 @@
     auto pass_fetch = [&](const int pass_) {
         const int* d = desc + (size_t)pass_ * L::DESC;
         raw_w = d[lane & (L::DESC - 1)];
-        tab = rowsrc[(size_t)pass_ * LR::WORDS + (lane & (LR::WORDS - 1))];
+        tab = rowsrc[(size_t)pass_ * RW + (lane & (RW - 1))];
+        if (TS) return;
 #pragma unroll
         for (int m = 0; m < TPW; ++m) ent[m] = d[S3_SLOT + lps[m]];
     };
-    auto pass_decode = [&](int& qmin_, int& gp0_, int& span_, uint32_t (&rel_)[L::SLOTS]) {
+    auto pass_decode = [&](int& qmin_, int& gp0_, int& span_, uint32_t (&rel_)[L::SLOTS], int& tiles_) {
         const int w = raw_w;
-        qmin_ = __builtin_amdgcn_readlane((int)tab, LR::BASE);
+        qmin_ = __builtin_amdgcn_readlane((int)tab, RW - 1);
         gp0_ = __builtin_amdgcn_readlane(w, S3_GP0);
         span_ = __builtin_amdgcn_readlane(w, S3_SPAN);
+        if (TS) { tiles_ = __builtin_amdgcn_readlane(w, S3_TILES); return; }
 #pragma unroll
         for (int s2 = 0; s2 < L::SLOTS; ++s2) {
             const uint32_t e = (uint32_t)__builtin_amdgcn_readlane(w, S3_SLOT + s2), rp = e >> 16;
@@ -101,9 +106,9 @@
                      : rp * (uint32_t)(G::TPP * CO * 4) + (WIN ? ((e >> S3_T0_SHIFT) & S3_T0_MASK) * (uint32_t)(2 * CO * 4) : 0u);
         }
     };
-    int qmin = 0, nrows = 0, gp0 = 0, span = 0;
+    int qmin = 0, nrows = 0, gp0 = 0, span = 0, tiles = 0;
     uint32_t rel[L::SLOTS] = {};
-    if (LISTED) { pass_fetch(pass); pass_decode(qmin, gp0, span, rel); }
+    if (LISTED) { pass_fetch(pass); pass_decode(qmin, gp0, span, rel, tiles); }
     else wino_pass_rows<G, S>(pass, total_tiles, qmin, nrows);
     const __amdgpu_buffer_rsrc_t srs0 = stage_rsrc(0, qmin, nrows);
 #pragma unroll
@@ -120,7 +125,21 @@
         bq[t][0] = buf_load16(wrs, boff, w_off(0, t));
         bq[t][1] = buf_load16(wrs, boff, w_off(0, t) + 2 * CO * 16);
     }
-    auto a_base = [&](const int pass_, const int qmin_, const int m, int& inr, int& zr, int& yy) {
+    uint32_t toff[TPW] = {};
+    auto a_base = [&](const int pass_, const int qmin_, const int tiles_, const int m, int& inr, int& zr, int& yy) {
+        if (TS) {
+            constexpr int MUL = P::TPP == 10 ? 205 : 171, SH = P::TPP == 10 ? 11 : 10;
+            static_assert(P::TPP == 10 || P::TPP == 6, "the division by multiplication");
+            const int o = tiles_ & S3_O_MASK, cnt = tiles_ >> S3_COUNT_SHIFT, t = m * 32 + j;
+            const int x = o + t, slot = (x * MUL) >> SH, r2 = x - slot * P::TPP, par = r2 & 1;
+            const int e = __builtin_amdgcn_ds_bpermute((S3_SLOT + slot) * 4, raw_w);
+            yy = 2 * ((e >> 8) & S3_Q_MASK) + par; zr = (r2 >> 1) * 32 + h * 16; inr = ((e & 0xff) + par) * P::RP + zr;
+            const uint32_t rp = (uint32_t)e >> 16;
+            toff[m] = t < cnt && rp != (uint32_t)S3_IDLE
+                    ? rp * (uint32_t)(G::TPP * CO * 4) + (uint32_t)(r2 * CO * 4) + (WIN ? ((e >> S3_T0_SHIFT) & S3_T0_MASK) * (uint32_t)(2 * CO * 4) : 0u)
+                    : 0x80000000u;
+            return;
+        }
         if (LISTED) {
             const int r2 = lr2[m], par = r2 & 1, e = ent[m];
             yy = 2 * ((e >> 8) & (WIN ? S3_Q_MASK : 0xff)) + par; zr = (r2 >> 1) * 32 + h * 16; inr = ((e & 0xff) + par) * P::RP + zr;
@@ -140,11 +159,12 @@
 #pragma unroll
     for (int m = 0; m < TPW; ++m) {
         int inr, zr, yy;
-        a_base(pass, qmin, m, inr, zr, yy);
+        a_base(pass, qmin, tiles, m, inr, zr, yy);
 #pragma unroll
         for (int ky = 0; ky < 5; ++ky) aoff[m][ky] = a_offset(inr, zr, yy, ky);
     }
     int an_in[TPW] = {}, an_z[TPW] = {}, an_y[TPW] = {};
+    uint32_t otab = h ? toff[1] : toff[0], otab_prev = 0x80000000u;
     auto P3_ACC = [](const float a) { float v; asm volatile("v_accvgpr_read_b32 %0, %1" : "=v"(v) : "a"(a)); return v; };
     const f32x16 zero16 = {0.f, 0.f, 0.f, 0.f, 0.f, 0.f, 0.f, 0.f, 0.f, 0.f, 0.f, 0.f, 0.f, 0.f, 0.f, 0.f};
     f32x16 acc[2][TPW][2];
@@ -167,6 +187,14 @@
         const float d0 = y[m][3][r] + P3_ACC(acc[1][m][1][r]), d1 = y[m][3][r + 1] + P3_ACC(acc[1][m][1][r + 1]);
         const float v0 = fmaxf(fmaxf(a0, y[m][1][r]), fmaxf(a1, y[m][1][r + 1]));
         const float v1 = fmaxf(fmaxf(y[m][2][r], d0), fmaxf(y[m][2][r + 1], d1));
+        if (TS) {
+            const int t0 = m * 32 + i;
+            const uint32_t o0 = (uint32_t)__builtin_amdgcn_readlane((int)otab_prev, t0), o1 = (uint32_t)__builtin_amdgcn_readlane((int)otab_prev, t0 + 4);
+            const int vo = co * 4 + (int)(h ? o1 : o0);
+            __builtin_amdgcn_raw_buffer_store_b32(__float_as_uint(fmaxf(v0 * out_scale + bz, 0.f)), rs, vo, 0, 2 );
+            __builtin_amdgcn_raw_buffer_store_b32(__float_as_uint(fmaxf(v1 * out_scale + bz, 0.f)), rs, vo + CO * 4, 0, 2);
+            return;
+        }
         if (LISTED) {
             const int t0 = m * 32 + i, t1 = t0 + 4;
             const uint32_t o0 = rel_prev[t0 / P::TPP] + (uint32_t)((t0 % P::TPP) * CO * 4);
@@ -198,7 +226,8 @@
         const bool draw = pass >= big_end || pass % PK == PK - 1;
         if (draw && tid == 0) s_next_pass = ticket_first((int)atomicAdd(pass_ctr, 1u) + (int)gridDim.x);
         bool have_next = false;
-        int qmin_n = qmin, nrows_n = nrows, gp0_n = gp0, span_n = span;
+        int qmin_n = qmin, nrows_n = nrows, gp0_n = gp0, span_n = span, tiles_n = tiles;
+        uint32_t otab_n = otab;
         uint32_t rel_n[L::SLOTS];
 #pragma unroll
         for (int s2 = 0; s2 < L::SLOTS; ++s2) rel_n[s2] = rel[s2];
@@ -210,7 +239,7 @@
                 have_next = next_pass < n_pass;
                 if (have_next) wino_pass_rows<G, S>(next_pass, total_tiles, qmin_n, nrows_n);
             }
-            if (LISTED && last_u) pass_decode(qmin_n, gp0_n, span_n, rel_n);
+            if (LISTED && last_u) pass_decode(qmin_n, gp0_n, span_n, rel_n, tiles_n);
             const uint8_t* pbase = ldsb + (g & 1) * P::BUF;
             const int sg = last_u ? 0 : g + 1;
             const int sqmin = last_u ? qmin_n : qmin, snrows = last_u ? nrows_n : nrows;
@@ -263,7 +292,8 @@
                 } else if (tt >= 2 && tt < 34) {
                     fold(g - 1, (tt - 2) / 16, (tt - 2) % 16);
                 }
-                if (last_u && have_next && (tt == 28 || tt == 30)) a_base(next_pass, qmin_n, (tt - 28) / 2, an_in[(tt - 28) / 2], an_z[(tt - 28) / 2], an_y[(tt - 28) / 2]);
+                if (last_u && have_next && (tt == 28 || tt == 30)) a_base(next_pass, qmin_n, tiles_n, (tt - 28) / 2, an_in[(tt - 28) / 2], an_z[(tt - 28) / 2], an_y[(tt - 28) / 2]);
+                if (TS && last_u && have_next && tt == 31) otab_n = h ? toff[1] : toff[0];
                 if (last_u && have_next && (tt == 39 || (tt >= 32 && tt < 39 && !(tt & 1)))) {
                     const int ky = tt == 39 ? 4 : (tt - 32) / 2;
 #pragma unroll
@@ -282,10 +312,11 @@
             __syncthreads();
         }
         ors_prev = ors;
+        otab_prev = otab; otab = otab_n;
 #pragma unroll
         for (int s2 = 0; s2 < L::SLOTS; ++s2) { rel_prev[s2] = rel[s2]; rel[s2] = rel_n[s2]; }
         if (!have_next) break;
-        pass = next_pass; qmin = qmin_n; nrows = nrows_n; gp0 = gp0_n; span = span_n;
+        pass = next_pass; qmin = qmin_n; nrows = nrows_n; gp0 = gp0_n; span = span_n; tiles = tiles_n;
     }
 #pragma unroll
     for (int b = 0; b < 16; ++b) tail(ors_prev, b / 8, b % 8);
diff --git a/trex_amd/csrc/cnn_plan.h b/trex_amd/csrc/cnn_plan.h
--- a/trex_amd/csrc/cnn_plan.h
+++ b/trex_amd/csrc/cnn_plan.h
@@ -9,6 +9,7 @@
 
 enum : int {
     GEOM_FP32_ACT = 0xfff,
+    GEOM_PAIR_SLOTS = 1 << 20,
     GEOM_NO_SKIP3X = 1 << 21,
     GEOM_NO_BGROWS = 1 << 22,
     GEOM_NO_SKIPX = 1 << 23,
@@ -19,7 +20,7 @@
     GEOM_TWO_KERNEL = 1 << 28,
     GEOM_ROLE_SPLIT = 1 << 29,
     GEOM_FUSED_2WG = 1 << 30,
-    GEOM_MASK = GEOM_FP32_ACT | GEOM_NO_SKIP3X | GEOM_NO_BGROWS | GEOM_NO_SKIPX | GEOM_DENSE_FC1 | GEOM_V3_COPY | GEOM_DENSE_CONV3 | GEOM_NO_SKIP | GEOM_TWO_KERNEL | GEOM_ROLE_SPLIT | GEOM_FUSED_2WG
+    GEOM_MASK = GEOM_FP32_ACT | GEOM_PAIR_SLOTS | GEOM_NO_SKIP3X | GEOM_NO_BGROWS | GEOM_NO_SKIPX | GEOM_DENSE_FC1 | GEOM_V3_COPY | GEOM_DENSE_CONV3 | GEOM_NO_SKIP | GEOM_TWO_KERNEL | GEOM_ROLE_SPLIT | GEOM_FUSED_2WG
 };
 
 enum class Chain { ROLE_SPLIT, FUSED_2WG, TWO_KERNEL, FP32_ACT, EXACT, ANY_SIZE };
@@ -53,6 +54,7 @@
     Launch act3_fill;
     bool v3_direct;
     bool skip3x;
+    bool skip3t;
     bool fc1_listed;
     bool skipx;
     bool bgrows;
@@ -106,6 +108,7 @@
         p.act3_fill = {ceil_div(n, 16), n};
         p.v3_direct = !(geom & GEOM_V3_COPY) && skip3_direct_fits((long long)n * SkipGeom::V3_ROWS);
         p.skip3x = p.v3_direct && !(geom & GEOM_NO_SKIP3X) && skip3x_direct_fits((long long)n * SkipGeom::V3_ROWS);
+        p.skip3t = !(geom & GEOM_PAIR_SLOTS) && skip3t_direct_fits((long long)n * SkipGeom::V3_ROWS);
     }
 
     const int n_pass2 = ceil_div(n * 20, W2bGeom::RPP), n_pass3 = ceil_div(n * GW::TPC, GW::MB);
diff --git a/trex_amd/csrc/cnn_skip3.h b/trex_amd/csrc/cnn_skip3.h
--- a/trex_amd/csrc/cnn_skip3.h
+++ b/trex_amd/csrc/cnn_skip3.h
@@ -171,6 +171,105 @@
     }
 }
 
+struct Skip3TGeom {
+    static constexpr int PAIRS = Skip3Geom::PAIRS, RUNS = Skip3Geom::RUNS, HALO = Skip3Geom::HALO, SPAN = Skip3Geom::SPAN, BLOCK = Skip3Geom::BLOCK;
+    static constexpr int TILES = Skip3Geom::TILES, TPP = 2 * TILES;
+    static constexpr int MB = 64;
+    static constexpr int MAXP = (TPP - 2 + MB + TPP - 1) / TPP;
+    static constexpr int SLOTS = MAXP;
+    static constexpr int NR = SkipGeom::POOL * MAXP + 2 * HALO * RUNS;
+    static constexpr int BLOCK_PASSES = (BLOCK * PAIRS * TPP + MB - 1) / MB + BLOCK + 1;
+    static constexpr int DESC = 16;
+    static constexpr int ROW_WORDS = 32;
+    static_assert(MAXP == 8 && NR == 24 && S3X_DESC_OK(DESC, SLOTS), "2 + 60 + 2 tiles: 8 pairs, and the descriptor holds their slots");
+    static_assert((long long)(SPAN + SLOTS) * SkipGeom::POOL * 10240 < (1ll << 31), "V3 byte distance inside a pass");
+};
+struct Skip3TXGeom {
+    static constexpr int PAIRS = Skip3Geom::PAIRS, RUNS = Skip3Geom::RUNS, HALO = Skip3Geom::HALO, SPAN = Skip3Geom::SPAN, BLOCK = Skip3Geom::BLOCK;
+    static constexpr int WT3 = Skip3XGeom::WT3, TILES = WT3, TPP = 2 * TILES;
+    static constexpr int MB = 64;
+    static constexpr int MAXP = (TPP - 2 + MB + TPP - 1) / TPP;
+    static constexpr int SLOTS = MAXP;
+    static constexpr int NR = SkipGeom::POOL * MAXP + 2 * HALO * RUNS;
+    static constexpr int ROW_WORDS = 64;
+    static constexpr int BLOCK_PASSES = (BLOCK * PAIRS * TPP + MB - 1) / MB + BLOCK + 1;
+    static constexpr int DESC = 32;
+    static_assert(MAXP == 12 && NR == 32 && NR < ROW_WORDS - 1, "12 pairs, and the row table holds their rows and `none`");
+    static_assert(S3X_DESC_OK(DESC, SLOTS), "the descriptor holds the slots");
+    static_assert((long long)(SPAN + SLOTS) * SkipGeom::POOL * 10240 < (1ll << 31), "V3 byte distance inside a pass");
+};
+template <class G> struct Skip3Tiled { static constexpr bool value = false; static constexpr int ROW_WORDS = 32 ; };
+template <> struct Skip3Tiled<Skip3TGeom> { static constexpr bool value = true; static constexpr int ROW_WORDS = Skip3TGeom::ROW_WORDS; };
+template <> struct Skip3Tiled<Skip3TXGeom> { static constexpr bool value = true; static constexpr int ROW_WORDS = Skip3TXGeom::ROW_WORDS; };
+
+struct Skip3TPass { int n, runs, o, gp0[Skip3Geom::RUNS], len[Skip3Geom::RUNS]; };
+
+template <class T>
+TREXHIP_HD constexpr int skip3t_room(const Skip3TPass& p, const int off) {
+    const int touched = p.runs ? p.len[0] : 0;
+    const int by_pairs = (T::MAXP - touched) * T::TPP - off, by_tiles = T::MB - p.n;
+    return by_pairs < by_tiles ? by_pairs : by_tiles;
+}
+template <class T, class E>
+TREXHIP_HD constexpr void skip3t_add_run(Skip3TPass& p, int& passes, int gp, const int len, E&& emit) {
+    int left = len * T::TPP, off = 0;
+    while (left > 0) {
+        if (p.runs && (skip3t_room<T>(p, off) <= 0 || p.runs == T::RUNS || gp - p.gp0[0] > T::SPAN)) { emit(passes, p); ++passes; p = Skip3TPass{}; }
+        const int room = skip3t_room<T>(p, off), take = left < room ? left : room;
+        const int touch = (off + take + T::TPP - 1) / T::TPP;
+        if (p.runs == 0) { p.o = off; p.gp0[0] = gp; p.len[0] = touch; }
+        else { p.gp0[1] = gp; p.len[1] = touch; }
+        ++p.runs; p.n += take; left -= take;
+        off += take; gp += off / T::TPP; off %= T::TPP;
+        if (left > 0) { emit(passes, p); ++passes; p = Skip3TPass{}; }
+    }
+}
+template <class E>
+TREXHIP_HD constexpr void skip3t_flush(Skip3TPass& p, int& passes, E&& emit) {
+    if (p.n) { emit(passes, p); ++passes; p = Skip3TPass{}; }
+}
+TREXHIP_HD constexpr Skip3Pass skip3t_pairs(const Skip3TPass& p) {
+    Skip3Pass r{};
+    r.runs = p.runs; r.gp0[0] = p.gp0[0]; r.len[0] = p.len[0];
+    r.gp0[1] = p.runs > 1 ? p.gp0[1] : 0; r.len[1] = p.runs > 1 ? p.len[1] : 0;
+    r.n = r.len[0] + r.len[1];
+    return r;
+}
+enum : int { S3_TILES = 6, S3_O_MASK = 0xff, S3_COUNT_SHIFT = 8 };
+template <class T>
+TREXHIP_HD constexpr void skip3t_describe(const Skip3TPass& p, int (&d)[T::DESC], const int t0a = 0, const int t0b = 0) {
+    skip3_describe<T>(skip3t_pairs(p), d, t0a, t0b);
+    d[S3_TILES] = p.o | p.n << S3_COUNT_SHIFT;
+}
+template <class T>
+TREXHIP_HD constexpr void skip3t_row_words(const Skip3Pass& p , const SkipRows own_a, const SkipRows own_b, const long long total,
+                                           unsigned (&w)[T::ROW_WORDS], const int t0a = 0, const int t0b = 0) {
+    using R = Skip3Reach;
+    constexpr int IMG = SkipGeom::V3_ROWS, BASE = T::ROW_WORDS - 1;
+    int src[T::NR] = {};
+    skip3_row_sources<T>(p, own_a, own_b, src);
+    const bool two = p.runs > 1;
+    const Skip3Rows a = skip3_run_rows(p.gp0[0], p.len[0]);
+    const Skip3Rows b = two ? skip3_run_rows(p.gp0[1], p.len[1]) : Skip3Rows{a.row0 + a.n, 0};
+    const long long last = b.row0 + b.n - 1;
+    bool image = false;
+    for (int i = 0; i < T::NR; ++i) image = image || (src[i] != S3_SRC_NONE && (src[i] & S3_SRC_IMAGE));
+    const bool front = image && IMG + last + 1 <= R::REACH_ROWS;
+    const long long base = front ? 0 : IMG + a.row0, back = IMG + total;
+    for (int i = 0; i < T::ROW_WORDS; ++i) {
+        const int s = i < T::NR ? src[i < T::NR ? i : 0] : S3_SRC_NONE;
+        const bool none = s == S3_SRC_NONE, img = !none && (s & S3_SRC_IMAGE);
+        const long long row = img ? (front ? 0 : back) + (s & ~S3_SRC_IMAGE) : IMG + s;
+        const unsigned off = none ? R::OFF_NONE : (unsigned)((row - base) * R::ROWB) + (unsigned)((i < a.n ? t0a : t0b) * R::TILEB);
+        w[i] = i == BASE ? (unsigned)base : off - ((unsigned)i << R::ROW_SHIFT);
+    }
+}
+TREXHIP_HD constexpr bool skip3t_direct_fits(const long long total) {
+    using R = Skip3Reach;
+    return total <= 2 * R::REACH_ROWS - 2 * SkipGeom::V3_ROWS - ((Skip3TXGeom::SPAN + Skip3TXGeom::SLOTS) * SkipGeom::POOL + 2 * Skip3TXGeom::HALO) - 1;
+}
+static_assert(Skip3TGeom::NR < Skip3TGeom::ROW_WORDS - 1 && Skip3TGeom::ROW_WORDS == Skip3Reach::WORDS, "the row table holds a pass's rows and `none`");
+
 
 static_assert(Skip3Geom::PAIRS == FC1_KSPLIT, "plane s of the split-K fc1 is row pair s");
 TREXHIP_HD constexpr bool skip3_fc1_listed(const bool all, const SkipBand b, const int q) {
diff --git a/trex_amd/csrc/cnn_skip_kernels.h b/trex_amd/csrc/cnn_skip_kernels.h
--- a/trex_amd/csrc/cnn_skip_kernels.h
+++ b/trex_amd/csrc/cnn_skip_kernels.h
@@ -205,23 +205,24 @@
 
 static constexpr int SKIP3_TB = 256;
 
-static constexpr int SKIP3_NT = 2 * SKIP3_TB;
+static constexpr int SKIP3_NT = 2 * SKIP3_TB, SKIP3_NT_TILED = 4 * SKIP3_TB;
+template <int NT>
 __device__ __forceinline__ void skip3_stage_runs(const int2* __restrict__ bands, const int2* __restrict__ cols, const int n, const bool all, uint16_t* s_run) {
     using G = Skip3Geom;
     const int c0 = blockIdx.x * SKIP3_TB * G::BLOCK;
     constexpr int U = 8;
-    static_assert(G::BLOCK % U == 0 && (SKIP3_TB * G::BLOCK) % (U * SKIP3_NT) == 0, "whole groups of loads");
-    for (int i0 = threadIdx.x; i0 < SKIP3_TB * G::BLOCK; i0 += U * SKIP3_NT) {
+    static_assert(G::BLOCK % U == 0 && (SKIP3_TB * G::BLOCK) % (U * NT) == 0, "whole groups of loads");
+    for (int i0 = threadIdx.x; i0 < SKIP3_TB * G::BLOCK; i0 += U * NT) {
         int2 b[U], c[U];
 #pragma unroll
         for (int u = 0; u < U; ++u) {
-            const int i = i0 + u * SKIP3_NT;
+            const int i = i0 + u * NT;
             b[u] = c0 + i < n ? bands[c0 + i] : make_int2(SKIP_BAND_NONE.y0, SKIP_BAND_NONE.y1);
             c[u] = cols && c0 + i < n ? cols[c0 + i] : make_int2(SKIP_BAND_NONE.y0, SKIP_BAND_NONE.y1);
         }
 #pragma unroll
         for (int u = 0; u < U; ++u) {
-            const int i = i0 + u * SKIP3_NT;
+            const int i = i0 + u * NT;
             const SkipPairs r = all && c0 + i < n ? SkipPairs{0, G::PAIRS - 1} : skip3_pairs({b[u].x, b[u].y});
             const int t0 = skip3_window({c[u].x, c[u].y}, all);
             s_run[(i % G::BLOCK) * SKIP3_TB + i / G::BLOCK] = (uint16_t)(r.lo <= r.hi ? r.lo | (r.hi - r.lo + 1) << 8 | (t0 + 1) << 12 : 0);
@@ -231,8 +232,8 @@
 }
 template <class G, class E>
 __device__ __forceinline__ int skip3_walk(const uint16_t* s_run, const int t, const int blk, int& passes, int& crops, E&& emit) {
-    constexpr bool WIN = G::TILES != Skip3Geom::TILES;
-    Skip3Pass p{};
+    constexpr bool WIN = G::TILES != Skip3Geom::TILES, TILED = Skip3Tiled<G>::value;
+    std::conditional_t<TILED, Skip3TPass, Skip3Pass> p{};
     int listed = 0;
 #pragma unroll 1
     for (int k = 0; k < G::BLOCK; ++k) {
@@ -240,51 +241,67 @@
         if (len && ((r >> 12) != 0) == WIN) {
             listed += len;
             ++crops;
-            skip3_add_run<G>(p, passes, (blk * G::BLOCK + k) * G::PAIRS + (r & 0xff), len, emit);
-        }
-    }
-    skip3_flush(p, passes, emit);
+            const int gp = (blk * G::BLOCK + k) * G::PAIRS + (r & 0xff);
+            if constexpr (TILED) skip3t_add_run<G>(p, passes, gp, len, emit);
+            else skip3_add_run<G>(p, passes, gp, len, emit);
+        }
+    }
+    if constexpr (TILED) skip3t_flush(p, passes, emit);
+    else skip3_flush(p, passes, emit);
     return listed;
 }
 
-__global__ __launch_bounds__(SKIP3_NT) void k_pair_count(const int2* __restrict__ bands, const int2* __restrict__ cols, const int n, const uint32_t* __restrict__ words,
+template <bool TILED>
+__global__ __launch_bounds__(TILED ? SKIP3_NT_TILED : SKIP3_NT) void k_pair_count(const int2* __restrict__ bands, const int2* __restrict__ cols, const int n, const uint32_t* __restrict__ words,
                                                          uint4* __restrict__ counts ,
                                                          uint32_t* __restrict__ tcounts ) {
-    __shared__ uint32_t s_pass, s_pair, s_wpass, s_wcrop;
+    __shared__ uint32_t s_pass, s_pair, s_wpass, s_wcrop, s_ppass, s_pwpass;
     __shared__ uint16_t s_run[SKIP3_TB * Skip3Geom::BLOCK];
-    if (threadIdx.x == 0) { s_pass = 0; s_pair = 0; s_wpass = 0; s_wcrop = 0; }
-    skip3_stage_runs(bands, cols, n, words[SK_EMPTY_RANGE] != 0, s_run);
-    const bool win = threadIdx.x >= SKIP3_TB;
+    if (threadIdx.x == 0) { s_pass = 0; s_pair = 0; s_wpass = 0; s_wcrop = 0; s_ppass = 0; s_pwpass = 0; }
+    skip3_stage_runs<TILED ? SKIP3_NT_TILED : SKIP3_NT>(bands, cols, n, words[SK_EMPTY_RANGE] != 0, s_run);
+    const int grp = threadIdx.x / SKIP3_TB;
+    const bool win = grp & 1;
     const int t = threadIdx.x & (SKIP3_TB - 1), blk = blockIdx.x * SKIP3_TB + t;
     if (blk * Skip3Geom::BLOCK < n) {
         int passes = 0, crops = 0, listed = 0;
-        if (!win) listed = skip3_walk<Skip3Geom>(s_run, t, blk, passes, crops, [](int, const Skip3Pass&) {});
-        else if (cols) listed = skip3_walk<Skip3XGeom>(s_run, t, blk, passes, crops, [](int, const Skip3Pass&) {});
-        tcounts[2 * blk + (win ? 1 : 0)] = (uint32_t)passes;
-        if (passes) atomicAdd(win ? &s_wpass : &s_pass, (uint32_t)passes);
-        if (listed) atomicAdd(&s_pair, (uint32_t)listed);
-        if (win && crops) atomicAdd(&s_wcrop, (uint32_t)crops);
-    }
-    __syncthreads();
-    if (threadIdx.x == 0) counts[blockIdx.x] = make_uint4(s_pass, s_pair, s_wpass, s_wcrop);
-}
-
+        const auto none = [](int, const auto&) {};
+        if (grp >= 2) {
+            if (!win) skip3_walk<Skip3Geom>(s_run, t, blk, passes, crops, none);
+            else if (cols) skip3_walk<Skip3XGeom>(s_run, t, blk, passes, crops, none);
+            if (passes) atomicAdd(win ? &s_pwpass : &s_ppass, (uint32_t)passes);
+        } else {
+            if (!win) listed = skip3_walk<std::conditional_t<TILED, Skip3TGeom, Skip3Geom>>(s_run, t, blk, passes, crops, none);
+            else if (cols) listed = skip3_walk<std::conditional_t<TILED, Skip3TXGeom, Skip3XGeom>>(s_run, t, blk, passes, crops, none);
+            tcounts[2 * blk + (win ? 1 : 0)] = (uint32_t)passes;
+            if (passes) atomicAdd(win ? &s_wpass : &s_pass, (uint32_t)passes);
+            if (listed) atomicAdd(&s_pair, (uint32_t)listed);
+            if (win && crops) atomicAdd(&s_wcrop, (uint32_t)crops);
+        }
+    }
+    __syncthreads();
+    if (threadIdx.x == 0) {
+        counts[blockIdx.x] = make_uint4(s_pass, s_pair, s_wpass, s_wcrop);
+        counts[gridDim.x + blockIdx.x] = TILED ? make_uint4(s_ppass, s_pwpass, 0, 0) : make_uint4(s_pass, s_wpass, 0, 0);
+    }
+}
+
+template <bool TILED>
 __global__ __launch_bounds__(SKIP3_NT) void k_pair_list(const int2* __restrict__ bands, const int2* __restrict__ cols, const int n, uint32_t* __restrict__ words,
                                                         const uint4* __restrict__ counts, const uint32_t* __restrict__ tcounts, int* __restrict__ desc,
                                                         int* __restrict__ xdesc ) {
-    using G = Skip3Geom;
-    using X = Skip3XGeom;
+    using G = std::conditional_t<TILED, Skip3TGeom, Skip3Geom>;
+    using X = std::conditional_t<TILED, Skip3TXGeom, Skip3XGeom>;
     __shared__ uint2 s_scan[SKIP3_TB];
     __shared__ uint16_t s_run[SKIP3_TB * G::BLOCK];
     const int tid = threadIdx.x, t = tid & (SKIP3_TB - 1), blk = blockIdx.x * SKIP3_TB + t;
     const bool win = tid >= SKIP3_TB;
     const bool mine = blk * G::BLOCK < n;
-    skip3_stage_runs(bands, cols, n, words[SK_EMPTY_RANGE] != 0, s_run);
-    uint32_t before = 0, wbefore = 0, pairs = 0, wcrops = 0;
+    skip3_stage_runs<SKIP3_NT>(bands, cols, n, words[SK_EMPTY_RANGE] != 0, s_run);
+    uint32_t before = 0, wbefore = 0, pairs = 0, wcrops = 0, ppasses = 0, pwpasses = 0;
     for (int b = 0; b <= (int)blockIdx.x; ++b) {
-        const uint4 c = counts[b];
+        const uint4 c = counts[b], pc = counts[gridDim.x + b];
         if (b < (int)blockIdx.x) { before += c.x; wbefore += c.z; }
-        pairs += c.y; wcrops += c.w;
+        pairs += c.y; wcrops += c.w; ppasses += pc.x; pwpasses += pc.y;
     }
     const uint2 cnt = mine ? make_uint2(tcounts[2 * blk], tcounts[2 * blk + 1]) : make_uint2(0, 0);
     if (!win) s_scan[t] = cnt;
@@ -296,20 +313,22 @@
         __syncthreads();
     }
     int at = win ? (int)(wbefore + s_scan[t].y - cnt.y) : (int)(before + s_scan[t].x - cnt.x), crops = 0;
+    const auto runs_of = [](const auto& p) {
+        int la = p.len[0];
+        if constexpr (std::is_same_v<std::decay_t<decltype(p)>, Skip3TPass>) la |= (p.o | p.n << S3_COUNT_SHIFT) << 8;
+        return make_int4(p.gp0[0], la, p.gp0[1], p.runs > 1 ? p.len[1] : 0);
+    };
     if (mine && !win)
-        skip3_walk<G>(s_run, t, blk, at, crops, [&](const int idx, const Skip3Pass& p) {
-            *reinterpret_cast<int4*>(desc + (size_t)idx * G::DESC) = make_int4(p.gp0[0], p.len[0], p.gp0[1], p.runs > 1 ? p.len[1] : 0);
-        });
+        skip3_walk<G>(s_run, t, blk, at, crops, [&](const int idx, const auto& p) { *reinterpret_cast<int4*>(desc + (size_t)idx * G::DESC) = runs_of(p); });
     if (mine && win && cols)
-        skip3_walk<X>(s_run, t, blk, at, crops, [&](const int idx, const Skip3Pass& p) {
-            *reinterpret_cast<int4*>(xdesc + (size_t)idx * X::DESC) = make_int4(p.gp0[0], p.len[0], p.gp0[1], p.runs > 1 ? p.len[1] : 0);
-        });
+        skip3_walk<X>(s_run, t, blk, at, crops, [&](const int idx, const auto& p) { *reinterpret_cast<int4*>(xdesc + (size_t)idx * X::DESC) = runs_of(p); });
     if (blockIdx.x == gridDim.x - 1 && tid == SKIP3_TB - 1) {
         const uint32_t listed = before + s_scan[t].x, wlisted = wbefore + s_scan[t].y;
         const long long dense = ((long long)n * (G::PAIRS * 10) + 63) / 64;
-        words[SK3_PAIRS] = (uint32_t)(n * G::PAIRS); words[SK3_LISTED] = pairs; words[SK3_PASSES] = listed; words[SK3_FILLED] = 0;
-        words[SK3X_PASSES] = wlisted; words[SK3X_CROPS] = wcrops; words[SK3X_CTR] = 0;
-        words[SK3_USE] = skip3_use_list((long long)listed + wlisted, dense) ? 1u : 0u;
+        words[SK3_PAIRS] = (uint32_t)(n * G::PAIRS); words[SK3_LISTED] = pairs; words[SK3_PASSES] = ppasses; words[SK3_FILLED] = 0;
+        words[SK3X_PASSES] = pwpasses; words[SK3X_CROPS] = wcrops; words[SK3X_CTR] = 0;
+        words[SK3_RAN] = listed; words[SK3X_RAN] = wlisted;
+        words[SK3_USE] = skip3_use_list((long long)ppasses + pwpasses, dense) ? 1u : 0u;
     }
 }
 
@@ -361,17 +380,26 @@
 }
 
 static constexpr int SKIP3_FC = 16;
+template <bool TILED>
 __global__ __launch_bounds__(256) void k_act3_fill(const int2* __restrict__ bands, const int2* __restrict__ cols, const int n, uint32_t* __restrict__ words,
                                                    const uint4* __restrict__ act3e, uint4* __restrict__ act3, int* __restrict__ desc,
                                                    uint32_t* __restrict__ rows ,
-                                                   int* __restrict__ xdesc, uint32_t* __restrict__ xrows,
+                                                   int* __restrict__ xdesc, uint32_t* __restrict__ xrows ,
                                                    const long long alloc_rows , const int direct,
                                                    const int copy ) {
-    using G = Skip3Geom;
+    using G = std::conditional_t<TILED, Skip3TGeom, Skip3Geom>;
     constexpr int PQ = 10 * 128 * 4 / 16;
-    using X = Skip3XGeom;
+    using X = std::conditional_t<TILED, Skip3TXGeom, Skip3XGeom>;
     constexpr int CQ = 128 * 4 / 16;
-    static_assert((Skip3Geom::BLOCK_PASSES + X::BLOCK_PASSES) * SKIP3_FC <= Skip3Geom::BLOCK * 256 && SKIP3_FC % 4 == 0, "a thread per pass of either list: 256 threads per SKIP3_FC crops");
+    static_assert((G::BLOCK_PASSES + X::BLOCK_PASSES) * SKIP3_FC <= Skip3Geom::BLOCK * 256 && SKIP3_FC % 4 == 0, "a thread per pass of either list: 256 threads per SKIP3_FC crops");
+    const auto pass_of = [](const int4 r, int& tiles) {
+        Skip3Pass p{};
+        const int la = TILED ? r.y & 0xff : r.y;
+        tiles = TILED ? r.y >> 8 : 0;
+        p.runs = r.w ? 2 : 1; p.n = la + r.w;
+        p.gp0[0] = r.x; p.len[0] = la; p.gp0[1] = r.z; p.len[1] = r.w;
+        return p;
+    };
     __shared__ uint32_t s_filled;
     const int lane = threadIdx.x & 63;
     if (!words[SK3_USE]) return;
@@ -379,42 +407,45 @@
     __syncthreads();
     const bool all = words[SK_EMPTY_RANGE] != 0;
     const int gid = blockIdx.x * 256 + threadIdx.x;
-    const int n_full = (int)words[SK3_PASSES], n_win = cols ? (int)words[SK3X_PASSES] : 0;
+    const int n_full = (int)words[SK3_RAN], n_win = cols ? (int)words[SK3X_RAN] : 0;
     const SkipRows every{0, SkipGeom::V3_ROWS - 1};
     const bool from_v3 = all || !direct;
     if (gid >= n_full && gid - n_full < n_win) {
         int4* dst = reinterpret_cast<int4*>(xdesc + (size_t)(gid - n_full) * X::DESC);
         const int4 r = dst[0];
-        Skip3Pass p{};
-        p.runs = r.w ? 2 : 1; p.n = r.y + r.w;
-        p.gp0[0] = r.x; p.len[0] = r.y; p.gp0[1] = r.z; p.len[1] = r.w;
+        int tiles;
+        const Skip3Pass p = pass_of(r, tiles);
         const int ca = r.x / X::PAIRS, cb = (r.w ? r.z : r.x) / X::PAIRS;
         const int2 xa = cols[ca], xb = cols[cb];
         const int t0a = skip3_window({xa.x, xa.y}, all), t0b = skip3_window({xb.x, xb.y}, all);
         int d[X::DESC];
         skip3_describe<X>(p, d, t0a, t0b);
+        if (TILED) d[S3_TILES] = tiles;
 #pragma unroll
         for (int k = 0; k < X::DESC / 4; ++k) dst[k] = make_int4(d[4 * k], d[4 * k + 1], d[4 * k + 2], d[4 * k + 3]);
         const int2 ba = bands[ca], bb = bands[cb];
-        unsigned w[Skip3Reach::WORDS];
-        skip3_row_words<X>(p, from_v3 ? every : skip_rows({ba.x, ba.y}), from_v3 ? every : skip_rows({bb.x, bb.y}), alloc_rows, w, t0a, t0b);
-        uint4* wd = reinterpret_cast<uint4*>(xrows + (size_t)(gid - n_full) * Skip3Reach::WORDS);
-#pragma unroll
-        for (int k = 0; k < Skip3Reach::WORDS / 4; ++k) wd[k] = make_uint4(w[4 * k], w[4 * k + 1], w[4 * k + 2], w[4 * k + 3]);
+        constexpr int XW = TILED ? Skip3TXGeom::ROW_WORDS : Skip3Reach::WORDS;
+        unsigned w[XW];
+        const SkipRows oa = from_v3 ? every : skip_rows({ba.x, ba.y}), ob = from_v3 ? every : skip_rows({bb.x, bb.y});
+        if constexpr (TILED) skip3t_row_words<X>(p, oa, ob, alloc_rows, w, t0a, t0b);
+        else skip3_row_words<X>(p, oa, ob, alloc_rows, w, t0a, t0b);
+        uint4* wd = reinterpret_cast<uint4*>(xrows + (size_t)(gid - n_full) * XW);
+#pragma unroll
+        for (int k = 0; k < XW / 4; ++k) wd[k] = make_uint4(w[4 * k], w[4 * k + 1], w[4 * k + 2], w[4 * k + 3]);
     }
     if (gid < n_full) {
         int4* dst = reinterpret_cast<int4*>(desc + (size_t)gid * G::DESC);
         const int4 r = dst[0];
-        Skip3Pass p{};
-        p.runs = r.w ? 2 : 1; p.n = r.y + r.w;
-        p.gp0[0] = r.x; p.len[0] = r.y; p.gp0[1] = r.z; p.len[1] = r.w;
+        int tiles;
+        const Skip3Pass p = pass_of(r, tiles);
         int d[G::DESC];
-        skip3_describe(p, d);
+        skip3_describe<G>(p, d);
+        if (TILED) d[S3_TILES] = tiles;
 #pragma unroll
         for (int k = 0; k < G::DESC / 4; ++k) dst[k] = make_int4(d[4 * k], d[4 * k + 1], d[4 * k + 2], d[4 * k + 3]);
         const int2 ba = bands[r.x / G::PAIRS], bb = bands[(r.w ? r.z : r.x) / G::PAIRS];
         unsigned w[Skip3Reach::WORDS];
-        skip3_row_words(p, from_v3 ? every : skip_rows({ba.x, ba.y}), from_v3 ? every : skip_rows({bb.x, bb.y}), alloc_rows, w);
+        skip3_row_words<G>(p, from_v3 ? every : skip_rows({ba.x, ba.y}), from_v3 ? every : skip_rows({bb.x, bb.y}), alloc_rows, w);
         uint4* wd = reinterpret_cast<uint4*>(rows + (size_t)gid * Skip3Reach::WORDS);
 #pragma unroll
         for (int k = 0; k < Skip3Reach::WORDS / 4; ++k) wd[k] = make_uint4(w[4 * k], w[4 * k + 1], w[4 * k + 2], w[4 * k + 3]);
diff --git a/trex_amd/csrc/cnn_skip_words.h b/trex_amd/csrc/cnn_skip_words.h
--- a/trex_amd/csrc/cnn_skip_words.h
+++ b/trex_amd/csrc/cnn_skip_words.h
@@ -27,8 +27,10 @@
     SKX_CTR = 29,
     SKX_V2_READ = 30,
     SKX_V2_MADE = 31,
-    SK_WORDS = 32
+    SK3_RAN = 32,
+    SK3X_RAN = 33,
+    SK_WORDS = 34
 };
-static_assert(SK_FILLED < SK3X_CROPS && SK3X_CTR < SK3_PAIRS && SK3_LAST < SKX_CROPS && SKX_V2_MADE < SK_WORDS, "no word twice, the last one inside the table");
+static_assert(SK_FILLED < SK3X_CROPS && SK3X_CTR < SK3_PAIRS && SK3_LAST < SKX_CROPS && SKX_V2_MADE < SK3_RAN && SK3X_RAN < SK_WORDS, "no word twice, the last one inside the table");
 
 }
```
